# ErickRosete/tacorl

Hardware: AMD Instinct MI355X
Metric: offline grad-steps/sec (batch=256, 84x84 RGB) (higher is better)
Workload: dtype bf16; 1 GPU; tacorl actor-critic training_step, frozen LMP (BASELINE configs[1]); per_gpu_batch=256, global_batch=256, window=16, image=84x84x3, frames=fp32 CHW (reference batch schema), latent_plan=16, n_action_samples=4, phase=Q (epoch>=bc_epochs), action_decoder_loss=every step (reference behaviour), parallelism=dp1, hip_graph=True, losses_finite=True

## Files before the change

### include/tacorl_hip.h

```cpp
#ifndef TACORL_HIP_H
#define TACORL_HIP_H
#include <stddef.h>
#ifdef __cplusplus
extern "C" {
#endif

typedef void* tacorl_stream_t;

#define TACORL_MAXP 16
enum { TACORL_F32 = 0, TACORL_BF16 = 1 };
enum { TACORL_ACT_NONE = 0, TACORL_ACT_RELU = 1, TACORL_ACT_SILU = 2 };

int tacorl_hip_version(void);
int tacorl_hip_init(int device);
const char* tacorl_hip_last_error(void);
int tacorl_time_mark(unsigned long long* marks, int slot, tacorl_stream_t stream);
int tacorl_time_spin(unsigned long long* marks, int slot, long ticks, tacorl_stream_t stream);

int tacorl_linear_fwd(int nprob, const float* const* x, int ldx, const float* const* w,
                      const float* const* b, float* const* y, float* const* z, const int* M,
                      int K, int N, int act, int compute_dtype, tacorl_stream_t stream);
size_t tacorl_linear_add_fwd_ws_bytes(int nprob, const int* M, int K, int N);
int tacorl_linear_add_fwd(int nprob, const float* const* x, int ldx, const float* const* w,
                          const float* const* b, const float* const* addend, int ld_add, float* const* y,
                          int ldy, const int* M, int K, int N, int act, int compute_dtype, void* ws,
                          size_t ws_bytes, tacorl_stream_t stream);
int tacorl_rnn_linear_supported(int M, int K, int N);
int tacorl_rnn_linear_fwd(const void* x_bf16, const void* w_bf16, const float* bias, const float* addend,
                          int ld_add, float* y, void* y_bf16, int M, int K, int N, int act,
                          tacorl_stream_t stream);
int tacorl_rnn_linear_fwd_batch(int nprob, const void* const* x_bf16, const void* const* w_bf16,
                                const float* const* bias, const float* const* addend, int ld_add,
                                float* const* y, void* const* y_bf16, int M, int K, int N, const int* acts,
                                tacorl_stream_t stream);
int tacorl_rnn_linear_fwd_batch_twin(int nprob, const void* const* x_bf16, const void* const* x2_bf16,
                                     const void* const* w_bf16, const float* const* bias, const float* const* addend,
                                     const float* const* addend2, int ld_add, float* const* y, float* const* y2,
                                     void* const* y_bf16, void* const* y2_bf16, int M, int M2, int K, int N,
                                     const int* acts, tacorl_stream_t stream);
int tacorl_rnn_linear_fwd_batch_ext(int nprob, const void* const* x_bf16, const void* const* x2_bf16,
                                    const void* const* w_bf16, const float* const* bias, const float* const* addend,
                                    const float* const* addend2, int ld_add, float* const* y, float* const* y2,
                                    void* const* y_bf16, void* const* y2_bf16, int M, int M2, int K, int N,
                                    const int* acts, const void* const* x_ext, const void* const* x2_ext,
                                    const void* const* w_ext, const float* const* bias2, tacorl_stream_t stream);
int tacorl_build_ad_input_bf16(const float* plan, const float* emb, int ld_emb, void* out_bf16, int B, int T, int Tm,
                               int P, int E, tacorl_stream_t stream);
int tacorl_rnn_linear_bwd_step(const void* x_bf16, const void* wt_bf16, const float* addend, int ld_add,
                               const float* mask_src, float* y, void* y_bf16, int M, int K, int N,
                               tacorl_stream_t stream);
int tacorl_rnn_wgrad_supported(int R, int M, int N);
int tacorl_rnn_wgrad(const void* dz_bf16, int ld_dz, const void* x_bf16, int ld_x, int R, int M, int N, float* dw,
                     float* db, int accumulate, tacorl_stream_t stream);
int tacorl_rnn_wgrad_batch(int n, const void* const* dz_bf16, int ld_dz, const void* const* x_bf16, int ld_x, const int* R,
                           int M, int N, float* const* dw, float* const* db, int accumulate, tacorl_stream_t stream);
size_t tacorl_rnn_wgrad_slabs_ws_bytes(int slabs, int Mp, int N);
int tacorl_rnn_wgrad_slabs(const void* dz_bf16, int ld_dz, const void* x_bf16, int ld_x, int R, int Mp, int N, int rows,
                           int slabs, float* dw, float* db, int accumulate, void* ws, size_t ws_bytes, tacorl_stream_t stream);
int tacorl_rnn_linear_bwd_batch(int nprob, const void* const* x_bf16, const void* const* wt_bf16,
                                const float* const* addend, int ld_add, const float* const* mask_src,
                                float* const* y, void* const* y_bf16, int M, int K, int N, tacorl_stream_t stream);
int tacorl_transpose_to_bf16(const float* src, void* dst, int R, int C, tacorl_stream_t stream);
int tacorl_transpose_to_bf16_batch(int n, const float* const* src, void* const* dst, const int* R, const int* C,
                                   tacorl_stream_t stream);
int tacorl_transpose_pad_to_bf16(const float* src, void* dst, int R, int C, int ld_dst, tacorl_stream_t stream);
int tacorl_pad_to_bf16(const float* src, int ld_src, void* dst, int ld_dst, long rows, int cols, tacorl_stream_t stream);

int tacorl_linear_dgrad(int nprob, const float* const* dz, int ld_dz, const float* const* w,
                        float* const* out, int ld_out, const float* const* src, int ld_src, int act_src,
                        const float* const* addend, int ld_add, const int* M, int O, int I,
                        int compute_dtype, tacorl_stream_t stream);
size_t tacorl_linear_dgrad_ws_bytes(int nprob, const int* M, int O, int I);
int tacorl_linear_dgrad_splitk(int nprob, const float* const* dz, int ld_dz, const float* const* w,
                               float* const* out, int ld_out, const float* const* src, int ld_src, int act_src,
                               const float* const* addend, int ld_add, const int* M, int O, int I,
                               int compute_dtype, void* ws, size_t ws_bytes, tacorl_stream_t stream);
size_t tacorl_linear_wgrad_ws_bytes(int nprob, const int* M, int K, int O);
int tacorl_linear_wgrad(int nprob, const float* const* x, int ldx, const float* const* dz, int ld_dz,
                        const int* M, int K, int O, float* const* dw, float* const* db, int accumulate,
                        int compute_dtype, void* ws, size_t ws_bytes, tacorl_stream_t stream);
int tacorl_conv2d_relu_fwd(int nprob, const void* const* x, const float* const* w,
                           const float* const* b, float* const* y, const int* n_img, int H, int W,
                           int C, int KH, int KW, int S, int CO, int x_dtype, int compute_dtype,
                           tacorl_stream_t stream);

long tacorl_encoder_param_layout(long* offsets11);
long tacorl_encoder_act_layout(int n_img, int H, int W, long* offsets5);
int tacorl_encoder_fwd(int nprob, const void* const* img, const float* const* params,
                       float* const* out , float* const* act, const int* n_img, int H,
                       int W, int img_dtype, int compute_dtype, tacorl_stream_t stream);
size_t tacorl_encoder_bwd_ws_bytes(int nprob, const int* n_img, int H, int W);
int tacorl_encoder_bwd(int nprob, const void* const* img, const float* const* params,
                       const float* const* act, const float* const* d_out, float* const* grads,
                       const int* n_img, int H, int W, int img_dtype, int compute_dtype,
                       int accumulate, void* ws, size_t ws_bytes, tacorl_stream_t stream);

long tacorl_encoder_fused_wpk_bytes(void);
int tacorl_encoder_fused_supported(int H, int W);
int tacorl_encoder_fused_act_format(int H, int W);
int tacorl_encoder_pack_weights(int nprob, const float* const* params, void* const* packed,
                                tacorl_stream_t stream);
int tacorl_encoder_fwd_fused(int nprob, const void* const* img, const void* const* packed,
                             const float* const* params, float* const* out, float* const* act,
                             const int* n_img, int H, int W, tacorl_stream_t stream);
int tacorl_encoder_fwd_fused_wg(int nprob, const void* const* img, const void* const* packed,
                                const float* const* params, float* const* out, float* const* act,
                                const int* n_img, int H, int W, int max_workgroups, tacorl_stream_t stream);

size_t tacorl_encoder_bwd_fused_ws_bytes(int nprob, const int* n_img, int H, int W);
int tacorl_encoder_bwd_fused(int nprob, const void* const* img, const float* const* params,
                             const float* const* act, const float* const* d_out,
                             float* const* grads, const int* n_img, int H, int W, int accumulate,
                             void* ws, size_t ws_bytes, tacorl_stream_t stream);
int tacorl_encoder_bwd_fused_pack(int nprob, const float* const* params, const int* n_img, int H, int W,
                                  void* ws, size_t ws_bytes, tacorl_stream_t stream);
int tacorl_encoder_bwd_fused_head(int nprob, const float* const* params, const float* const* act,
                                  const float* const* d_out, const int* n_img, int H, int W,
                                  int prepacked, void* ws, size_t ws_bytes, tacorl_stream_t stream);
int tacorl_encoder_bwd_fused_fc_wgrad(int nprob, const float* const* act, const float* const* d_out,
                                      float* const* grads, const int* n_img, int H, int W,
                                      int accumulate, void* ws, size_t ws_bytes, tacorl_stream_t stream);
int tacorl_encoder_bwd_fused_conv(int nprob, const void* const* img, const float* const* params,
                                  const float* const* act, float* const* grads, const int* n_img, int H,
                                  int W, int accumulate, int prepacked, void* ws, size_t ws_bytes,
                                  tacorl_stream_t stream);
int tacorl_encoder_bwd_fused_conv_parts(int nprob, const void* const* img, const float* const* params,
                                        const float* const* act, float* const* grads, const int* n_img, int H,
                                        int W, int accumulate, int prepacked, int parts, void* ws,
                                        size_t ws_bytes, tacorl_stream_t stream);

long tacorl_mlp_param_layout(int n_layers, const int* dims, long* w_off, long* b_off);
long tacorl_mlp_act_layout(int M, int n_layers, const int* dims, const int* acts, long* z_off,
                           long* y_off);
int tacorl_mlp_fwd(int nprob, const float* const* x, int ldx, const float* const* params,
                   float* const* act, const int* M, int n_layers, const int* dims,
                   const int* acts, int compute_dtype, tacorl_stream_t stream);
int tacorl_mlp_fwd_fused_supported(int nprob, int n_layers, const int* dims, int ldx);
int tacorl_mlp_lean_supported(int nprob, int n_layers, const int* dims, int ldx, int ldo, int ldd);
int tacorl_mlp_fwd_fused(int nprob, const float* const* x, int ldx, const float* const* params,
                         const void* const* params_bf16, float* const* act, const int* M,
                         int n_layers, const int* dims, const int* acts, int lean, tacorl_stream_t stream);
int tacorl_mlp_fwd_fused_gather_supported(int nprob, const int* M, int n_layers, const int* dims, const int* acts,
                                          int ldx, int lean);
int tacorl_mlp_fwd_fused_gather(int nprob, const int* nseg, const float* const* seg_ptr, const int* seg_ld,
                                const int* seg_c0, const int* seg_mod, float* const* x_out, int ldx,
                                const float* const* params, const void* const* params_bf16, float* const* act,
                                const int* M, int n_layers, const int* dims, const int* acts, int lean,
                                tacorl_stream_t stream);
int tacorl_to_bf16_batch(int n, const float* const* src, void* const* dst, const long* count,
                         tacorl_stream_t stream);
size_t tacorl_mlp_bwd_ws_bytes(int nprob, const int* M, int n_layers, const int* dims);
int tacorl_mlp_bwd(int nprob, const float* const* x, int ldx, const float* const* params,
                   const float* const* act, const float* const* d_out, int ldo, float* const* grads,
                   float* const* d_x, int ldd, const int* M, int n_layers, const int* dims,
                   const int* acts, int compute_dtype, int accumulate, void* ws, size_t ws_bytes,
                   tacorl_stream_t stream);
int tacorl_mlp_bwd_fused_supported(int nprob, int n_layers, const int* dims, int ldo, int ldd);
size_t tacorl_mlp_bwd_fused_ws_bytes(int nprob, const int* M, int n_layers, const int* dims);
int tacorl_mlp_bwd_fused_dgrad(int nprob, const float* const* params, const float* const* act,
                               const float* const* d_out, int ldo, float* const* d_x, int ldd,
                               const int* M, int n_layers, const int* dims, const int* acts,
                               int prepacked, void* ws, size_t ws_bytes, tacorl_stream_t stream);
int tacorl_mlp_bwd_fused_pack(int nprob, const float* const* params, const int* M, int n_layers,
                              const int* dims, void* ws, size_t ws_bytes, tacorl_stream_t stream);
int tacorl_prep_batch_begin(void);
int tacorl_reduce_batch_begin(void);
int tacorl_reduce_batch_end(tacorl_stream_t stream);
int tacorl_prep_batch_end(tacorl_stream_t stream);
int tacorl_mlp_bwd_fused_wgrad(int nprob, const float* const* x, int ldx, const float* const* act,
                               const float* const* d_out, int ldo, float* const* grads, const int* M,
                               int n_layers, const int* dims, const int* acts, int accumulate, int lean,
                               void* ws, size_t ws_bytes, tacorl_stream_t stream);

int tacorl_pack_images(const float* src, long img_pitch, int src_nchw, void* dst, int dst_dtype,
                       int n, int C, int H, int W, tacorl_stream_t stream);
int tacorl_pack_images_batch(int njobs, const float* const* src, const long* img_pitch, void* const* dst,
                             const int* n_img, int dst_dtype, int H, int W, tacorl_stream_t stream);
int tacorl_pack_images_window_batch(int njobs, const float* const* src, const long* img_pitch, void* const* dst,
                                    const int* n_img, void* const* dst_first, void* const* dst_last,
                                    const int* window, int dst_dtype, int H, int W, tacorl_stream_t stream);
int tacorl_pack_images_u8_batch(int njobs, const void* const* src, const long* img_pitch_bytes, void* const* dst,
                                const int* n_img, int dst_dtype, int H, int W, tacorl_stream_t stream);
int tacorl_pack_images_u8_gather_batch(int njobs, const void* const* src, const long* img_pitch_bytes,
                                       const long* const* index, const int* index_stride, void* const* dst,
                                       const int* n_img, int dst_dtype, int H, int W, tacorl_stream_t stream);
int tacorl_gather_frames_u8(const void* frames, long frame_bytes, const long* index, void* dst, long n,
                            tacorl_stream_t stream);
int tacorl_pack_images_u8_aug_batch(int njobs, const void* const* src, const long* img_pitch_bytes,
                                    void* const* dst, const int* const* shift, const float* const* jitter,
                                    const int* n_img, int dst_dtype, int H, int W, int pad,
                                    tacorl_stream_t stream);
int tacorl_pack_images_u8_resize_aug_gather_batch(int njobs, const void* const* src, const long* img_pitch_bytes,
                                                  const long* const* index, const int* index_stride, void* const* dst,
                                                  const int* const* shift, const float* const* jitter, const int* n_img,
                                                  int dst_dtype, int src_H, int src_W, int H, int W, int pad,
                                                  tacorl_stream_t stream);
int tacorl_pack_images_u8_aug_gather_batch(int njobs, const void* const* src, const long* img_pitch_bytes,
                                           const long* const* index, const int* index_stride, void* const* dst,
                                           const int* const* shift, const float* const* jitter, const int* n_img,
                                           int dst_dtype, int H, int W, int pad, tacorl_stream_t stream);
int tacorl_stage_transition(const void* disp, int disp_dtype, float* reward, float* done, int B,
                            const float* acts_src, float* acts_dst, long n_acts, tacorl_stream_t stream);
int tacorl_copy_cols(const float* src, int ld_src, float* dst, int ld_dst, int rows, int cols,
                     int src_row_mod, int accumulate, tacorl_stream_t stream);
int tacorl_copy_cols_batch(int n, const float* const* src, const int* ld_src, float* const* dst,
                           const int* ld_dst, const int* rows, const int* cols,
                           const int* src_row_mod, const int* accumulate, tacorl_stream_t stream);
int tacorl_reduce_rows_mod(const float* in, int ld_in, float* out, int ld_out, int B, int cols,
                           int reps, tacorl_stream_t stream);
int tacorl_reduce_rows_mod_batch(int n, const float* const* in, int ld_in, float* const* out, int ld_out, int B,
                                 int cols, int reps, tacorl_stream_t stream);
int tacorl_uniform_actions(const float* u01, float* dst, int ld_dst, int rows, int A,
                           int discrete_gripper, tacorl_stream_t stream);

int tacorl_tanh_normal_sample(const float* head, int ld_head, const float* eps, const float* gumbel_u,
                              int hard_rsample, float* act_out, int ld_act, float* logp, int* grip_idx,
                              int n, int M, int Ac, tacorl_stream_t stream);
int tacorl_tanh_normal_sample_batch(int njobs, const float* const* head, int ld_head,
                                    const float* const* eps, const float* const* gumbel_u,
                                    const int* hard_rsample, float* const* act_out, int ld_act,
                                    float* const* logp, int* const* grip_idx, const int* n, int M, int Ac,
                                    const float* u01, float* u_dst, int u_rows, int A, int u_discrete,
                                    tacorl_stream_t stream);

int tacorl_add_rows_bcast(const float* x, int ldx, const float* add, float* out, int R, int T, int D,
                          int Dp, tacorl_stream_t stream);
int tacorl_attention_fwd(const float* qkv, float* out, int B, int T, int D, int H, tacorl_stream_t stream);
int tacorl_attention_dropout_fwd(const float* qkv, float* out, const unsigned char* keep, float keep_scale, int B,
                                 int T, int D, int H, tacorl_stream_t stream);
int tacorl_attention_dropout_bwd(const float* qkv, const float* d_out, float* d_qkv, const unsigned char* keep,
                                 float keep_scale, int B, int T, int D, int H, tacorl_stream_t stream);
int tacorl_dropout_mul(float* x, const unsigned char* keep, float keep_scale, long n, tacorl_stream_t stream);
int tacorl_add_layernorm_fwd(const float* x, const float* res, const float* w, const float* b, float* y,
                             float* stats, int R, int D, float eps, tacorl_stream_t stream);
int tacorl_pr_encoder_fused_supported(int D, int T, int H, int FF, int L);
int tacorl_pr_encoder_fused_train_supported(int D, int T, int H, int FF, int L);
int tacorl_pr_encoder_fused(const float* emb, int ld_emb, const float* params, const void* params_bf16,
                            const long* offsets, float* pooled, int B, int D, int T, int H, int FF, int L,
                            tacorl_stream_t stream);
int tacorl_pr_encoder_fused_sample(const float* emb, int ld_emb, const float* params, const void* params_bf16,
                                   const long* offsets, float* pooled, int B, int D, int T, int H, int FF, int L,
                                   const float* Wc, const float* bc, const float* eps, float* head, float* plan,
                                   int A, float min_std, tacorl_stream_t stream);
int tacorl_pr_encoder_fused_train(const float* emb, int ld_emb, const float* params, const void* params_bf16,
                                  const long* offsets, float* pooled, int B, int D, int T, int H, int FF, int L,
                                  float* const* save, tacorl_stream_t stream);
int tacorl_pr_encoder_bwd_fused(const float* params, const long* offsets, const float* d_pool, const float* d_head,
                                const float* Wc, int A2, float* dx, const float* const* saved, float* const* dz,
                                const void* const* wt, float* ln_part, float* const* ln_grads, int B, int D, int T, int H,
                                int FF, int L, tacorl_stream_t stream);
int tacorl_pr_encoder_fused_train_sample(const float* emb, int ld_emb, const float* params, const void* params_bf16,
                                         const long* offsets, float* pooled, int B, int D, int T, int H, int FF, int L,
                                         float* const* save, const float* Wc, const float* bc, const float* eps,
                                         float* head, float* plan, int A, float min_std, tacorl_stream_t stream);
int tacorl_pr_head_compose(const float* w_fc, const float* b_fc, const float* w_head, const float* b_head,
                           float* Wc, float* bc, int D, int FC, int A2, tacorl_stream_t stream);
int tacorl_mean_over_t(const float* x, float* out, int B, int T, int D, tacorl_stream_t stream);
int tacorl_pr_sample(const float* head, const float* eps, float* plan, float* mu_out, float* std_out,
                     int B, int A, float min_std, tacorl_stream_t stream);

int tacorl_build_ad_input(const float* plan, const float* emb, int ld_emb, float* out, int B, int T,
                          int Tm, int P, int E, tacorl_stream_t stream);
int tacorl_ad_input_proj(const float* plan, const float* emb, int ld_emb, const float* w_ih, const float* b_ih,
                         float* out, int B, int T, int Tm, int P, int E, int H, tacorl_stream_t stream);
size_t tacorl_logistic_mixture_ws_bytes(int B, int Tm, int Da);
int tacorl_logistic_mixture_loss(const float* heads, int ldh, const float* actions, float* d_heads,
                                 float* loss_out, int B, int T, int Tm, int Da, int K, int num_classes,
                                 float gripper_alpha, float grad_scale, void* ws, size_t ws_bytes,
                                 tacorl_stream_t stream);
int tacorl_logistic_mixture_finish(const void* ws, size_t ws_bytes, int B, int Tm, int Da, float* loss_out,
                                   tacorl_stream_t stream);
int tacorl_logistic_mixture_sample(const float* heads, int ldh, const float* rand_a, const float* rand_b,
                                   float* out, int R, int Da, int K, tacorl_stream_t stream);

int tacorl_relu_mask_mul(const float* dy, const float* add, const float* h, float* out, long n,
                         tacorl_stream_t stream);
int tacorl_ad_input_bwd(const float* dx, float* d_plan, float* d_emb, int ld_emb, int B, int T, int Tm,
                        int P, int E, int accumulate, tacorl_stream_t stream);
int tacorl_plmp_demb_finish(float* d_emb, const float* dx, int ld_dx, int D_in, const float* dS, int ld_ds,
                            const float* dgin, float* const* f_dout, int ncam, int B, int T, int Ec,
                            tacorl_stream_t stream);
int tacorl_bcast_over_t(const float* src, float* dst, int B, int T, int D, float scale, int accumulate,
                        tacorl_stream_t stream);
int tacorl_attention_bwd(const float* qkv, const float* d_out, float* d_qkv, int B, int T, int D, int H,
                         tacorl_stream_t stream);
size_t tacorl_add_layernorm_bwd_ws_bytes(int R, int D);
int tacorl_add_layernorm_bwd(const float* dy, const float* x, const float* res, const float* w,
                             const float* stats, float* dv, float* dw, float* db, int R, int D,
                             int accumulate, void* ws, size_t ws_bytes, tacorl_stream_t stream);
int tacorl_gauss_kl_balanced(const float* head_q, const float* head_p, float* d_head_q, float* d_head_p,
                             int B, int A, float kl_alpha, float kl_beta, float min_std, int balanced,
                             float grad_scale, float* out2, tacorl_stream_t stream);
int tacorl_pr_sample_bwd(const float* head, const float* eps, const float* d_plan, float* d_head, int B,
                         int A, float min_std, tacorl_stream_t stream);

enum {
  TACORL_LG_ALPHA_LOSS = 0, TACORL_LG_ALPHA, TACORL_LG_ACTOR_LOSS, TACORL_LG_BELL1, TACORL_LG_BELL2,
  TACORL_LG_CONS1, TACORL_LG_CONS2, TACORL_LG_Q1LOSS, TACORL_LG_Q2LOSS, TACORL_LG_ALPHA_P,
  TACORL_LG_ALPHA_P_LOSS, TACORL_LG_Q1_DATA, TACORL_LG_Q1_RAND, TACORL_LG_Q1_POL, TACORL_LG_Q2_DATA,
  TACORL_LG_Q2_RAND, TACORL_LG_Q2_POL, TACORL_LG_ACTION_LOSS, TACORL_LG_COUNT
};
int tacorl_alpha_loss(const float* logp, int B, const float* log_alpha, float target_entropy,
                      float grad_scale, float* g_log_alpha, float* logs, tacorl_stream_t stream);
int tacorl_alpha_loss_step(const float* logp, int B, float* log_alpha, float target_entropy, float* g_log_alpha,
                           float* logs, float* m, float* v, float lr, int* step_counter, tacorl_stream_t stream);
int tacorl_actor_qmin(const float* q1, const float* q2, const float* logp, int B, const float* log_alpha,
                      float* dq1, float* dq2, float grad_scale, float* logs, tacorl_stream_t stream);
int tacorl_actor_head_bwd(const float* head, int ld_head, const float* eps, const float* logp,
                          const float* g_act1, const float* g_act2, int ld_g, const float* value,
                          int ld_value, const int* grip_idx, const float* log_alpha, float grad_scale,
                          float* d_head, int B, int Ac, int has_grip, float* logs, tacorl_stream_t stream);

size_t tacorl_cql_ws_bytes(int B);
int tacorl_cql_loss(const float* q1, const float* q2, float* dq1, float* dq2, const float* tq1,
                    const float* tq2, const float* logp_cur, const float* logp_nxt, const float* next_logp,
                    const float* reward, const float* done, const float* log_alpha,
                    const float* log_alpha_prime, int B, int n, int A, float discount, float reward_scale,
                    float temp, float cons_w, float gap, int deterministic_backup, float grad_scale,
                    float* g_log_alpha_prime, float* logs, void* ws, size_t ws_bytes, tacorl_stream_t stream);

size_t tacorl_adam_ws_bytes(long n);
int tacorl_adam_step(float* param, const float* grad, float* m, float* v, long n, float lr,
                     float max_norm, int* step_counter, float* target, float tau, void* ws,
                     size_t ws_bytes, tacorl_stream_t stream);
size_t tacorl_adam_batch_ws_bytes(int nb);
int tacorl_adam_step_batch(int nb, float* const* param, const float* const* grad, float* const* m,
                           float* const* v, const long* n, const float* lr, const float* max_norm,
                           int* const* step_counter, float* const* target, const float* tau, void* ws,
                           size_t ws_bytes, tacorl_stream_t stream);
int tacorl_adam_step_batch_mirror(int nb, float* const* param, const float* const* grad, float* const* m,
// ... 10 lines not shown
```

### tacorl_amd/_lib.py

```python
import ctypes as C
import os

HERE = os.path.dirname(os.path.abspath(__file__))
LIB_PATH = os.environ.get("TACORL_HIP_LIB") or os.path.join(HERE, "lib", "libtacorl_hip.so")

F32, BF16 = 0, 1
ACT_NONE, ACT_RELU, ACT_SILU = 0, 1, 2
MAXP = 16

LOG_SLOTS = [
    "alpha_loss", "alpha", "actor_loss", "bellman_q1_loss", "bellman_q2_loss", "conservative_q1_loss",
    "conservative_q2_loss", "q1_loss", "q2_loss", "alpha_prime", "alpha_prime_loss", "q1_data", "q1_random",
    "q1_policy", "q2_data", "q2_random", "q2_policy", "action_loss",
]

_p, _i, _l, _f, _sz = C.c_void_p, C.c_int, C.c_long, C.c_float, C.c_size_t
_SIGS = {
    "tacorl_hip_version": (_i, []),
    "tacorl_hip_init": (_i, [_i]),
    "tacorl_hip_last_error": (C.c_char_p, []),
    "tacorl_time_mark": (_i, [_p, _i, _p]),
    "tacorl_time_spin": (_i, [_p, _i, _l, _p]),
    "tacorl_linear_fwd": (_i, [_i, _p, _i, _p, _p, _p, _p, _p, _i, _i, _i, _i, _p]),
    "tacorl_linear_add_fwd_ws_bytes": (_sz, [_i, _p, _i, _i]),
    "tacorl_linear_add_fwd": (_i, [_i, _p, _i, _p, _p, _p, _i, _p, _i, _p, _i, _i, _i, _i, _p, _sz, _p]),
    "tacorl_rnn_linear_supported": (_i, [_i, _i, _i]),
    "tacorl_rnn_linear_fwd": (_i, [_p, _p, _p, _p, _i, _p, _p, _i, _i, _i, _i, _p]),
    "tacorl_rnn_linear_fwd_batch": (_i, [_i, _p, _p, _p, _p, _i, _p, _p, _i, _i, _i, _p, _p]),
    "tacorl_rnn_linear_fwd_batch_twin": (_i, [_i, _p, _p, _p, _p, _p, _p, _i, _p, _p, _p, _p, _i, _i, _i, _i, _p, _p]),
    "tacorl_rnn_linear_fwd_batch_ext": (_i, [_i, _p, _p, _p, _p, _p, _p, _i, _p, _p, _p, _p, _i, _i, _i, _i, _p, _p, _p, _p, _p, _p]),
    "tacorl_rnn_linear_bwd_step": (_i, [_p, _p, _p, _i, _p, _p, _p, _i, _i, _i, _p]),
    "tacorl_rnn_linear_bwd_batch": (_i, [_i, _p, _p, _p, _i, _p, _p, _p, _i, _i, _i, _p]),
    "tacorl_rnn_wgrad_supported": (_i, [_i, _i, _i]),
    "tacorl_rnn_wgrad": (_i, [_p, _i, _p, _i, _i, _i, _i, _p, _p, _i, _p]),
    "tacorl_rnn_wgrad_batch": (_i, [_i, _p, _i, _p, _i, _p, _i, _i, _p, _p, _i, _p]),
    "tacorl_rnn_wgrad_slabs_ws_bytes": (_sz, [_i, _i, _i]),
    "tacorl_rnn_wgrad_slabs": (_i, [_p, _i, _p, _i, _i, _i, _i, _i, _i, _p, _p, _i, _p, _sz, _p]),
    "tacorl_transpose_to_bf16": (_i, [_p, _p, _i, _i, _p]),
    "tacorl_transpose_to_bf16_batch": (_i, [_i, _p, _p, _p, _p, _p]),
    "tacorl_transpose_pad_to_bf16": (_i, [_p, _p, _i, _i, _i, _p]),
    "tacorl_pad_to_bf16": (_i, [_p, _i, _p, _i, _l, _i, _p]),
    "tacorl_pr_encoder_fused_supported": (_i, [_i, _i, _i, _i, _i]),
    "tacorl_pr_encoder_fused_train_supported": (_i, [_i, _i, _i, _i, _i]),
    "tacorl_pr_encoder_fused": (_i, [_p, _i, _p, _p, _p, _p, _i, _i, _i, _i, _i, _i, _p]),
    "tacorl_pr_encoder_fused_train": (_i, [_p, _i, _p, _p, _p, _p, _i, _i, _i, _i, _i, _i, _p, _p]),
    "tacorl_pr_encoder_bwd_fused": (_i, [_p, _p, _p, _p, _p, _i, _p, _p, _p, _p, _p, _p, _i, _i, _i, _i, _i, _i, _p]),
    "tacorl_pr_encoder_fused_train_sample": (_i, [_p, _i, _p, _p, _p, _p, _i, _i, _i, _i, _i, _i, _p, _p, _p, _p, _p, _p, _i, _f, _p]),
    "tacorl_pr_encoder_fused_sample": (_i, [_p, _i, _p, _p, _p, _p, _i, _i, _i, _i, _i, _i, _p, _p, _p, _p, _p, _i, _f, _p]),
    "tacorl_pr_head_compose": (_i, [_p, _p, _p, _p, _p, _p, _i, _i, _i, _p]),
    "tacorl_to_bf16_batch": (_i, [_i, _p, _p, _p, _p]),
    "tacorl_mlp_bwd_fused_supported": (_i, [_i, _i, _p, _i, _i]),
    "tacorl_mlp_bwd_fused_ws_bytes": (_sz, [_i, _p, _i, _p]),
    "tacorl_mlp_bwd_fused_dgrad": (_i, [_i, _p, _p, _p, _i, _p, _i, _p, _i, _p, _p, _i, _p, _sz, _p]),
    "tacorl_mlp_bwd_fused_pack": (_i, [_i, _p, _p, _i, _p, _p, _sz, _p]),
    "tacorl_prep_batch_begin": (_i, []),
    "tacorl_reduce_batch_begin": (_i, []),
    "tacorl_reduce_batch_end": (_i, [_p]),
    "tacorl_prep_batch_end": (_i, [_p]),
    "tacorl_mlp_bwd_fused_wgrad": (_i, [_i, _p, _i, _p, _p, _i, _p, _p, _i, _p, _p, _i, _i, _p, _sz, _p]),
    "tacorl_mlp_fwd_fused_supported": (_i, [_i, _i, _p, _i]),
    "tacorl_mlp_lean_supported": (_i, [_i, _i, _p, _i, _i, _i]),
    "tacorl_mlp_fwd_fused": (_i, [_i, _p, _i, _p, _p, _p, _p, _i, _p, _p, _i, _p]),
    "tacorl_mlp_fwd_fused_gather_supported": (_i, [_i, _p, _i, _p, _p, _i, _i]),
    "tacorl_mlp_fwd_fused_gather": (_i, [_i, _p, _p, _p, _p, _p, _p, _i, _p, _p, _p, _p, _i, _p, _p, _i, _p]),
    "tacorl_add_rows_bcast": (_i, [_p, _i, _p, _p, _i, _i, _i, _i, _p]),
    "tacorl_attention_fwd": (_i, [_p, _p, _i, _i, _i, _i, _p]),
    "tacorl_attention_dropout_fwd": (_i, [_p, _p, _p, _f, _i, _i, _i, _i, _p]),
    "tacorl_attention_dropout_bwd": (_i, [_p, _p, _p, _p, _f, _i, _i, _i, _i, _p]),
    "tacorl_dropout_mul": (_i, [_p, _p, _f, _l, _p]),
    "tacorl_add_layernorm_fwd": (_i, [_p, _p, _p, _p, _p, _p, _i, _i, _f, _p]),
    "tacorl_mean_over_t": (_i, [_p, _p, _i, _i, _i, _p]),
    "tacorl_pr_sample": (_i, [_p, _p, _p, _p, _p, _i, _i, _f, _p]),
    "tacorl_build_ad_input": (_i, [_p, _p, _i, _p, _i, _i, _i, _i, _i, _p]),
    "tacorl_build_ad_input_bf16": (_i, [_p, _p, _i, _p, _i, _i, _i, _i, _i, _p]),
    "tacorl_ad_input_proj": (_i, [_p, _p, _i, _p, _p, _p, _i, _i, _i, _i, _i, _i, _p]),
    "tacorl_logistic_mixture_ws_bytes": (_sz, [_i, _i, _i]),
    "tacorl_logistic_mixture_loss": (_i, [_p, _i, _p, _p, _p, _i, _i, _i, _i, _i, _i, _f, _f, _p, _sz, _p]),
    "tacorl_logistic_mixture_finish": (_i, [_p, _sz, _i, _i, _i, _p, _p]),
    "tacorl_logistic_mixture_sample": (_i, [_p, _i, _p, _p, _p, _i, _i, _i, _p]),
    "tacorl_linear_dgrad": (_i, [_i, _p, _i, _p, _p, _i, _p, _i, _i, _p, _i, _p, _i, _i, _i, _p]),
    "tacorl_linear_dgrad_ws_bytes": (_sz, [_i, _p, _i, _i]),
    "tacorl_linear_dgrad_splitk": (_i, [_i, _p, _i, _p, _p, _i, _p, _i, _i, _p, _i, _p, _i, _i, _i, _p, _sz, _p]),
    "tacorl_linear_wgrad_ws_bytes": (_sz, [_i, _p, _i, _i]),
    "tacorl_linear_wgrad": (_i, [_i, _p, _i, _p, _i, _p, _i, _i, _p, _p, _i, _i, _p, _sz, _p]),
    "tacorl_relu_mask_mul": (_i, [_p, _p, _p, _p, _l, _p]),
    "tacorl_ad_input_bwd": (_i, [_p, _p, _p, _i, _i, _i, _i, _i, _i, _i, _p]),
    "tacorl_plmp_demb_finish": (_i, [_p, _p, _i, _i, _p, _i, _p, _p, _i, _i, _i, _i, _p]),
    "tacorl_bcast_over_t": (_i, [_p, _p, _i, _i, _i, _f, _i, _p]),
    "tacorl_attention_bwd": (_i, [_p, _p, _p, _i, _i, _i, _i, _p]),
    "tacorl_add_layernorm_bwd_ws_bytes": (_sz, [_i, _i]),
    "tacorl_add_layernorm_bwd": (_i, [_p, _p, _p, _p, _p, _p, _p, _p, _i, _i, _i, _p, _sz, _p]),
    "tacorl_gauss_kl_balanced": (_i, [_p, _p, _p, _p, _i, _i, _f, _f, _f, _i, _f, _p, _p]),
    "tacorl_pr_sample_bwd": (_i, [_p, _p, _p, _p, _i, _i, _f, _p]),
    "tacorl_conv2d_relu_fwd": (_i, [_i, _p, _p, _p, _p, _p, _i, _i, _i, _i, _i, _i, _i, _i, _i, _p]),
    "tacorl_encoder_param_layout": (_l, [_p]),
    "tacorl_encoder_act_layout": (_l, [_i, _i, _i, _p]),
    "tacorl_encoder_fwd": (_i, [_i, _p, _p, _p, _p, _p, _i, _i, _i, _i, _p]),
    "tacorl_encoder_bwd_ws_bytes": (_sz, [_i, _p, _i, _i]),
    "tacorl_encoder_bwd": (_i, [_i, _p, _p, _p, _p, _p, _p, _i, _i, _i, _i, _i, _p, _sz, _p]),
    "tacorl_encoder_fused_wpk_bytes": (_l, []),
    "tacorl_encoder_fused_supported": (_i, [_i, _i]),
    "tacorl_encoder_fused_act_format": (_i, [_i, _i]),
    "tacorl_encoder_pack_weights": (_i, [_i, _p, _p, _p]),
    "tacorl_encoder_fwd_fused": (_i, [_i, _p, _p, _p, _p, _p, _p, _i, _i, _p]),
    "tacorl_encoder_fwd_fused_wg": (_i, [_i, _p, _p, _p, _p, _p, _p, _i, _i, _i, _p]),
    "tacorl_encoder_bwd_fused_ws_bytes": (_sz, [_i, _p, _i, _i]),
    "tacorl_encoder_bwd_fused": (_i, [_i, _p, _p, _p, _p, _p, _p, _i, _i, _i, _p, _sz, _p]),
    "tacorl_encoder_bwd_fused_pack": (_i, [_i, _p, _p, _i, _i, _p, _sz, _p]),
    "tacorl_encoder_bwd_fused_head": (_i, [_i, _p, _p, _p, _p, _i, _i, _i, _p, _sz, _p]),
    "tacorl_encoder_bwd_fused_fc_wgrad": (_i, [_i, _p, _p, _p, _p, _i, _i, _i, _p, _sz, _p]),
    "tacorl_encoder_bwd_fused_conv": (_i, [_i, _p, _p, _p, _p, _p, _i, _i, _i, _i, _p, _sz, _p]),
    "tacorl_encoder_bwd_fused_conv_parts": (_i, [_i, _p, _p, _p, _p, _p, _i, _i, _i, _i, _i, _p, _sz, _p]),
    "tacorl_mlp_param_layout": (_l, [_i, _p, _p, _p]),
    "tacorl_mlp_act_layout": (_l, [_i, _i, _p, _p, _p, _p]),
    "tacorl_mlp_fwd": (_i, [_i, _p, _i, _p, _p, _p, _i, _p, _p, _i, _p]),
    "tacorl_mlp_bwd_ws_bytes": (_sz, [_i, _p, _i, _p]),
    "tacorl_mlp_bwd": (_i, [_i, _p, _i, _p, _p, _p, _i, _p, _p, _i, _p, _i, _p, _p, _i, _i, _p, _sz, _p]),
    "tacorl_pack_images": (_i, [_p, _l, _i, _p, _i, _i, _i, _i, _i, _p]),
    "tacorl_pack_images_batch": (_i, [_i, _p, _p, _p, _p, _i, _i, _i, _p]),
    "tacorl_pack_images_window_batch": (_i, [_i, _p, _p, _p, _p, _p, _p, _p, _i, _i, _i, _p]),
    "tacorl_pack_images_u8_batch": (_i, [_i, _p, _p, _p, _p, _i, _i, _i, _p]),
    "tacorl_pack_images_u8_gather_batch": (_i, [_i, _p, _p, _p, _p, _p, _p, _i, _i, _i, _p]),
    "tacorl_pack_images_u8_aug_gather_batch": (_i, [_i, _p, _p, _p, _p, _p, _p, _p, _p, _i, _i, _i, _i, _p]),
    "tacorl_pack_images_u8_resize_aug_gather_batch": (_i, [_i, _p, _p, _p, _p, _p, _p, _p, _p, _i, _i, _i, _i, _i, _i, _p]),
    "tacorl_gather_frames_u8": (_i, [_p, _l, _p, _p, _l, _p]),
    "tacorl_pack_images_u8_aug_batch": (_i, [_i, _p, _p, _p, _p, _p, _p, _i, _i, _i, _i, _p]),
    "tacorl_stage_transition": (_i, [_p, _i, _p, _p, _i, _p, _p, _l, _p]),
    "tacorl_copy_cols": (_i, [_p, _i, _p, _i, _i, _i, _i, _i, _p]),
    "tacorl_copy_cols_batch": (_i, [_i, _p, _p, _p, _p, _p, _p, _p, _p, _p]),
    "tacorl_reduce_rows_mod": (_i, [_p, _i, _p, _i, _i, _i, _i, _p]),
    "tacorl_reduce_rows_mod_batch": (_i, [_i, _p, _i, _p, _i, _i, _i, _i, _p]),
    "tacorl_uniform_actions": (_i, [_p, _p, _i, _i, _i, _i, _p]),
    "tacorl_tanh_normal_sample": (_i, [_p, _i, _p, _p, _i, _p, _i, _p, _p, _i, _i, _i, _p]),
    "tacorl_tanh_normal_sample_batch": (_i, [_i, _p, _i, _p, _p, _p, _p, _i, _p, _p, _p, _i, _i, _p, _p, _i, _i, _i, _p]),
    "tacorl_alpha_loss": (_i, [_p, _i, _p, _f, _f, _p, _p, _p]),
    "tacorl_alpha_loss_step": (_i, [_p, _i, _p, _f, _p, _p, _p, _p, _f, _p, _p]),
    "tacorl_actor_qmin": (_i, [_p, _p, _p, _i, _p, _p, _p, _f, _p, _p]),
    "tacorl_actor_head_bwd": (_i, [_p, _i, _p, _p, _p, _p, _i, _p, _i, _p, _p, _f, _p, _i, _i, _i, _p, _p]),
    "tacorl_cql_ws_bytes": (_sz, [_i]),
    "tacorl_cql_loss": (_i, [_p] * 13 + [_i, _i, _i, _f, _f, _f, _f, _f, _i, _f, _p, _p, _p, _sz, _p]),
    "tacorl_adam_ws_bytes": (_sz, [_l]),
    "tacorl_adam_step": (_i, [_p, _p, _p, _p, _l, _f, _f, _p, _p, _f, _p, _sz, _p]),
    "tacorl_adam_batch_ws_bytes": (_sz, [_i]),
    "tacorl_adam_step_batch": (_i, [_i, _p, _p, _p, _p, _p, _p, _p, _p, _p, _p, _p, _sz, _p]),
    "tacorl_adam_step_batch_mirror": (_i, [_i, _p, _p, _p, _p, _p, _p, _p, _p, _p, _p, _p, _p, _p, _sz, _p]),
}

_lib = None


class TacorlHipError(RuntimeError):
    pass


def lib():
    global _lib
    if _lib is None:
        import torch

        if not os.path.exists(LIB_PATH):
            raise TacorlHipError(
                f"{LIB_PATH} not found: the HIP extension is required (no CPU fallback). "
                "Build it with `python -m tacorl_amd.build`.")
        L = C.CDLL(LIB_PATH)
        override = bool(os.environ.get("TACORL_HIP_LIB"))
        missing = []
        for name, (res, args) in _SIGS.items():
            fn = getattr(L, name, None)
            if fn is None:
                missing.append(name)
                continue
            fn.restype, fn.argtypes = res, args
        if override:
            import sys

            if missing:
                raise TacorlHipError(f"TACORL_HIP_LIB={LIB_PATH} lacks {len(missing)} entry point(s) of this binding "
                                     f"({', '.join(missing[:5])}...): rebuild it from this tree")
            print(f"[tacorl_amd] TACORL_HIP_LIB override active: {LIB_PATH}", file=sys.stderr, flush=True)
        _lib = L
    return _lib


def declared_symbols():
    return list(_SIGS)


def call(name, *args):
    fn = getattr(lib(), name)
    rc = fn(*args)
    if fn.restype is _i and rc != 0:
        raise TacorlHipError(f"{name} failed ({rc}): {lib().tacorl_hip_last_error().decode()}")
    return rc


def ptr(t):
    return None if t is None else C.c_void_p(t.data_ptr())


def ptr_array(tensors):
    arr = (C.c_void_p * len(tensors))()
    for i, t in enumerate(tensors):
        if t is None:
            arr[i] = None
        elif isinstance(t, int):
            arr[i] = t
        elif isinstance(t, C.c_void_p):
            arr[i] = t.value
        else:
            arr[i] = t.data_ptr()
    return arr


def int_array(vals):
    return (C.c_int * len(vals))(*[int(v) for v in vals])


def stream():
    import torch

    return C.c_void_p(torch.cuda.current_stream().cuda_stream)
```

### tacorl_amd/csrc/encoder_fused.h

```cpp
#pragma once
#include "../../include/tacorl_hip.h"
#include "common.h"

#define EF_CHUNK 16
constexpr int cmaxi(int a, int b) { return a > b ? a : b; }
#define EF_MAXCH 12
#define EF_MAXP 16
#define ACT1_STRIDE 80
#define SA_STRIDE 272
#define H1_STRIDE 528

typedef unsigned int u32x4 __attribute__((ext_vector_type(4)));
typedef unsigned int u32x2 __attribute__((ext_vector_type(2)));

struct EFProblem {
  const __bf16* img;
  const u32x4* wpk;
  const float* params;
  float* out;
  float* act;
  long a_y2, a_y3, a_sa, a_h1;
  int n_img;
  int cost;
  long ustart;
};
struct EFArgs {
  EFProblem p[EF_MAXP];
  long utotal;
  int nprob;
  int H, W, OH1, OW1, OH2, OW2, OH3, OW3;
  int img_bytes;
  int lds_img;
  int act_bf16;
};

#define WP_C1 0
#define WP_C2 (WP_C1 + 2 * 6 * 64)
#define WP_C3 (WP_C2 + 4 * 16 * 64)
#define WP_F1 (WP_C3 + 4 * 18 * 64)
#define WP_F2 (WP_F1 + 16 * 4 * 64)
#define WP_TOTAL (WP_F2 + 2 * 8 * 64)

__device__ __forceinline__ bf16x8 as_bf16x8(u32x4 v) { return __builtin_bit_cast(bf16x8, v); }
__device__ __forceinline__ float relu1(float x) {
  float r;
  asm("v_max_f32_e32 %0, 0, %1" : "=v"(r) : "v"(x));
  return r;
}
#define EF_DPP4(OP, CTRL, x)                                                                  \
  asm volatile(OP " %0, %0, %0 " CTRL " row_mask:0xf bank_mask:0xf\n\t"                        \
               OP " %1, %1, %1 " CTRL " row_mask:0xf bank_mask:0xf\n\t"                        \
               OP " %2, %2, %2 " CTRL " row_mask:0xf bank_mask:0xf\n\t"                        \
               OP " %3, %3, %3 " CTRL " row_mask:0xf bank_mask:0xf"                             \
               : "+v"((x)[0]), "+v"((x)[1]), "+v"((x)[2]), "+v"((x)[3]))
#define EF_DPP4_FIRST(OP, CTRL, x)                                                            \
  asm volatile("s_nop 1\n\t"                                                                   \
               OP " %0, %0, %0 " CTRL " row_mask:0xf bank_mask:0xf\n\t"                        \
               OP " %1, %1, %1 " CTRL " row_mask:0xf bank_mask:0xf\n\t"                        \
               OP " %2, %2, %2 " CTRL " row_mask:0xf bank_mask:0xf\n\t"                        \
               OP " %3, %3, %3 " CTRL " row_mask:0xf bank_mask:0xf"                             \
               : "+v"((x)[0]), "+v"((x)[1]), "+v"((x)[2]), "+v"((x)[3]))
#define EF_ROW16_4(OP, x)                          \
  do {                                             \
    EF_DPP4_FIRST(OP, "quad_perm:[1,0,3,2]", x);   \
    EF_DPP4(OP, "quad_perm:[2,3,0,1]", x);         \
    EF_DPP4(OP, "row_half_mirror", x);             \
    EF_DPP4(OP, "row_mirror", x);                  \
  } while (0)
__device__ __forceinline__ u32x2 pack4_bf16(float a, float b, float c, float d) {
  bf16x4 t = {(__bf16)a, (__bf16)b, (__bf16)c, (__bf16)d};
  return __builtin_bit_cast(u32x2, t);
}

#ifndef EF_VAR
#define EF_VAR 0
#endif
#if EF_VAR & 2
#define MFMA_AW(acc, wfrag, bfrag) asm volatile("" : "+v"(acc) : "a"(wfrag), "v"(bfrag))
#else
#define MFMA_AW(acc, wfrag, bfrag) \
  asm volatile("v_mfma_f32_16x16x32_bf16 %0, %1, %2, %0" : "+v"(acc) : "a"(wfrag), "v"(bfrag))
#endif
#define MFMA_CHAIN_BEGIN(acc) asm volatile("s_nop 1" : "+v"(acc))
#if EF_VAR & 2
#define MFMA_FIRST_AW(acc, wfrag, bfrag, bias) asm volatile("" : "=v"(acc) : "a"(wfrag), "v"(bfrag), "v"(bias))
#else
#define MFMA_FIRST_AW(acc, wfrag, bfrag, bias) \
  asm volatile("v_mfma_f32_16x16x32_bf16 %0, %1, %2, %3" : "=v"(acc) : "a"(wfrag), "v"(bfrag), "v"(bias))
#endif
#define MFMA_CHAIN_END(acc) asm volatile("s_nop 11" : "+v"(acc))
#if EF_VAR & 2
#define EF_MFMA_TXT(...) ""
#else
#define EF_MFMA_TXT(...) __VA_ARGS__
#endif

int ef_ring_supported(int H, int W);
int ef_ring_launch(EFArgs& a, int nb, int H, int W, hipStream_t st);
```

### tacorl_amd/csrc/encoder_fused.hip

```cpp
#include <stdio.h>
#include <stdlib.h>

#include "encoder_fused.h"
#include "enc_bwd_fused.h"

#ifndef EF_DEFER
#define EF_DEFER 1
#endif
#define EF_DCHUNK 8
#ifndef EF_SETUP_COST
#define EF_SETUP_COST 128
#endif
#ifndef EF_ACT_COST
#define EF_ACT_COST 72
#endif


struct EFPackArgs {
  const float* params[16];
  u32x4* out[16];
};
__global__ void ef_pack_kernel(EFPackArgs a, long o_w1, long o_w2, long o_w3, long o_f1, long o_f2) {
  const float* __restrict__ params = a.params[blockIdx.y];
  u32x4* __restrict__ out = a.out[blockIdx.y];
  const int f = blockIdx.x * 4 + (threadIdx.x >> 6), l = threadIdx.x & 63;
  if (f >= WP_TOTAL / 64) return;
  const float* W; int K, j, s;
  if (f < WP_C2 / 64) { W = params + o_w1; K = 192; j = f / 6; s = f % 6; }
  else if (f < WP_C3 / 64) { int r = f - WP_C2 / 64; W = params + o_w2; K = 512; j = r / 16; s = r % 16; }
  else if (f < WP_F1 / 64) { int r = f - WP_C3 / 64; W = params + o_w3; K = 576; j = r / 18; s = r % 18; }
  else if (f < WP_F2 / 64) { int r = f - WP_F1 / 64; W = params + o_f1; K = 128; j = r / 4; s = r % 4; }
  else { int r = f - WP_F2 / 64; W = params + o_f2; K = 256; j = r / 8; s = r % 8; }
  const float* src = W + (long)(16 * j + (l & 15)) * K + 32 * s + 8 * (l >> 4);
  if (f < WP_C2 / 64)
    src = W + (long)(8 * ((l & 15) >> 2) + 4 * j + (l & 3)) * K + (4 * (s / 3) + (l >> 4)) * 24 + 8 * (s % 3);
  else if (f < WP_C3 / 64)
    src = W + (long)(32 * (j >> 1) + 8 * ((l & 15) >> 2) + 4 * (j & 1) + (l & 3)) * K + 32 * s + 8 * (l >> 4);
  bf16x8 v;
#pragma unroll
  for (int e = 0; e < 8; e++) v[e] = (__bf16)src[e];
  out[(long)f * 64 + l] = __builtin_bit_cast(u32x4, v);
}

extern "C" long tacorl_encoder_fused_wpk_bytes(void) { return (long)WP_TOTAL * 16; }
extern "C" int tacorl_encoder_pack_weights(int nprob, const float* const* params, void* const* packed,
                                           tacorl_stream_t stream) {
  long po[11];
  tacorl_encoder_param_layout(po);
  if (nprob < 1 || nprob > 16) return TACORL_EINVAL;
  EFPackArgs a{};
  for (int p = 0; p < nprob; p++) { a.params[p] = params[p]; a.out[p] = (u32x4*)packed[p]; }
  hipLaunchKernelGGL(ef_pack_kernel, dim3((WP_TOTAL / 64 + 3) / 4, nprob), dim3(256), 0, (hipStream_t)stream, a, po[0],
                     po[2], po[4], po[7], po[9]);
  return hipGetLastError() == hipSuccess ? TACORL_OK : TACORL_ELAUNCH;
}

#define MFMA6_FIRST(acc, bias, w, o, f) \
  asm volatile(EF_MFMA_TXT("v_mfma_f32_16x16x32_bf16 %0, %1, %7, %13\n\t" \
      "v_mfma_f32_16x16x32_bf16 %0, %2, %8, %0\n\t" \
      "v_mfma_f32_16x16x32_bf16 %0, %3, %9, %0\n\t" \
      "v_mfma_f32_16x16x32_bf16 %0, %4, %10, %0\n\t" \
      "v_mfma_f32_16x16x32_bf16 %0, %5, %11, %0\n\t" \
      "v_mfma_f32_16x16x32_bf16 %0, %6, %12, %0\n\t") \
      : "=&v"(acc) : "a"((w)[(o) + 0]), "a"((w)[(o) + 1]), "a"((w)[(o) + 2]), "a"((w)[(o) + 3]), "a"((w)[(o) + 4]), "a"((w)[(o) + 5]), "v"((f)[0]), "v"((f)[1]), "v"((f)[2]), "v"((f)[3]), "v"((f)[4]), "v"((f)[5]), "v"(bias))
#define MFMA6_MORE(acc, w, o, f) \
  asm volatile(EF_MFMA_TXT("v_mfma_f32_16x16x32_bf16 %0, %1, %7, %0\n\t" \
      "v_mfma_f32_16x16x32_bf16 %0, %2, %8, %0\n\t" \
      "v_mfma_f32_16x16x32_bf16 %0, %3, %9, %0\n\t" \
      "v_mfma_f32_16x16x32_bf16 %0, %4, %10, %0\n\t" \
      "v_mfma_f32_16x16x32_bf16 %0, %5, %11, %0\n\t" \
      "v_mfma_f32_16x16x32_bf16 %0, %6, %12, %0\n\t") \
      : "+v"(acc) : "a"((w)[(o) + 0]), "a"((w)[(o) + 1]), "a"((w)[(o) + 2]), "a"((w)[(o) + 3]), "a"((w)[(o) + 4]), "a"((w)[(o) + 5]), "v"((f)[0]), "v"((f)[1]), "v"((f)[2]), "v"((f)[3]), "v"((f)[4]), "v"((f)[5]))
#define MFMA8_FIRST(acc, bias, w, o, f) \
  asm volatile(EF_MFMA_TXT("v_mfma_f32_16x16x32_bf16 %0, %1, %9, %17\n\t" \
      "v_mfma_f32_16x16x32_bf16 %0, %2, %10, %0\n\t" \
      "v_mfma_f32_16x16x32_bf16 %0, %3, %11, %0\n\t" \
      "v_mfma_f32_16x16x32_bf16 %0, %4, %12, %0\n\t" \
      "v_mfma_f32_16x16x32_bf16 %0, %5, %13, %0\n\t" \
      "v_mfma_f32_16x16x32_bf16 %0, %6, %14, %0\n\t" \
      "v_mfma_f32_16x16x32_bf16 %0, %7, %15, %0\n\t" \
      "v_mfma_f32_16x16x32_bf16 %0, %8, %16, %0\n\t") \
      : "=&v"(acc) : "a"((w)[(o) + 0]), "a"((w)[(o) + 1]), "a"((w)[(o) + 2]), "a"((w)[(o) + 3]), "a"((w)[(o) + 4]), "a"((w)[(o) + 5]), "a"((w)[(o) + 6]), "a"((w)[(o) + 7]), "v"((f)[0]), "v"((f)[1]), "v"((f)[2]), "v"((f)[3]), "v"((f)[4]), "v"((f)[5]), "v"((f)[6]), "v"((f)[7]), "v"(bias))
#define MFMA8_MORE(acc, w, o, f) \
  asm volatile(EF_MFMA_TXT("v_mfma_f32_16x16x32_bf16 %0, %1, %9, %0\n\t" \
      "v_mfma_f32_16x16x32_bf16 %0, %2, %10, %0\n\t" \
      "v_mfma_f32_16x16x32_bf16 %0, %3, %11, %0\n\t" \
      "v_mfma_f32_16x16x32_bf16 %0, %4, %12, %0\n\t" \
      "v_mfma_f32_16x16x32_bf16 %0, %5, %13, %0\n\t" \
      "v_mfma_f32_16x16x32_bf16 %0, %6, %14, %0\n\t" \
      "v_mfma_f32_16x16x32_bf16 %0, %7, %15, %0\n\t" \
      "v_mfma_f32_16x16x32_bf16 %0, %8, %16, %0\n\t") \
      : "+v"(acc) : "a"((w)[(o) + 0]), "a"((w)[(o) + 1]), "a"((w)[(o) + 2]), "a"((w)[(o) + 3]), "a"((w)[(o) + 4]), "a"((w)[(o) + 5]), "a"((w)[(o) + 6]), "a"((w)[(o) + 7]), "v"((f)[0]), "v"((f)[1]), "v"((f)[2]), "v"((f)[3]), "v"((f)[4]), "v"((f)[5]), "v"((f)[6]), "v"((f)[7]))
#define MFMA9_FIRST(acc, bias, w, o, f) \
  asm volatile(EF_MFMA_TXT("v_mfma_f32_16x16x32_bf16 %0, %1, %10, %19\n\t" \
      "v_mfma_f32_16x16x32_bf16 %0, %2, %11, %0\n\t" \
      "v_mfma_f32_16x16x32_bf16 %0, %3, %12, %0\n\t" \
      "v_mfma_f32_16x16x32_bf16 %0, %4, %13, %0\n\t" \
      "v_mfma_f32_16x16x32_bf16 %0, %5, %14, %0\n\t" \
      "v_mfma_f32_16x16x32_bf16 %0, %6, %15, %0\n\t" \
      "v_mfma_f32_16x16x32_bf16 %0, %7, %16, %0\n\t" \
      "v_mfma_f32_16x16x32_bf16 %0, %8, %17, %0\n\t" \
      "v_mfma_f32_16x16x32_bf16 %0, %9, %18, %0\n\t") \
      : "=&v"(acc) : "a"((w)[(o) + 0]), "a"((w)[(o) + 1]), "a"((w)[(o) + 2]), "a"((w)[(o) + 3]), "a"((w)[(o) + 4]), "a"((w)[(o) + 5]), "a"((w)[(o) + 6]), "a"((w)[(o) + 7]), "a"((w)[(o) + 8]), "v"((f)[0]), "v"((f)[1]), "v"((f)[2]), "v"((f)[3]), "v"((f)[4]), "v"((f)[5]), "v"((f)[6]), "v"((f)[7]), "v"((f)[8]), "v"(bias))
#define MFMA9_MORE(acc, w, o, f) \
  asm volatile(EF_MFMA_TXT("v_mfma_f32_16x16x32_bf16 %0, %1, %10, %0\n\t" \
      "v_mfma_f32_16x16x32_bf16 %0, %2, %11, %0\n\t" \
      "v_mfma_f32_16x16x32_bf16 %0, %3, %12, %0\n\t" \
      "v_mfma_f32_16x16x32_bf16 %0, %4, %13, %0\n\t" \
      "v_mfma_f32_16x16x32_bf16 %0, %5, %14, %0\n\t" \
      "v_mfma_f32_16x16x32_bf16 %0, %6, %15, %0\n\t" \
      "v_mfma_f32_16x16x32_bf16 %0, %7, %16, %0\n\t" \
      "v_mfma_f32_16x16x32_bf16 %0, %8, %17, %0\n\t" \
      "v_mfma_f32_16x16x32_bf16 %0, %9, %18, %0\n\t") \
      : "+v"(acc) : "a"((w)[(o) + 0]), "a"((w)[(o) + 1]), "a"((w)[(o) + 2]), "a"((w)[(o) + 3]), "a"((w)[(o) + 4]), "a"((w)[(o) + 5]), "a"((w)[(o) + 6]), "a"((w)[(o) + 7]), "a"((w)[(o) + 8]), "v"((f)[0]), "v"((f)[1]), "v"((f)[2]), "v"((f)[3]), "v"((f)[4]), "v"((f)[5]), "v"((f)[6]), "v"((f)[7]), "v"((f)[8]))


template <int H_, int W_>
struct EFGeom {
  static constexpr int H = H_, W = W_;
  static constexpr int OH1 = (H - 8) / 4 + 1, OW1 = (W - 8) / 4 + 1;
  static constexpr int OH2 = (OH1 - 4) / 2 + 1, OW2 = (OW1 - 4) / 2 + 1;
  static constexpr int OH3 = OH2 - 2, OW3 = OW2 - 2;
  static constexpr int IMG_BYTES = H * W * 6;
  static constexpr int NPX1 = OH1 * OW1, NPX2 = OH2 * OW2, NPX3 = OH3 * OW3;
  static constexpr int PAD1 = (H == 84 && W == 84) ? 16 : (H == 44 && W == 60) ? 0 : 48;
  static constexpr int PX2 = 160;
  static constexpr int PAD2 = (H == 44 && W == 60) ? 32 : 192;
  static constexpr int PITCH1 = OW1 * 80 + PAD1, PITCH2 = OW2 * PX2 + PAD2;
  static constexpr int ACT1_BYTES = OH1 * PITCH1, ACT2_BYTES = OH2 * PITCH2;
  static constexpr bool S2 = (H == 84 && W == 84);
  static constexpr int D1S = 16 * 64 + 16, D2S = 9 * 128 + 16;
  static constexpr bool DEFER = EF_DEFER != 0 && NPX2 % 16 == 1 && NPX3 % 16 == 1 && NPX2 > 16 && NPX3 > 16 &&
                                2 * ((IMG_BYTES + 15) & ~15) + ACT1_BYTES + ACT2_BYTES + EF_CHUNK * (272 + 528) +
                                        EF_DCHUNK * (D1S + D2S) <= 160 * 1024;
  static constexpr int DEFER_BYTES = DEFER ? EF_DCHUNK * (D1S + D2S) : 0;
  static constexpr int NPX2M = DEFER ? NPX2 - 1 : NPX2, NPX3M = DEFER ? NPX3 - 1 : NPX3;
  static constexpr int FIXED_BYTES = ACT1_BYTES + ACT2_BYTES + EF_CHUNK * (272 + 528) + DEFER_BYTES;
  static constexpr bool WHOLE = 2 * ((IMG_BYTES + 15) & ~15) + FIXED_BYTES <= 160 * 1024;
  static constexpr int BR = WHOLE ? OH1 : 4, NB = (OH1 + BR - 1) / BR;
  static constexpr int BAND_ROWS = WHOLE ? H : 4 * BR + 4;
  static constexpr int BAND_BYTES = BAND_ROWS * W * 6, LDS_IMG = (BAND_BYTES + 15) & ~15;
  static constexpr int NPXB = BR * OW1;
  static constexpr int LDS_BYTES = 2 * LDS_IMG + FIXED_BYTES;
  static constexpr bool OK = (WHOLE ? IMG_BYTES % 16 == 0 : (W * 6) % 16 == 0) && BAND_BYTES <= EF_MAXCH * 256 * 16 &&
                             LDS_BYTES <= 160 * 1024 && OH3 >= 1 && OW3 >= 1;
};

#ifndef EF_VAR
#define EF_VAR 0
#endif
#ifndef EF_X
#define EF_X 0
#endif
#if EF_X & 8
#define EF_IMG_BARRIER() do { } while (0)
#else
#define EF_IMG_BARRIER() __builtin_amdgcn_s_barrier()
#endif
#if defined(EF_STAMPS) || defined(EF_BLKCLK)
__device__ unsigned long long ef_blk[512];
extern "C" int tacorl_ef_blk_read(unsigned long long* out) {
  return hipMemcpyFromSymbol(out, HIP_SYMBOL(ef_blk), sizeof(ef_blk)) == hipSuccess ? TACORL_OK : TACORL_ELAUNCH;
}
#endif
// ... 44 lines not shown
  if ((long)u_hi <= seg_s || (long)u_lo >= seg_e) continue;
  const int pcost = a_.p[pi].cost;
  const long f0 = (long)u_lo > seg_s ? ((long)u_lo - seg_s + pcost - 1) / pcost : 0;
  const long f1 = (long)u_hi < seg_e ? ((long)u_hi - seg_s + pcost - 1) / pcost : a_.p[pi].n_img;
  if (f1 <= f0) continue;
  const EFProblem P = a_.p[pi];
  int tid;
  asm volatile("v_mov_b32 %0, 0" : "=v"(tid));
  tid += threadIdx.x;
  const int w = tid >> 6, l = tid & 63, r16 = l & 15, g = l >> 4;
  const int nworkers = 1;
  const long worker = f0, seg_end = f1;

  unsigned char* act1 = lds + 2 * a.lds_img;
  const int npx1 = a.OH1 * a.OW1, npx2 = a.OH2 * a.OW2, npx3 = a.OH3 * a.OW3;
  unsigned char* act2 = act1 + G::ACT1_BYTES;
  unsigned char* sa = act2 + G::ACT2_BYTES;
  unsigned char* h1 = sa + EF_CHUNK * SA_STRIDE;
  unsigned char* const d1 = h1 + EF_CHUNK * H1_STRIDE;
  unsigned char* const d2 = d1 + EF_DCHUNK * G::D1S;
  unsigned char* const ps = h1;
  static_assert(!G::DEFER || EF_DCHUNK * 1024 <= EF_CHUNK * H1_STRIDE, "the soft-argmax state fits the FC tail's h1 buffer");
  static_assert(EF_CHUNK % EF_DCHUNK == 0, "a leftover-pixel group never straddles an FC chunk");

  long po[11];
  {
    const long sz[11] = {32 * 8 * 8 * 3, 32, 64 * 4 * 4 * 32, 64, 64 * 3 * 3 * 64, 64, 1, 256 * 128, 256, 32 * 256, 32};
    long off = 0;
    for (int i = 0; i < 11; i++) { po[i] = off; off = (off + sz[i] + 3) & ~3L; }
  }
  const int cg = w & 1, ph = w >> 1;
  u32x4 wc1a[6], wc1b[6], wc2a[16], wc2b[16], wc3[18];
#pragma unroll
  for (int s = 0; s < 6; s++) { wc1a[s] = P.wpk[WP_C1 + s * 64 + l]; wc1b[s] = P.wpk[WP_C1 + (6 + s) * 64 + l]; }
#pragma unroll
  for (int s = 0; s < 16; s++) {
    wc2a[s] = P.wpk[WP_C2 + ((2 * cg) * 16 + s) * 64 + l];
    wc2b[s] = P.wpk[WP_C2 + ((2 * cg + 1) * 16 + s) * 64 + l];
  }
#pragma unroll
  for (int s = 0; s < 18; s++) wc3[s] = P.wpk[WP_C3 + (w * 18 + s) * 64 + l];
  float b1[2][4], b2[2][4], b3[4];
#pragma unroll
  for (int q = 0; q < 4; q++) {
    b1[0][q] = P.params[po[1] + 8 * g + q];
    b1[1][q] = P.params[po[1] + 8 * g + 4 + q];
    b2[0][q] = P.params[po[3] + 32 * cg + 8 * g + q];
    b2[1][q] = P.params[po[3] + 32 * cg + 8 * g + 4 + q];
    b3[q] = P.params[po[5] + 16 * w + 4 * g + q];
  }
  const f32x4 bias1a = {b1[0][0], b1[0][1], b1[0][2], b1[0][3]}, bias1b = {b1[1][0], b1[1][1], b1[1][2], b1[1][3]},
              bias2a = {b2[0][0], b2[0][1], b2[0][2], b2[0][3]}, bias2b = {b2[1][0], b2[1][1], b2[1][2], b2[1][3]},
              bias3 = {b3[0], b3[1], b3[2], b3[3]};
  const float temp = P.params[po[6]];
  asm volatile("" ::"v"(bias1a), "v"(bias1b), "v"(bias2a), "v"(bias2b), "v"(bias3), "v"(temp));

#if EF_VAR & 1
  u32x4 kconst;
  asm volatile("v_mov_b32 %0, 0x3c003c00" : "=v"(kconst[0]));
  kconst[1] = kconst[2] = kconst[3] = kconst[0];
#endif
  const int k1g = g * a.W * 6;

  const unsigned dma_voff = G::WHOLE ? (unsigned)l * 16u : (unsigned)tid * 16u;
  const unsigned dma_voff_l = (unsigned)l * 16u;
  const unsigned lds_base = (unsigned)(unsigned long)(__attribute__((address_space(3))) unsigned char*)lds;
  constexpr int NPC = (G::IMG_BYTES + 1023) / 1024;
  constexpr int NT1W = (G::NPXB + 15) >> 4, PER1W = (NT1W + 3) >> 2, NFULL = NT1W - 4 * (PER1W - 1);
  constexpr int DQ_BAL = NFULL == 4 ? (NPC + 3) / 4 : (NPC + 4 * NFULL + 3) / 4;
  constexpr int DQ_HI = PER1W > 1 && DQ_BAL > 2 * (PER1W - 1) ? 2 * (PER1W - 1) : DQ_BAL;
  constexpr int DQ_LO = NFULL == 4 ? DQ_HI : cmaxi((NPC - (4 - NFULL) * DQ_HI + NFULL - 1) / NFULL, 0);
  static_assert(!G::WHOLE || NFULL * DQ_LO + (4 - NFULL) * DQ_HI >= NPC, "every KiB of the image has an issuer");
  const int wu = __builtin_amdgcn_readfirstlane(w);
  const int dqn = wu < NFULL ? DQ_LO : DQ_HI, dq0 = wu < NFULL ? wu * DQ_LO : NFULL * DQ_LO + (wu - NFULL) * DQ_HI;
  auto dma_pieces = [&](long img_idx, int band, int buf, int i0, int i1) {
    const int row0 = G::WHOLE ? 0 : 4 * G::BR * band;
    const int rows = G::WHOLE ? G::H : min(G::BAND_ROWS, G::H - row0);
    const int n16 = G::WHOLE ? (G::IMG_BYTES >> 4) : (rows * G::W * 6) >> 4;
    const unsigned char* src = reinterpret_cast<const unsigned char*>(P.img) + img_idx * G::IMG_BYTES + row0 * (G::W * 6);
    if constexpr (!G::WHOLE) {
      static_assert(G::WHOLE || G::BAND_BYTES <= 4 * 4096, "a band is at most four KiB pieces per wave");
      const int p0 = 4 * wu, left = n16 - p0 * 64, nfull = left <= 0 ? 0 : (left >= 256 ? 4 : left >> 6);
      const unsigned dstw = lds_base + buf * a.lds_img + p0 * 1024;
      const unsigned char* srcw = src + p0 * 1024;
      const unsigned m0v = __builtin_amdgcn_readfirstlane(dstw);
      unsigned keep_m0;
#define EF_BAND_ASM(LOADS)                                                                                              \
  asm volatile("s_mov_b32 %0, m0\n\ts_mov_b32 m0, %2\n\ts_nop 0\n\t" LOADS "s_mov_b32 m0, %0"                         \
               : "=&s"(keep_m0) : "v"(dma_voff_l), "s"(m0v), "s"(srcw) : "memory")
#define EF_LD(OFF) "global_load_lds_dwordx4 %1, %3 offset:" #OFF "\n\t"
      if (nfull == 4) EF_BAND_ASM(EF_LD(0) EF_LD(1024) EF_LD(2048) EF_LD(3072));
      else if (nfull == 3) EF_BAND_ASM(EF_LD(0) EF_LD(1024) EF_LD(2048));
      else if (nfull == 2) EF_BAND_ASM(EF_LD(0) EF_LD(1024));
      else if (nfull == 1) EF_BAND_ASM(EF_LD(0));
      const int part = left - 64 * nfull;
      if (nfull < 4 && part > 0 && l < part) {
        asm volatile("s_mov_b32 %0, m0\n\ts_mov_b32 m0, %2\n\ts_nop 0\n\tglobal_load_lds_dwordx4 %1, %3\n\ts_mov_b32 m0, %0"
                     : "=&s"(keep_m0)
                     : "v"(dma_voff_l), "s"(__builtin_amdgcn_readfirstlane(dstw + nfull * 1024)), "s"(srcw + nfull * 1024)
                     : "memory");
      }
#undef EF_LD
#undef EF_BAND_ASM
      return;
    }
    const unsigned dst0 = lds_base + buf * a.lds_img + (G::WHOLE ? dq0 : w) * 1024;
    if constexpr (G::WHOLE) src += dq0 * 1024;
#pragma unroll
    for (int i = i0; i < i1; i++) {
      if (i >= (G::WHOLE ? DQ_HI : EF_MAXCH)) break;
      constexpr int STEP = G::WHOLE ? 1024 : 4096;
      const int c0 = G::WHOLE ? (dq0 + i) * 64 : i * 256 + w * 64;
      constexpr int LASTN = (G::IMG_BYTES >> 4) - (NPC - 1) * 64;
      const bool wave_on = G::WHOLE ? (i < dqn && dq0 + i < NPC) : c0 < n16;
      if (wave_on) {
        if (G::WHOLE ? (dq0 + i < NPC - 1 || l < LASTN) : (c0 + l < n16)) {
          unsigned keep_m0;
          asm volatile("s_mov_b32 %0, m0\n\ts_mov_b32 m0, %2\n\ts_nop 0\n\tglobal_load_lds_dwordx4 %1, %3\n\ts_mov_b32 m0, %0"
                       : "=&s"(keep_m0)
                       : "v"(dma_voff), "s"(__builtin_amdgcn_readfirstlane(dst0 + i * STEP)), "s"(src + i * STEP)
                       : "memory");
        }
      }
    }
  };
  auto dma_load = [&](long img_idx, int band, int buf) { dma_pieces(img_idx, band, buf, 0, G::WHOLE ? DQ_HI : EF_MAXCH); };
  constexpr int DQ0_LAST = NFULL == 4 ? 3 * DQ_HI : NFULL * DQ_LO + (3 - NFULL) * DQ_HI;
  constexpr int ILAST = NPC - 1 - DQ0_LAST;
  const unsigned char* lean_src = nullptr;
  unsigned lean_dst = 0;
  auto lean_begin = [&](long img_idx, int buf) {
    lean_src = reinterpret_cast<const unsigned char*>(P.img) + img_idx * G::IMG_BYTES + dq0 * 1024;
    lean_dst = lds_base + buf * a.lds_img + dq0 * 1024;
  };
#define EF_LEAN_LD(OFF) asm volatile("global_load_lds_dwordx4 %0, %1 offset:" #OFF :: "v"(dma_voff), "s"(gsrc) : "memory")
  auto lean_piece = [&](int i) {
    if (!G::WHOLE || i >= DQ_HI) return;
    const bool on = i < DQ_LO || wu >= NFULL;
    if (!on) return;
    if (i > ILAST && wu == 3) return;
    const unsigned char* gsrc = lean_src + (i & ~3) * 1024;
    if ((i & 3) == 0) asm volatile("s_mov_b32 m0, %0\n\ts_nop 0" :: "s"(__builtin_amdgcn_readfirstlane(lean_dst + i * 1024)) : "memory");
    constexpr int LASTN = (G::IMG_BYTES >> 4) - (NPC - 1) * 64;
    if (i == ILAST && wu == 3 && l >= LASTN) return;
    switch (i & 3) {
      case 0: EF_LEAN_LD(0); break;
      case 1: EF_LEAN_LD(1024); break;
      case 2: EF_LEAN_LD(2048); break;
      default: EF_LEAN_LD(3072); break;
    }
  };
#undef EF_LEAN_LD

  long cur = worker;
  int it = 0, buf = 0;
  dma_load(cur, 0, 0);
  __builtin_amdgcn_s_waitcnt(0x0F70);
  __syncthreads();
  STAMP(0);

  while (true) {
    const int slot = it & (EF_CHUNK - 1);
    const int dslot = it & (EF_DCHUNK - 1);
    const long nxt = cur + nworkers;
    const bool has_next = nxt < seg_end;
#pragma unroll 1
    for (int band = 0; band < G::NB; band++) {
#if !(EF_X & 1)
      if (band + 1 < G::NB) dma_load(cur, band + 1, buf ^ 1);
      else if (has_next && !G::WHOLE) dma_load(nxt, 0, buf ^ 1);
#endif
#if EF_X & 4
      if (G::WHOLE) lean_begin(worker, buf ^ 1);
#else
      if (G::WHOLE) lean_begin(has_next ? nxt : cur, buf ^ 1);
#endif
      STAMP(1);
      const unsigned char* ib = lds + buf * a.lds_img;
      constexpr int NT1 = (G::NPXB + 15) >> 4, PER1 = (NT1 + 3) >> 2;
      const int npxb = G::WHOLE ? npx1 : min(G::BR, a.OH1 - band * G::BR) * a.OW1;
      const int nt1 = G::WHOLE ? NT1 : (npxb + 15) >> 4, px0 = band * G::NPXB;
      auto px1 = [&](int mt, int& oy, int& ox) -> bool {
        if (G::S2) {
          constexpr int half = G::OW1 / 2, NE = G::OH1 * half, TE = NE / 16, REM = NE % 16;
          static_assert(!G::S2 || (G::OW1 % 2 == 0 && REM <= 8 && G::WHOLE), "stride-2 conv1 tiles");
          int par, n; bool ok = true;
          if (mt < 2 * TE) { par = mt >= TE ? 1 : 0; n = 16 * (mt - par * TE) + r16; }
          else { par = r16 >> 3; n = 16 * TE + (r16 & 7); ok = (r16 & 7) < REM; n = min(n, NE - 1); }
          oy = n / half; ox = 2 * (n - oy * half) + par;
          return ok;
        } else {
          const int pb = mt * 16 + r16, pc = min(pb, npxb - 1);
          oy = pc / a.OW1; ox = pc - oy * a.OW1;
          return pb < npxb;
        }
      };
      auto base1 = [&](int oy, int ox) { return ib + ((4 * oy * a.W + 4 * ox) * 3) * 2 + k1g; };
      auto ld1 = [&](const unsigned char* base, u32x4 (&bf)[6]) {
#pragma unroll
        for (int s = 0; s < 6; s++) {
          const int off = (s / 3) * 4 * G::W * 6 + (s % 3) * 16;
#if EF_VAR & 1
          bf[s] = kconst; (void)base;
#else
          const u32x2 lo = *reinterpret_cast<const u32x2*>(base + off);
          const u32x2 hi = *reinterpret_cast<const u32x2*>(base + off + 8);
          bf[s] = u32x4{lo[0], lo[1], hi[0], hi[1]};
#endif
        }
      };
      auto ld1one = [&](const unsigned char* base, int s) -> u32x4 {
        const int off = (s / 3) * 4 * G::W * 6 + (s % 3) * 16;
#if EF_VAR & 1
        (void)base; return kconst;
#else
        const u32x2 lo = *reinterpret_cast<const u32x2*>(base + off);
        const u32x2 hi = *reinterpret_cast<const u32x2*>(base + off + 8);
        return u32x4{lo[0], lo[1], hi[0], hi[1]};
#endif
      };
      constexpr int DPT = !G::WHOLE ? 0 : PER1 > 1 ? cmaxi((DQ_HI + PER1 - 2) / (PER1 - 1), (DQ_LO + PER1 - 1) / PER1) : DQ_HI;
      static_assert(DPT <= 2, "a tile's first chain places at most two DMA pieces");
      constexpr bool OV = G::WHOLE;
      f32x4 A0[PER1], A1[PER1];
      int OY[PER1], OX[PER1];
      bool OK[PER1];
#pragma unroll
      for (int i = 0; i < PER1; i++) OK[i] = px1(min(w + 4 * i, nt1 - 1), OY[i], OX[i]);
      auto epi1 = [&](int i) {
        if (OK[i]) {
          const f32x4 acc0 = A0[i], acc1 = A1[i];
          const int oyi = band * G::BR + OY[i], ox = OX[i];
          const f32x4 r0 = {relu1(acc0[0]), relu1(acc0[1]), relu1(acc0[2]), relu1(acc0[3])};
          const f32x4 r1 = {relu1(acc1[0]), relu1(acc1[1]), relu1(acc1[2]), relu1(acc1[3])};
          const u32x2 lo = pack4_bf16(r0[0], r0[1], r0[2], r0[3]), hi = pack4_bf16(r1[0], r1[1], r1[2], r1[3]);
          const u32x4 pk = {lo[0], lo[1], hi[0], hi[1]};
#if !(EF_X & 2)
          *reinterpret_cast<u32x4*>(act1 + oyi * G::PITCH1 + ox * ACT1_STRIDE + (8 * g) * 2) = pk;
#else
          asm volatile("" :: "v"(pk));
#endif
          if (P.act)
            *reinterpret_cast<u32x4*>(reinterpret_cast<__bf16*>(P.act) + (long)cur * npx1 * 32 + (unsigned)((oyi * a.OW1 + ox) * 32 + 8 * g)) = pk;
        }
      };
      u32x4 fa[6], fb[6];
      auto dma_of_tile = [&](int i) {
#if !(EF_X & 1)
        if (G::WHOLE) {
#pragma unroll
          for (int q = 0; q < DPT; q++) lean_piece(i * DPT + q);
        }
#endif
      };
      auto chains1 = [&](int i, u32x4 (&bf)[6], int prev) {
        const bool do_refill = i + 2 < PER1;
        const unsigned char* refill = base1(OY[do_refill ? i + 2 : i], OX[do_refill ? i + 2 : i]);
        __builtin_amdgcn_sched_barrier(0);
        MFMA_FIRST_AW(A0[i], wc1a[0], bf[0], bias1a);
#pragma unroll
        for (int s = 1; s < 6; s++) {
          MFMA_AW(A0[i], wc1a[s], bf[s]);
#if !(EF_X & 1)
          if (G::WHOLE && (s == 1 || s == 3) && (s >> 1) < DPT) lean_piece(i * DPT + (s >> 1));
#endif
          if (s == 4 && prev >= 0) {
            asm volatile("" : "+v"(A0[prev]), "+v"(A1[prev]));
            epi1(prev);
          }
          if (i == 0 && PER1 > 1) {
            const unsigned char* b1 = base1(OY[1], OX[1]);
            if (s == 1) fb[0] = ld1one(b1, 0);
            if (s == 2) { fb[1] = ld1one(b1, 1); fb[2] = ld1one(b1, 2); }
            if (s == 3) fb[3] = ld1one(b1, 3);
            if (s == 4) { fb[4] = ld1one(b1, 4); fb[5] = ld1one(b1, 5); }
          }
          __builtin_amdgcn_sched_barrier(0);
        }
        MFMA_FIRST_AW(A1[i], wc1b[0], bf[0], bias1b);
#pragma unroll
        for (int s = 1; s < 6; s++) {
          MFMA_AW(A1[i], wc1b[s], bf[s]);
          if (do_refill) bf[s - 1] = ld1one(refill, s - 1);
          __builtin_amdgcn_sched_barrier(0);
        }
        if (do_refill) bf[5] = ld1one(refill, 5);
        __builtin_amdgcn_sched_barrier(0);
      };
      auto finish1 = [&](int i) {
        MFMA_CHAIN_END(A1[i]);
        asm volatile("" : "+v"(A0[i]));
        epi1(i);
      };
      ld1(base1(OY[0], OX[0]), fa);
#pragma unroll
      for (int i = 0; i < PER1; i++) {
        const bool exists = (OV && i + 1 < PER1) || w + 4 * i < nt1;
        if (exists) {
          if (i & 1) chains1(i, fb, OV && i > 0 ? i - 1 : -1); else chains1(i, fa, OV && i > 0 ? i - 1 : -1);
          if (!OV || i + 1 == PER1) finish1(i);
        } else {
          dma_of_tile(i);
          if (OV && i > 0) finish1(i - 1);
        }
      }
      static_assert(!G::WHOLE || ((PER1 - (NFULL < 4 ? 1 : 0)) * DPT >= DQ_HI && PER1 * DPT >= DQ_LO), "every piece of the next image is issued");
      if (band + 1 < G::NB) {
        asm volatile("s_waitcnt vmcnt(0)" ::: "memory");
        __syncthreads();
        buf ^= 1;
      }
    }
    STAMP(2);
    asm volatile("s_waitcnt lgkmcnt(0)" ::: "memory");
    EF_IMG_BARRIER();
    STAMP(3);

    {
      constexpr int NT2 = (G::NPX2M + 15) >> 4;
      auto base2 = [&](int mt) {
        const int pc = min(mt * 16 + r16, npx2 - 1);
        const int oy = pc / a.OW2, ox = pc - oy * a.OW2;
        return act1 + (2 * oy) * G::PITCH1 + 2 * ox * ACT1_STRIDE + 16 * g;
      };
      auto ld2 = [&](const unsigned char* base, int h, u32x4 (&bf)[8]) {
#pragma unroll
        for (int i = 0; i < 8; i++) {
          const int s = 8 * h + i, ky = s >> 2, kx = s & 3;
#if EF_VAR & 1
          bf[i] = kconst; (void)base;
#else
          bf[i] = *reinterpret_cast<const u32x4*>(base + ky * G::PITCH1 + kx * ACT1_STRIDE);
#endif
        }
      };
      u32x4 fa[8], fb[8];
      auto ld2one = [&](const unsigned char* base, int s) -> u32x4 {
#if EF_VAR & 1
        (void)base; return kconst;
#else
        return *reinterpret_cast<const u32x4*>(base + (s >> 2) * G::PITCH1 + (s & 3) * ACT1_STRIDE);
#endif
      };
      constexpr int PER2 = (NT2 + 1) / 2;
      f32x4 C0[PER2], C1[PER2];
      auto epi2 = [&](int t2) {
        const f32x4 acc0 = C0[t2], acc1 = C1[t2];
        int oz;
        asm volatile("s_mov_b32 %0, 0" : "=s"(oz));
        const int pm = (ph + 2 * t2) * 16 + r16 + oz;
        if (pm < npx2) {
          const f32x4 r0 = {relu1(acc0[0]), relu1(acc0[1]), relu1(acc0[2]), relu1(acc0[3])};
          const f32x4 r1 = {relu1(acc1[0]), relu1(acc1[1]), relu1(acc1[2]), relu1(acc1[3])};
          const u32x2 lo = pack4_bf16(r0[0], r0[1], r0[2], r0[3]), hi = pack4_bf16(r1[0], r1[1], r1[2], r1[3]);
          const u32x4 pk = {lo[0], lo[1], hi[0], hi[1]};
          const int oy2 = pm / a.OW2, ox2 = pm - oy2 * a.OW2;
          *reinterpret_cast<u32x4*>(act2 + oy2 * G::PITCH2 + ox2 * G::PX2 + (32 * cg + 8 * g) * 2) = pk;
          if (P.act) {
            __bf16* y = reinterpret_cast<__bf16*>(P.act + P.a_y2) + (long)cur * (npx2 * 64) + (unsigned)(pm * 64 + 32 * cg + 8 * g);
            *reinterpret_cast<u32x4*>(y) = pk;
          }
        }
      };
      auto finish2 = [&](int t2) {
        MFMA_CHAIN_END(C1[t2]);
        asm volatile("" : "+v"(C0[t2]));
        epi2(t2);
      };
      if constexpr (G::DEFER) {
        static_assert(!G::DEFER || (NT2 == 5 && PER2 == 3 && G::NPX2M == 80), "leftover-pixel deferral: five full conv2 tiles");
        u32x4 d1v;
        const bool d1w = wu == 3;
        int lz;
        asm volatile("v_mov_b32 %0, 0" : "=v"(lz));
        lz += l;
        if (d1w) d1v = *reinterpret_cast<const u32x4*>(act1 + (2 * (G::OH2 - 1) + (lz >> 4)) * G::PITCH1 +
                                                        (2 * (G::OW2 - 1) + ((lz >> 2) & 3)) * ACT1_STRIDE + (lz & 3) * 16);
        const unsigned char* bcur = base2(ph);
        const unsigned char* const bfirst = bcur;
        ld2(bcur, 0, fa);
        if (d1w) *reinterpret_cast<u32x4*>(d1 + dslot * G::D1S + (lz >> 2) * 64 + (lz & 3) * 16) = d1v;
        auto epi2h = [&]() {
          const f32x4 acc = C0[2];
          int oz;
          asm volatile("s_mov_b32 %0, 0" : "=s"(oz));
          const int pm = (NT2 - 1) * 16 + r16 + oz;
          const int gq = (l + oz) >> 4;
          const u32x2 pk = pack4_bf16(relu1(acc[0]), relu1(acc[1]), relu1(acc[2]), relu1(acc[3]));
          const int oy2 = pm / a.OW2, ox2 = pm - oy2 * a.OW2;
          *reinterpret_cast<u32x2*>(act2 + oy2 * G::PITCH2 + ox2 * G::PX2 + (32 * cg + 8 * gq + 4 * ph) * 2) = pk;
          if (P.act) {
            __bf16* y = reinterpret_cast<__bf16*>(P.act + P.a_y2) + (long)cur * (npx2 * 64) + (unsigned)(pm * 64 + 32 * cg + 8 * gq + 4 * ph);
            *reinterpret_cast<u32x2*>(y) = pk;
          }
        };
#pragma unroll
        for (int t2 = 0; t2 < 2; t2++) {
          const int mt = ph + 2 * t2;
          bcur = base2(t2 == 0 ? mt + 2 : NT2 - 1);
          __builtin_amdgcn_sched_barrier(0);
          MFMA_FIRST_AW(C0[t2], wc2a[0], fa[0], bias2a);
#pragma unroll
          for (int i = 1; i < 8; i++) {
            MFMA_AW(C0[t2], wc2a[i], fa[i]);
            if (i == 4 && t2 > 0) {
              asm volatile("" : "+v"(C0[t2 - 1]), "+v"(C1[t2 - 1]));
              epi2(t2 - 1);
            }
            if (t2 == 0) fb[i - 1] = ld2one(bfirst, 8 + i - 1);
            __builtin_amdgcn_sched_barrier(0);
          }
          if (t2 == 0) fb[7] = ld2one(bfirst, 15);
          MFMA_FIRST_AW(C1[t2], wc2b[0], fa[0], bias2b);
#pragma unroll
          for (int i = 1; i < 8; i++) {
            MFMA_AW(C1[t2], wc2b[i], fa[i]);
            fa[i - 1] = ld2one(bcur, i - 1);
            __builtin_amdgcn_sched_barrier(0);
          }
          MFMA_AW(C0[t2], wc2a[8], fb[0]);
          fa[7] = ld2one(bcur, 7);
          __builtin_amdgcn_sched_barrier(0);
#pragma unroll
          for (int i = 1; i < 8; i++) MFMA_AW(C0[t2], wc2a[8 + i], fb[i]);
          MFMA_AW(C1[t2], wc2b[8], fb[0]);
#pragma unroll
          for (int i = 1; i < 8; i++) {
            MFMA_AW(C1[t2], wc2b[8 + i], fb[i]);
            fb[i - 1] = ld2one(bcur, 8 + i - 1);
            __builtin_amdgcn_sched_barrier(0);
          }
          fb[7] = ld2one(bcur, 15);
          __builtin_amdgcn_sched_barrier(0);
        }
        if (ph == 0) {
          MFMA_FIRST_AW(C0[2], wc2a[0], fa[0], bias2a);
#pragma unroll
          for (int i = 1; i < 5; i++) MFMA_AW(C0[2], wc2a[i], fa[i]);
        } else {
          MFMA_FIRST_AW(C0[2], wc2b[0], fa[0], bias2b);
#pragma unroll
          for (int i = 1; i < 5; i++) MFMA_AW(C0[2], wc2b[i], fa[i]);
        }
        __builtin_amdgcn_sched_barrier(0);
        asm volatile("" : "+v"(C0[1]), "+v"(C1[1]));
        epi2(1);
        __builtin_amdgcn_sched_barrier(0);
        if (ph == 0) {
#pragma unroll
          for (int i = 5; i < 16; i++) { if (i < 8) MFMA_AW(C0[2], wc2a[i], fa[i]); else MFMA_AW(C0[2], wc2a[i], fb[i - 8]); }
        } else {
#pragma unroll
          for (int i = 5; i < 16; i++) { if (i < 8) MFMA_AW(C0[2], wc2b[i], fa[i]); else MFMA_AW(C0[2], wc2b[i], fb[i - 8]); }
        }
        MFMA_CHAIN_END(C0[2]);
        epi2h();
      } else if (ph < NT2) {
        const unsigned char* bcur = base2(ph);
        const unsigned char* const bfirst = bcur;
        ld2(bcur, 0, fa);
#pragma unroll
        for (int t2 = 0; t2 < PER2; t2++) {
          const int mt = ph + 2 * t2;
          const bool exists = t2 + 1 < PER2 || NT2 % 2 == 0 || mt < NT2;
          if (exists) {
            bcur = base2(mt + 2 < NT2 ? mt + 2 : mt);
            const bool refill = NT2 % 2 != 0 || t2 + 1 < NT2 / 2;
            __builtin_amdgcn_sched_barrier(0);
            MFMA_FIRST_AW(C0[t2], wc2a[0], fa[0], bias2a);
#pragma unroll
            for (int i = 1; i < 8; i++) {
              MFMA_AW(C0[t2], wc2a[i], fa[i]);
              if (i == 4 && t2 > 0) {
                asm volatile("" : "+v"(C0[t2 - 1]), "+v"(C1[t2 - 1]));
                epi2(t2 - 1);
              }
              if (t2 == 0) fb[i - 1] = ld2one(bfirst, 8 + i - 1);
              __builtin_amdgcn_sched_barrier(0);
            }
            if (t2 == 0) fb[7] = ld2one(bfirst, 15);
            MFMA_FIRST_AW(C1[t2], wc2b[0], fa[0], bias2b);
#pragma unroll
            for (int i = 1; i < 8; i++) {
              MFMA_AW(C1[t2], wc2b[i], fa[i]);
              if (refill) fa[i - 1] = ld2one(bcur, i - 1);
              __builtin_amdgcn_sched_barrier(0);
            }
            MFMA_AW(C0[t2], wc2a[8], fb[0]);
            if (refill) fa[7] = ld2one(bcur, 7);
            __builtin_amdgcn_sched_barrier(0);
#pragma unroll
            for (int i = 1; i < 8; i++) MFMA_AW(C0[t2], wc2a[8 + i], fb[i]);
            MFMA_AW(C1[t2], wc2b[8], fb[0]);
#pragma unroll
            for (int i = 1; i < 8; i++) {
              MFMA_AW(C1[t2], wc2b[8 + i], fb[i]);
              if (refill) fb[i - 1] = ld2one(bcur, 8 + i - 1);
              __builtin_amdgcn_sched_barrier(0);
            }
            if (refill) fb[7] = ld2one(bcur, 15);
            __builtin_amdgcn_sched_barrier(0);
            if (t2 + 1 == PER2) finish2(t2);
          } else if (t2 > 0) {
            finish2(t2 - 1);
          }
        }
      }
    }
    STAMP(4);
    const bool early_land = G::WHOLE && P.act == nullptr;
#if EF_X & 32
    if (early_land) asm volatile("s_waitcnt lgkmcnt(0)" ::: "memory");
#else
    if (early_land) asm volatile("s_waitcnt vmcnt(0) lgkmcnt(0)" ::: "memory");
#endif
    else asm volatile("s_waitcnt lgkmcnt(0)" ::: "memory");
    EF_IMG_BARRIER();
    STAMP(5);

    {
      constexpr int NT3 = (G::NPX3M + 15) >> 4;
      const float inv_t = (1.0f / temp) * 1.44269504088896f;
      u32x4 d2v;
      const bool d2w = G::DEFER && wu == 2;
      int lz3 = 0;
      if (G::DEFER) { asm volatile("v_mov_b32 %0, 0" : "=v"(lz3)); lz3 += l; }
      if (d2w) {
        const int j = lz3 >> 3, ky = (j * 11) >> 5, kx = j - 3 * ky;
        d2v = *reinterpret_cast<const u32x4*>(act2 + (G::OH3 - 1 + ky) * G::PITCH2 + (G::OW3 - 1 + kx) * G::PX2 + (lz3 & 7) * 16);
      }
      f32x4 v3[NT3];
      float fx[NT3], fy[NT3];
      auto base3 = [&](int mt, int& ox, int& oy) {
        const int pc = min(mt * 16 + r16, npx3 - 1);
        oy = pc / a.OW3; ox = pc - oy * a.OW3;
        return act2 + oy * G::PITCH2 + ox * G::PX2 + 16 * g;
      };
      auto ld3 = [&](const unsigned char* base, int h, u32x4 (&bf)[9]) {
#pragma unroll
        for (int i = 0; i < 9; i++) {
          const int s = 9 * h + i, tap = s >> 1, ky = tap / 3, kx = tap - 3 * ky;
#if EF_VAR & 1
          bf[i] = kconst; (void)base;
#else
          bf[i] = *reinterpret_cast<const u32x4*>(base + ky * G::PITCH2 + kx * G::PX2 + 64 * (s & 1));
#endif
        }
      };
      u32x4 fa[9], fb[9];
      int ox, oy;
      const unsigned char* bcur = base3(0, ox, oy);
      const unsigned char* const bfirst = bcur;
      ld3(bcur, 0, fa);
      if (d2w) *reinterpret_cast<u32x4*>(d2 + dslot * G::D2S + (lz3 >> 3) * 128 + (lz3 & 7) * 16) = d2v;
      auto ld3one = [&](const unsigned char* base, int s) -> u32x4 {
        const int tap = s >> 1, ky = tap / 3, kx = tap - 3 * ky;
#if EF_VAR & 1
        (void)base; return kconst;
#else
        return *reinterpret_cast<const u32x4*>(base + ky * G::PITCH2 + kx * G::PX2 + 64 * (s & 1));
#endif
      };
      f32x4 accs[NT3];
      auto epi3 = [&](int mt) {
        const f32x4 acc = accs[mt];
        const bool ok = mt * 16 + r16 < G::NPX3M;
        int oz3;
        asm volatile("s_mov_b32 %0, 0" : "=s"(oz3));
        if (P.act && ok)
          *reinterpret_cast<f32x4*>(P.act + P.a_y3 + (long)cur * npx3 * 64 + (unsigned)((mt * 16 + r16 + oz3) * 64 + 16 * w + 4 * g)) =
              f32x4{relu1(acc[0]), relu1(acc[1]), relu1(acc[2]), relu1(acc[3])};
#pragma unroll
        for (int q = 0; q < 4; q++)
          v3[mt][q] = (mt * 16 + 15 < G::NPX3M || ok) ? relu1(acc[q]) * inv_t : -INFINITY;
      };
#pragma unroll
      for (int mt = 0; mt < NT3; mt++) {
        fx[mt] = (float)ox; fy[mt] = (float)oy;
        const bool more = mt + 1 < NT3;
        if (more) bcur = base3(mt + 1, ox, oy);
        __builtin_amdgcn_sched_barrier(0);
        MFMA_FIRST_AW(accs[mt], wc3[0], fa[0], bias3);
#pragma unroll
        for (int i = 1; i < 18; i++) {
          if (i < 9) MFMA_AW(accs[mt], wc3[i], fa[i]); else MFMA_AW(accs[mt], wc3[i], fb[i - 9]);
          if (mt == 0 && i <= 9) fb[i - 1] = ld3one(bfirst, 9 + i - 1);
          if (more) { if (i - 1 < 9) fa[i - 1] = ld3one(bcur, i - 1); else fb[i - 10] = ld3one(bcur, i - 1); }
          if (i == 4 && mt > 0) { asm volatile("" : "+v"(accs[mt - 1])); epi3(mt - 1); }
          __builtin_amdgcn_sched_barrier(0);
        }
        if (more) fb[8] = ld3one(bcur, 17);
        __builtin_amdgcn_sched_barrier(0);
      }
      MFMA_CHAIN_END(accs[NT3 - 1]);
      epi3(NT3 - 1);
      STAMP(6);
      float mx[4], se[4], sx[4], sy[4];
#if EF_X & 16
#pragma unroll
      for (int q = 0; q < 4; q++) { mx[q] = v3[0][q]; se[q] = v3[1][q]; sx[q] = v3[2][q]; sy[q] = v3[NT3 - 1][q]; }
#else
#pragma unroll
      for (int q = 0; q < 4; q++) {
        float m = v3[0][q];
#pragma unroll
        for (int mt = 1; mt < NT3; mt++) m = fmaxf(m, v3[mt][q]);
        mx[q] = m; se[q] = 0.f; sx[q] = 0.f; sy[q] = 0.f;
      }
      EF_ROW16_4("v_max_f32_dpp", mx);
      {
        const f32x2 m01 = {mx[0], mx[1]}, m23 = {mx[2], mx[3]};
        f32x2 se01 = {0.f, 0.f}, se23 = {0.f, 0.f}, sxy[4] = {{0.f, 0.f}, {0.f, 0.f}, {0.f, 0.f}, {0.f, 0.f}};
#pragma unroll
        for (int mt = 0; mt < NT3; mt++) {
          const f32x2 d01 = f32x2{v3[mt][0], v3[mt][1]} - m01, d23 = f32x2{v3[mt][2], v3[mt][3]} - m23;
          const f32x2 e01 = {__builtin_amdgcn_exp2f(d01[0]), __builtin_amdgcn_exp2f(d01[1])};
          const f32x2 e23 = {__builtin_amdgcn_exp2f(d23[0]), __builtin_amdgcn_exp2f(d23[1])};
          se01 += e01; se23 += e23;
          const f32x2 fxy = {fx[mt], fy[mt]};
          sxy[0] = __builtin_elementwise_fma(f32x2{e01[0], e01[0]}, fxy, sxy[0]);
          sxy[1] = __builtin_elementwise_fma(f32x2{e01[1], e01[1]}, fxy, sxy[1]);
          sxy[2] = __builtin_elementwise_fma(f32x2{e23[0], e23[0]}, fxy, sxy[2]);
          sxy[3] = __builtin_elementwise_fma(f32x2{e23[1], e23[1]}, fxy, sxy[3]);
        }
        se[0] = se01[0]; se[1] = se01[1]; se[2] = se23[0]; se[3] = se23[1];
#pragma unroll
        for (int q = 0; q < 4; q++) { sx[q] = sxy[q][0]; sy[q] = sxy[q][1]; }
      }
      EF_ROW16_4("v_add_f32_dpp", se);
      EF_ROW16_4("v_add_f32_dpp", sx);
      EF_ROW16_4("v_add_f32_dpp", sy);
#endif
      if constexpr (G::DEFER) {
        if (r16 == 0) {
#pragma unroll
          for (int q = 0; q < 4; q++)
            *reinterpret_cast<f32x4*>(ps + dslot * 1024 + (16 * w + 4 * g + q) * 16) = f32x4{mx[q], se[q], sx[q], sy[q]};
        }
      } else
      if (r16 == 0) {
        float fx_[4], fy_[4];
#pragma unroll
        for (int q = 0; q < 4; q++) {
          const float r = __builtin_amdgcn_rcpf(se[q]);
          fx_[q] = sx[q] * r; fy_[q] = sy[q] * r;
        }
        const u32x2 lo = pack4_bf16(fx_[0], fy_[0], fx_[1], fy_[1]), hi = pack4_bf16(fx_[2], fy_[2], fx_[3], fy_[3]);
        *reinterpret_cast<u32x4*>(sa + slot * SA_STRIDE + 4 * (16 * w + 4 * g)) = u32x4{lo[0], lo[1], hi[0], hi[1]};
        if (P.act) {
          float* f = P.act + P.a_sa + (long)cur * 128 + (unsigned)(2 * (16 * w + 4 * g));
          *reinterpret_cast<f32x4*>(f) = f32x4{fx_[0], fy_[0], fx_[1], fy_[1]};
          *reinterpret_cast<f32x4*>(f + 4) = f32x4{fx_[2], fy_[2], fx_[3], fy_[3]};
        }
      }
    }

    STAMP(7);
    if constexpr (G::DEFER) {
      if (dslot == EF_DCHUNK - 1 || !has_next) {
        int ld_;
        asm volatile("v_mov_b32 %0, 0" : "=v"(ld_));
        ld_ += l;
        const int r16 = ld_ & 15, g = ld_ >> 4;
        const int nd = dslot + 1, jimg = min(r16, nd - 1);
        const long img0 = cur - (long)dslot * nworkers;
        {
          const unsigned char* bA = d1 + jimg * G::D1S + 16 * g;
          u32x4 f[16];
#pragma unroll
          for (int s2 = 0; s2 < 16; s2++) f[s2] = *reinterpret_cast<const u32x4*>(bA + s2 * 64);
          f32x4 acc;
          __builtin_amdgcn_sched_barrier(0);
          if (ph == 0) {
            MFMA_FIRST_AW(acc, wc2a[0], f[0], bias2a);
#pragma unroll
            for (int s2 = 1; s2 < 16; s2++) MFMA_AW(acc, wc2a[s2], f[s2]);
          } else {
            MFMA_FIRST_AW(acc, wc2b[0], f[0], bias2b);
#pragma unroll
            for (int s2 = 1; s2 < 16; s2++) MFMA_AW(acc, wc2b[s2], f[s2]);
          }
          MFMA_CHAIN_END(acc);
          const u32x2 pk = pack4_bf16(relu1(acc[0]), relu1(acc[1]), relu1(acc[2]), relu1(acc[3]));
          if (r16 < nd) {
            *reinterpret_cast<u32x2*>(d2 + r16 * G::D2S + 8 * 128 + (32 * cg + 8 * g + 4 * ph) * 2) = pk;
            if (P.act) {
              __bf16* y = reinterpret_cast<__bf16*>(P.act + P.a_y2) + img0 * (npx2 * 64) +
                          (unsigned)(r16 * (unsigned)nworkers * (unsigned)(npx2 * 64) + (npx2 - 1) * 64 + 32 * cg + 8 * g + 4 * ph);
              *reinterpret_cast<u32x2*>(y) = pk;
            }
          }
        }
        asm volatile("s_waitcnt lgkmcnt(0)" ::: "memory");
        __builtin_amdgcn_s_barrier();
        {
          const unsigned char* bB = d2 + jimg * G::D2S + 16 * g;
          u32x4 f[18];
#pragma unroll
          for (int s3 = 0; s3 < 18; s3++) f[s3] = *reinterpret_cast<const u32x4*>(bB + (s3 >> 1) * 128 + 64 * (s3 & 1));
          f32x4 st[4];
#pragma unroll
          for (int q = 0; q < 4; q++) st[q] = *reinterpret_cast<const f32x4*>(ps + jimg * 1024 + (16 * w + 4 * g + q) * 16);
          f32x4 acc;
          __builtin_amdgcn_sched_barrier(0);
          MFMA_FIRST_AW(acc, wc3[0], f[0], bias3);
#pragma unroll
          for (int s3 = 1; s3 < 18; s3++) MFMA_AW(acc, wc3[s3], f[s3]);
          MFMA_CHAIN_END(acc);
          const float inv_t = (1.0f / temp) * 1.44269504088896f;
          const f32x4 y3 = {relu1(acc[0]), relu1(acc[1]), relu1(acc[2]), relu1(acc[3])};
          float fx_[4], fy_[4];
#pragma unroll
          for (int q = 0; q < 4; q++) {
            const float v = y3[q] * inv_t, m = st[q][0];
            const float M = fmaxf(m, v);
            const float ea = __builtin_amdgcn_exp2f(m - M), eb = __builtin_amdgcn_exp2f(v - M);
            const float se = st[q][1] * ea + eb;
            const float sx = st[q][2] * ea + eb * (float)(G::OW3 - 1), sy = st[q][3] * ea + eb * (float)(G::OH3 - 1);
            const float r = __builtin_amdgcn_rcpf(se);
            fx_[q] = sx * r; fy_[q] = sy * r;
          }
          if (r16 < nd) {
            const u32x2 lo = pack4_bf16(fx_[0], fy_[0], fx_[1], fy_[1]), hi = pack4_bf16(fx_[2], fy_[2], fx_[3], fy_[3]);
            *reinterpret_cast<u32x4*>(sa + (slot - dslot + r16) * SA_STRIDE + 4 * (16 * w + 4 * g)) = u32x4{lo[0], lo[1], hi[0], hi[1]};
            if (P.act) {
              const unsigned jo = (unsigned)r16 * (unsigned)nworkers;
              *reinterpret_cast<f32x4*>(P.act + P.a_y3 + img0 * (npx3 * 64) + (unsigned)(jo * (unsigned)(npx3 * 64) + (npx3 - 1) * 64 + 16 * w + 4 * g)) = y3;
              float* fo = P.act + P.a_sa + img0 * 128 + (unsigned)(jo * 128u + 2 * (16 * w + 4 * g));
              *reinterpret_cast<f32x4*>(fo) = f32x4{fx_[0], fy_[0], fx_[1], fy_[1]};
              *reinterpret_cast<f32x4*>(fo + 4) = f32x4{fx_[2], fy_[2], fx_[3], fy_[3]};
            }
          }
        }
      }
    }
    const bool chunk_done = (slot == EF_CHUNK - 1) || !has_next;
    if (chunk_done) {
      u32x4 wf1[4][4];
      int lf;
      asm volatile("v_mov_b32 %0, 0" : "=v"(lf));
      lf += tid;
      const int w = lf >> 6, l = lf & 63, g = l >> 4;
#pragma unroll
      for (int j = 0; j < 4; j++)
#pragma unroll
        for (int s = 0; s < 4; s++) wf1[j][s] = P.wpk[WP_F1 + ((4 * w + j) * 4 + s) * 64 + l];
      f32x4 bf1[4];
#pragma unroll
      for (int j = 0; j < 4; j++) bf1[j] = *reinterpret_cast<const f32x4*>(P.params + po[8] + 16 * (4 * w + j) + 4 * g);
      u32x4 wf2[8];
#pragma unroll
      for (int s = 0; s < 8; s++) wf2[s] = P.wpk[WP_F2 + ((w & 1) * 8 + s) * 64 + l];
      const f32x4 bf2 = *reinterpret_cast<const f32x4*>(P.params + po[10] + 16 * (w & 1) + 4 * g);
      asm volatile("s_waitcnt lgkmcnt(0)" ::: "memory");
      __builtin_amdgcn_s_barrier();
      const int n_in_chunk = slot + 1;
      {
        const unsigned char* base = sa + min(r16, EF_CHUNK - 1) * SA_STRIDE + 16 * g;
#pragma unroll
        for (int j = 0; j < 4; j++) {
          f32x4 acc = {0.f, 0.f, 0.f, 0.f};
          const u32x4 (&wf)[4] = wf1[j];
          const float c0 = bf1[j][0], c1 = bf1[j][1], c2 = bf1[j][2], c3 = bf1[j][3];
#pragma unroll
          for (int s = 0; s < 4; s++)
            acc = __builtin_amdgcn_mfma_f32_16x16x32_bf16(as_bf16x8(wf[s]), as_bf16x8(*reinterpret_cast<const u32x4*>(base + 64 * s)), acc, 0, 0, 0);
          const f32x4 r = {fmaxf(acc[0] + c0, 0.f), fmaxf(acc[1] + c1, 0.f), fmaxf(acc[2] + c2, 0.f), fmaxf(acc[3] + c3, 0.f)};
          if (r16 < EF_CHUNK)
            *reinterpret_cast<u32x2*>(h1 + r16 * H1_STRIDE + (16 * (4 * w + j) + 4 * g) * 2) = pack4_bf16(r[0], r[1], r[2], r[3]);
          if (P.act && r16 < n_in_chunk)
            *reinterpret_cast<f32x4*>(P.act + P.a_h1 + (worker + (long)(it - slot) * nworkers) * 256 +
                                      (unsigned)(r16 * (unsigned)nworkers * 256u + 16 * (4 * w + j) + 4 * g)) = r;
        }
      }
      asm volatile("s_waitcnt lgkmcnt(0)" ::: "memory");
      __builtin_amdgcn_s_barrier();
      if (w < 2) {
        const unsigned char* base = h1 + min(r16, EF_CHUNK - 1) * H1_STRIDE + 16 * g;
        f32x4 acc = {0.f, 0.f, 0.f, 0.f};
        const float c0 = bf2[0], c1 = bf2[1], c2 = bf2[2], c3 = bf2[3];
#pragma unroll
        for (int s = 0; s < 8; s++)
          acc = __builtin_amdgcn_mfma_f32_16x16x32_bf16(as_bf16x8(wf2[s]), as_bf16x8(*reinterpret_cast<const u32x4*>(base + 64 * s)), acc, 0, 0, 0);
        int lq;
        asm volatile("v_mov_b32 %0, 0" : "=v"(lq));
        lq += l;
        const int r16 = lq & 15, g = lq >> 4;
        if (r16 < n_in_chunk) {
          float* o = P.out + (worker + (long)(it - slot) * nworkers) * 32 + (unsigned)(r16 * (unsigned)nworkers * 32u + 16 * w + 4 * g);
          f32x4 r = {acc[0] + c0, acc[1] + c1, acc[2] + c2, acc[3] + c3};
          *reinterpret_cast<f32x4*>(o) = r;
        }
      }
    }
    STAMP(8);
    if (!has_next) {
      asm volatile("s_waitcnt vmcnt(0)" ::: "memory");
      break;
    }
    if (!early_land) {
      asm volatile("s_waitcnt vmcnt(0)" ::: "memory");
      __syncthreads();
    }
    STAMP(9);
    cur = nxt; it++; buf ^= 1;
  }
#if defined(EF_STAMPS) || defined(EF_BLKCLK)
  n_served += it + 1;
#endif
  __syncthreads();
  }
#if defined(EF_STAMPS) || defined(EF_BLKCLK)
  if (threadIdx.x == 0 && blockIdx.x < 256) { ef_blk[blockIdx.x] = clock64() - t_entry; ef_blk[256 + blockIdx.x] = n_served; }
#endif
}


#define EF_GEOMS(X) X(84, 84) X(64, 64) X(44, 60) X(128, 128)

extern "C" int tacorl_encoder_fused_supported(int H, int W) {
#define X(h, w) if (H == h && W == w) return EFGeom<h, w>::OK ? 1 : 0;
  EF_GEOMS(X)
#undef X
  return ef_ring_supported(H, W);
}

template <int H, int W>
static int ef_launch(EFArgs& a, int nb, hipStream_t st) {
  static bool attr_set = false;
  auto kfn = encoder_fused_kernel<H, W>;
  if (!attr_set) {
    (void)hipFuncSetAttribute(reinterpret_cast<const void*>(kfn), hipFuncAttributeMaxDynamicSharedMemorySize, 160 * 1024);
    attr_set = true;
  }
  constexpr size_t lds_bytes = EFGeom<H, W>::LDS_BYTES;
  hipLaunchKernelGGL(kfn, dim3(nb), dim3(256), lds_bytes, st, a);
  return hipGetLastError() == hipSuccess ? TACORL_OK : TACORL_ELAUNCH;
}

extern "C" int tacorl_encoder_fused_act_format(int H, int W) {
  if (ef_ring_supported(H, W)) return ebw_supported(H, W) ? 1 : 2;
  return tacorl_encoder_fused_supported(H, W) ? 1 : 0;
}

extern "C" int tacorl_encoder_fwd_fused(int nprob, const void* const* img, const void* const* packed,
                                        const float* const* params, float* const* out, float* const* act,
                                        const int* n_img, int H, int W, tacorl_stream_t stream) {
  return tacorl_encoder_fwd_fused_wg(nprob, img, packed, params, out, act, n_img, H, W, 0, stream);
}
extern "C" int tacorl_encoder_fwd_fused_wg(int nprob, const void* const* img, const void* const* packed,
                                           const float* const* params, float* const* out, float* const* act,
                                           const int* n_img, int H, int W, int max_workgroups, tacorl_stream_t stream) {
  if (nprob < 1 || nprob > EF_MAXP || !tacorl_encoder_fused_supported(H, W)) return TACORL_EINVAL;
  if (max_workgroups < 0 || (max_workgroups > 0 && max_workgroups < nprob)) return TACORL_EINVAL;
  EFArgs a{};
  a.nprob = nprob; a.H = H; a.W = W;
  long total = 0;
  for (int p = 0; p < nprob; p++) total += n_img[p];
  if (total == 0) return TACORL_OK;
  const int budget = max_workgroups > 0 && max_workgroups < 256 ? max_workgroups : 256;
  const bool ring = ef_ring_supported(H, W) != 0;
  a.act_bf16 = tacorl_encoder_fused_act_format(H, W) == 1;
  const int setup_cost = ring ? EF_SETUP_COST / 4 : EF_SETUP_COST;
  long units = 0;
  int first = 1;
  for (int p = 0; p < nprob; p++) {
    a.p[p].img = (const __bf16*)img[p]; a.p[p].wpk = (const u32x4*)packed[p]; a.p[p].params = params[p];
    a.p[p].out = out[p]; a.p[p].n_img = n_img[p];
    a.p[p].act = act ? act[p] : nullptr;
    a.p[p].cost = a.p[p].act ? (ring ? (a.act_bf16 ? 84 : 96) : EF_ACT_COST) : 64;
    if (n_img[p] > 0 && !first) units += setup_cost;
    a.p[p].ustart = units;
    units += (long)a.p[p].cost * n_img[p];
    if (n_img[p] > 0) first = 0;
    if (a.p[p].act) {
      long ao[5];
      tacorl_encoder_act_layout(n_img[p], H, W, ao);
      a.p[p].a_y2 = ao[1]; a.p[p].a_y3 = ao[2]; a.p[p].a_sa = ao[3]; a.p[p].a_h1 = ao[4];
    }
  }
  a.utotal = units;
  const int nb = (int)(total < budget ? total : budget);
  if (ring) return ef_ring_launch(a, nb, H, W, (hipStream_t)stream);
#define X(h, w) if (H == h && W == w) return ef_launch<h, w>(a, nb, (hipStream_t)stream);
  EF_GEOMS(X)
#undef X
  return TACORL_EINVAL;
}
```

### tacorl_amd/csrc/rl_ops.hip

```cpp
#include <stdio.h>

#include "../../include/tacorl_hip.h"
#include "common.h"

#define LAUNCH_OK() (hipGetLastError() == hipSuccess ? TACORL_OK : TACORL_ELAUNCH)

__device__ __forceinline__ float softplusf(float x) {
  return x > 20.f ? x : log1pf(expf(x));
}
__device__ __forceinline__ float block_sum_256(float v, float* sh) {
  v = wave_sum(v);
  __syncthreads();
  if ((threadIdx.x & 63) == 0) sh[threadIdx.x >> 6] = v;
  __syncthreads();
  return sh[0] + sh[1] + sh[2] + sh[3];
}

template <typename OutT>
__global__ void pack_images_kernel(const float* __restrict__ src, long img_pitch, int src_nchw,
                                   OutT* __restrict__ dst, int n, int C, int HW) {
  const long total = (long)n * HW;
  for (long i = (long)blockIdx.x * blockDim.x + threadIdx.x; i < total; i += (long)gridDim.x * blockDim.x) {
    const long img = i / HW;
    const int px = (int)(i - img * HW);
    const float* s = src + img * img_pitch;
    OutT* d = dst + i * C;
    for (int c = 0; c < C; c++) d[c] = (OutT)(src_nchw ? s[(long)c * HW + px] : s[(long)px * C + c]);
  }
}
extern "C" int tacorl_pack_images(const float* src, long img_pitch, int src_nchw, void* dst, int dst_dtype,
                                  int n, int C, int H, int W, tacorl_stream_t stream) {
  if (n <= 0) return TACORL_OK;
  const long total = (long)n * H * W;
  const int blocks = (int)((total + 255) / 256 > 4096 ? 4096 : (total + 255) / 256);
  if (dst_dtype == TACORL_BF16)
    hipLaunchKernelGGL(pack_images_kernel<__bf16>, dim3(blocks), dim3(256), 0, (hipStream_t)stream, src, img_pitch,
                       src_nchw, (__bf16*)dst, n, C, H * W);
  else
    hipLaunchKernelGGL(pack_images_kernel<float>, dim3(blocks), dim3(256), 0, (hipStream_t)stream, src, img_pitch,
                       src_nchw, (float*)dst, n, C, H * W);
  return LAUNCH_OK();
}

#define PACK_MAXJ 8
struct PackTbl {
  const float* src[PACK_MAXJ];
  void* dst[PACK_MAXJ];
  long pitch[PACK_MAXJ];
  int n[PACK_MAXJ];
  void* dupA[PACK_MAXJ];
  void* dupB[PACK_MAXJ];
  int dupT[PACK_MAXJ];
};
template <typename OutT>
__global__ void pack_nchw3_batch_kernel(PackTbl t, int HW) {
  const int j = blockIdx.y, q4 = HW / 4;
  const long total = (long)t.n[j] * q4;
  const float* __restrict__ src = t.src[j];
  OutT* __restrict__ dst = reinterpret_cast<OutT*>(t.dst[j]);
  for (long q = (long)blockIdx.x * blockDim.x + threadIdx.x; q < total; q += (long)gridDim.x * blockDim.x) {
    const long img = q / q4;
    const int p = (int)(q - img * q4) * 4;
    const float* s = src + img * t.pitch[j] + p;
    const f32x4 r = *reinterpret_cast<const f32x4*>(s), g = *reinterpret_cast<const f32x4*>(s + HW),
                b = *reinterpret_cast<const f32x4*>(s + 2 * HW);
    const float v[12] = {r[0], g[0], b[0], r[1], g[1], b[1], r[2], g[2], b[2], r[3], g[3], b[3]};
    OutT* d = dst + (img * HW + p) * 3;
    OutT* d2 = nullptr;
    if (t.dupT[j] > 0) {
      const long b = img / t.dupT[j];
      const int tt = (int)(img - b * t.dupT[j]);
      OutT* base = tt == 0 ? reinterpret_cast<OutT*>(t.dupA[j]) : (tt == t.dupT[j] - 1 ? reinterpret_cast<OutT*>(t.dupB[j]) : nullptr);
      if (base) d2 = base + (b * HW + p) * 3;
    }
    if constexpr (sizeof(OutT) == 2) {
#pragma unroll
      for (int k = 0; k < 3; k++) {
        const bf16x4 o = bf16x4{(__bf16)v[4 * k], (__bf16)v[4 * k + 1], (__bf16)v[4 * k + 2], (__bf16)v[4 * k + 3]};
        *reinterpret_cast<bf16x4*>(d + 4 * k) = o;
        if (d2) *reinterpret_cast<bf16x4*>(d2 + 4 * k) = o;
      }
    } else {
#pragma unroll
      for (int k = 0; k < 3; k++) {
        const f32x4 o = f32x4{v[4 * k], v[4 * k + 1], v[4 * k + 2], v[4 * k + 3]};
        *reinterpret_cast<f32x4*>(d + 4 * k) = o;
        if (d2) *reinterpret_cast<f32x4*>(d2 + 4 * k) = o;
      }
    }
  }
}
extern "C" int tacorl_pack_images_batch(int njobs, const float* const* src, const long* img_pitch, void* const* dst,
                                        const int* n_img, int dst_dtype, int H, int W, tacorl_stream_t stream) {
  return tacorl_pack_images_window_batch(njobs, src, img_pitch, dst, n_img, nullptr, nullptr, nullptr, dst_dtype, H, W, stream);
}
extern "C" int tacorl_pack_images_window_batch(int njobs, const float* const* src, const long* img_pitch, void* const* dst,
                                               const int* n_img, void* const* dst_first, void* const* dst_last,
                                               const int* window, int dst_dtype, int H, int W, tacorl_stream_t stream) {
  if (njobs < 1 || njobs > PACK_MAXJ || (H * W) % 4) return TACORL_EINVAL;
  PackTbl t{};
  long mx = 0;
  int m = 0;
  for (int j = 0; j < njobs; j++) {
    if (n_img[j] <= 0) continue;
    if (((uintptr_t)src[j] & 15) || ((uintptr_t)dst[j] & 15) || img_pitch[j] % 4) return TACORL_EINVAL;
    const int T = window ? window[j] : 0;
    if (T < 0 || (T > 0 && (T < 2 || n_img[j] % T || !dst_first || !dst_last || !dst_first[j] || !dst_last[j] ||
                            (((uintptr_t)dst_first[j] | (uintptr_t)dst_last[j]) & 15))))
      return TACORL_EINVAL;
    t.dupT[m] = T; t.dupA[m] = T ? dst_first[j] : nullptr; t.dupB[m] = T ? dst_last[j] : nullptr;
    t.src[m] = src[j]; t.dst[m] = dst[j]; t.pitch[m] = img_pitch[j]; t.n[m] = n_img[j];
    const long tot = (long)n_img[j] * (H * W / 4);
    mx = tot > mx ? tot : mx;
    m++;
  }
  if (m == 0) return TACORL_OK;
  const int blocks = (int)((mx + 255) / 256 > 8192 ? 8192 : (mx + 255) / 256);
  if (dst_dtype == TACORL_BF16)
    hipLaunchKernelGGL(pack_nchw3_batch_kernel<__bf16>, dim3(blocks, m), dim3(256), 0, (hipStream_t)stream, t, H * W);
  else
    hipLaunchKernelGGL(pack_nchw3_batch_kernel<float>, dim3(blocks, m), dim3(256), 0, (hipStream_t)stream, t, H * W);
  return LAUNCH_OK();
}

struct PackU8Tbl {
  const unsigned char* src[PACK_MAXJ];
  void* dst[PACK_MAXJ];
  long pitch[PACK_MAXJ];
  const long* idx[PACK_MAXJ];
  int istride[PACK_MAXJ];
  int n[PACK_MAXJ];
};
typedef unsigned int pk_u32x4 __attribute__((ext_vector_type(4)));
template <typename OutT>
__global__ void pack_u8_batch_kernel(PackU8Tbl t, int chunks) {
  const int j = blockIdx.y;
  const long total = (long)t.n[j] * chunks;
  const unsigned char* __restrict__ src = t.src[j];
  OutT* __restrict__ dst = reinterpret_cast<OutT*>(t.dst[j]);
  const long* __restrict__ idx = t.idx[j];
  const int istride = t.istride[j];
  for (long q = (long)blockIdx.x * blockDim.x + threadIdx.x; q < total; q += (long)gridDim.x * blockDim.x) {
    const long img = q / chunks;
    const int c = (int)(q - img * chunks);
    const long frame = idx ? idx[img * istride] : img;
    const pk_u32x4 v = *reinterpret_cast<const pk_u32x4*>(src + frame * t.pitch[j] + (long)c * 16);
    float f[16];
#pragma unroll
    for (int e = 0; e < 16; e++) {
      const float x = (float)((v[e >> 2] >> (8 * (e & 3))) & 0xffu);
      f[e] = (x / 255.0f - 0.5f) / 0.5f;
    }
    OutT* d = dst + (img * chunks + c) * 16;
    if constexpr (sizeof(OutT) == 2) {
#pragma unroll
      for (int k = 0; k < 4; k++)
        *reinterpret_cast<bf16x4*>(d + 4 * k) = bf16x4{(__bf16)f[4 * k], (__bf16)f[4 * k + 1], (__bf16)f[4 * k + 2], (__bf16)f[4 * k + 3]};
    } else {
#pragma unroll
      for (int k = 0; k < 4; k++) *reinterpret_cast<f32x4*>(d + 4 * k) = f32x4{f[4 * k], f[4 * k + 1], f[4 * k + 2], f[4 * k + 3]};
    }
  }
}
extern "C" int tacorl_pack_images_u8_batch(int njobs, const void* const* src, const long* img_pitch_bytes, void* const* dst,
                                           const int* n_img, int dst_dtype, int H, int W, tacorl_stream_t stream) {
  return tacorl_pack_images_u8_gather_batch(njobs, src, img_pitch_bytes, nullptr, nullptr, dst, n_img, dst_dtype, H, W, stream);
}
extern "C" int tacorl_pack_images_u8_gather_batch(int njobs, const void* const* src, const long* img_pitch_bytes,
                                                  const long* const* index, const int* index_stride, void* const* dst,
                                                  const int* n_img, int dst_dtype, int H, int W, tacorl_stream_t stream) {
  const long bytes = (long)H * W * 3;
  if (njobs < 1 || njobs > PACK_MAXJ || bytes % 16) return TACORL_EINVAL;
  PackU8Tbl t{};
  long mx = 0;
  int m = 0;
  for (int j = 0; j < njobs; j++) {
    if (n_img[j] <= 0) continue;
    if (((uintptr_t)src[j] & 15) || ((uintptr_t)dst[j] & 15) || img_pitch_bytes[j] % 16) return TACORL_EINVAL;
    t.src[m] = (const unsigned char*)src[j]; t.dst[m] = dst[j]; t.pitch[m] = img_pitch_bytes[j]; t.n[m] = n_img[j];
    t.idx[m] = index ? index[j] : nullptr;
    t.istride[m] = (index && index[j] && index_stride) ? index_stride[j] : 1;
    if (t.idx[m] && t.istride[m] < 1) return TACORL_EINVAL;
    const long tot = (long)n_img[j] * (bytes / 16);
    mx = tot > mx ? tot : mx;
    m++;
  }
  if (m == 0) return TACORL_OK;
  const int blocks = (int)((mx + 255) / 256 > 8192 ? 8192 : (mx + 255) / 256);
  if (dst_dtype == TACORL_BF16)
    hipLaunchKernelGGL(pack_u8_batch_kernel<__bf16>, dim3(blocks, m), dim3(256), 0, (hipStream_t)stream, t, (int)(bytes / 16));
  else
    hipLaunchKernelGGL(pack_u8_batch_kernel<float>, dim3(blocks, m), dim3(256), 0, (hipStream_t)stream, t, (int)(bytes / 16));
  return LAUNCH_OK();
}

__global__ void stage_transition_kernel(const void* __restrict__ disp, int disp_dtype, float* __restrict__ reward,
                                        float* __restrict__ done, int B, const float* __restrict__ acts_src,
                                        float* __restrict__ acts_dst, long n_acts) {
  const long i = (long)blockIdx.x * blockDim.x + threadIdx.x;
  if (i < B) {
    bool one;
    if (disp_dtype == 0) one = static_cast<const float*>(disp)[i] == 1.0f;
    else if (disp_dtype == 1) one = static_cast<const long long*>(disp)[i] == 1;
    else if (disp_dtype == 2) one = static_cast<const int*>(disp)[i] == 1;
    else one = static_cast<const unsigned char*>(disp)[i] == 1;
    const float r = one ? 1.0f : 0.0f;
    reward[i] = r;
    if (done) done[i] = r;
  }
  for (long k = i; k < n_acts; k += (long)gridDim.x * blockDim.x) acts_dst[k] = acts_src[k];
}
extern "C" int tacorl_stage_transition(const void* disp, int disp_dtype, float* reward, float* done, int B,
                                       const float* acts_src, float* acts_dst, long n_acts, tacorl_stream_t stream) {
  if (!disp || !reward || B < 1 || disp_dtype < 0 || disp_dtype > 3 || (n_acts > 0 && (!acts_src || !acts_dst))) return TACORL_EINVAL;
  const long work = n_acts > B ? n_acts : B;
  const int blocks = (int)((work + 255) / 256 > 1024 ? 1024 : (work + 255) / 256);
  hipLaunchKernelGGL(stage_transition_kernel, dim3(blocks < (B + 255) / 256 ? (B + 255) / 256 : blocks), dim3(256), 0,
                     (hipStream_t)stream, disp, disp_dtype, reward, done, B, acts_src, acts_dst, n_acts);
  return LAUNCH_OK();
}

__global__ void copy_cols_kernel(const float* __restrict__ src, int ld_src, float* __restrict__ dst, int ld_dst,
                                 int rows, int cols, int src_row_mod, int accumulate) {
  const long total = (long)rows * cols;
  for (long i = (long)blockIdx.x * blockDim.x + threadIdx.x; i < total; i += (long)gridDim.x * blockDim.x) {
    const int r = (int)(i / cols), c = (int)(i - (long)r * cols);
    const int rs = src_row_mod > 0 ? r % src_row_mod : r;
    const float v = src[(long)rs * ld_src + c];
    float* d = dst + (long)r * ld_dst + c;
    *d = accumulate ? *d + v : v;
  }
}
extern "C" int tacorl_copy_cols(const float* src, int ld_src, float* dst, int ld_dst, int rows, int cols,
                                int src_row_mod, int accumulate, tacorl_stream_t stream) {
  if (rows <= 0 || cols <= 0) return TACORL_OK;
  const long total = (long)rows * cols;
  const int blocks = (int)((total + 255) / 256 > 2048 ? 2048 : (total + 255) / 256);
  hipLaunchKernelGGL(copy_cols_kernel, dim3(blocks), dim3(256), 0, (hipStream_t)stream, src, ld_src, dst, ld_dst, rows,
                     cols, src_row_mod, accumulate);
  return LAUNCH_OK();
}

#define COPY_MAXB 32
struct CopyTbl {
  const float* src[COPY_MAXB];
  float* dst[COPY_MAXB];
  int ld_src[COPY_MAXB], ld_dst[COPY_MAXB], rows[COPY_MAXB], cols[COPY_MAXB], mod[COPY_MAXB], acc[COPY_MAXB];
};
__global__ void copy_cols_batch_kernel(CopyTbl t) {
  const int d = blockIdx.y, cols = t.cols[d], mod = t.mod[d], acc = t.acc[d];
  const long total = (long)t.rows[d] * cols;
  const float* __restrict__ src = t.src[d];
  float* __restrict__ dst = t.dst[d];
  for (long i = (long)blockIdx.x * blockDim.x + threadIdx.x; i < total; i += (long)gridDim.x * blockDim.x) {
    const int r = (int)(i / cols), c = (int)(i - (long)r * cols);
    const int rs = mod > 0 ? r % mod : r;
    const float v = src[(long)rs * t.ld_src[d] + c];
    float* o = dst + (long)r * t.ld_dst[d] + c;
    *o = acc ? *o + v : v;
  }
}
extern "C" int tacorl_copy_cols_batch(int n, const float* const* src, const int* ld_src, float* const* dst,
                                      const int* ld_dst, const int* rows, const int* cols, const int* src_row_mod,
                                      const int* accumulate, tacorl_stream_t stream) {
  if (n < 0 || n > COPY_MAXB) return TACORL_EINVAL;
  CopyTbl t{};
  long maxt = 0;
  int m = 0;
  for (int i = 0; i < n; i++) {
    if (rows[i] <= 0 || cols[i] <= 0) continue;
    t.src[m] = src[i]; t.dst[m] = dst[i]; t.ld_src[m] = ld_src[i]; t.ld_dst[m] = ld_dst[i]; t.rows[m] = rows[i];
    t.cols[m] = cols[i]; t.mod[m] = src_row_mod ? src_row_mod[i] : 0; t.acc[m] = accumulate ? accumulate[i] : 0;
    const long tot = (long)rows[i] * cols[i];
    maxt = tot > maxt ? tot : maxt;
// ... 710 lines not shown
```

### tacorl_amd/engine.py

```python
import contextlib
import os

import torch

from . import blocks, ops
from . import dist as D
from ._lib import ACT_NONE, ACT_RELU, ACT_SILU, BF16, F32, LOG_SLOTS, call, ptr


def _al4(x):
    return (x + 3) // 4 * 4


class NetBlock:

    def __init__(self, cams, goal_cams, head_dims, head_acts, head_names, device, head_parts=None, hidden=256):
        self.cams, self.goal_cams = list(cams), list(goal_cams)
        self.all_cams = sorted(set(self.cams) | set(self.goal_cams))
        self.E_obs, self.G = 32 * len(self.cams), 32 * len(self.goal_cams)
        self.genc_dims, self.genc_acts = [self.G, hidden, hidden, self.G], [ACT_RELU, ACT_RELU, ACT_NONE]
        self.head_dims, self.head_acts = list(head_dims), list(head_acts)
        off = 0
        self.enc_off = {}
        for c in self.all_cams:
            self.enc_off[c] = off
            off += blocks.encoder_size()
        self.genc_off = off
        off += blocks.mlp_size(self.genc_dims)
        self.head_off = off
        off += blocks.mlp_size(self.head_dims)
        self.size = off
        z = lambda: torch.zeros(self.size, device=device)
        self.param, self.grad, self.m, self.v = z(), z(), z(), z()
        self.param_bf16 = torch.zeros(self.size, device=device, dtype=torch.bfloat16)
        self.step = torch.zeros(1, dtype=torch.int32, device=device)
        self._head_names, self._head_parts = head_names, head_parts
        self.views, self.grad_views = self._views_of(self.param), self._views_of(self.grad)

    def _views_of(self, flat):
        dst = {}
        for c in self.all_cams:
            for k, v in blocks.encoder_views(flat, self.enc_off[c]).items():
                dst[f"encoder.networks.{c}.{k}"] = v
        gn = [(f"goal_encoder.mlp.{i}.weight", f"goal_encoder.mlp.{i}.bias") for i in (0, 2, 4)]
        dst.update(blocks.mlp_views(flat, self.genc_off, self.genc_dims, gn))
        if self._head_parts is None:
            dst.update(blocks.mlp_views(flat, self.head_off, self.head_dims, self._head_names))
        else:
            dst.update(blocks.mlp_views(flat, self.head_off, self.head_dims[:-1], self._head_names))
            dst.update(blocks.head_views(flat, self.head_off, self.head_dims, self.head_dims[-2], self._head_parts))
        return dst

    def views_of(self, flat):
        return self._views_of(flat)

    def rebind_grad(self, flat):
        assert flat.numel() == self.size and flat.is_contiguous()
        flat.copy_(self.grad)
        self.grad = flat
        self.grad_views = self._views_of(flat)

    def enc(self, cam, flat=None):
        flat = self.param if flat is None else flat
        return flat.data_ptr() + 4 * self.enc_off[cam]

    def genc(self, flat=None):
        return (self.param if flat is None else flat).data_ptr() + 4 * self.genc_off

    def head(self, flat=None):
        return (self.param if flat is None else flat).data_ptr() + 4 * self.head_off

    def genc_bf16(self):
        return self.param_bf16.data_ptr() + 2 * self.genc_off

    def head_bf16(self):
        return self.param_bf16.data_ptr() + 2 * self.head_off


class Scalar:
    def __init__(self, device, value=0.0):
        self.param = torch.full((1,), float(value), device=device)
        self.grad, self.m, self.v = (torch.zeros(1, device=device) for _ in range(3))
        self.step = torch.zeros(1, dtype=torch.int32, device=device)


class ACEngine:
    def __init__(self, cams, goal_cams, hw, action_dim, B, device, *, n=4, discount=0.99, tau=0.005, actor_lr=3e-4,
                 critic_lr=3e-4, deterministic_backup=False, reward_scale=1.0, clip_grad_val=1.0,
                 conservative_weight=1.0, lagrange_thresh=5.0, temp=1.0, with_lagrange=False,
                 discrete_gripper=False, target_entropy=-7.0, policy_layers=3, q_layers=3, hidden=256,
                 compute=F32, img_dtype=torch.float32, world_size=1):
        if sorted(cams) != sorted(goal_cams):
            raise NotImplementedError("observation and goal modalities must coincide (all in-scope configs)")
        self.cams, self.hw, self.B, self.n, self.A = list(cams), dict(hw or {}), B, n, action_dim
        self.dev, self.compute, self.img_dtype = device, compute, img_dtype
        self.dg = bool(discrete_gripper)
        self.Ac = action_dim - 1 if self.dg else action_dim
        self.HD = 2 * self.Ac + (2 if self.dg else 0)
        self.hp = dict(discount=discount, tau=tau, actor_lr=actor_lr, critic_lr=critic_lr,
                       deterministic_backup=deterministic_backup, reward_scale=reward_scale,
                       clip=clip_grad_val, cons_w=conservative_weight, gap=lagrange_thresh, temp=temp,
                       target_entropy=target_entropy)
        self.with_lagrange = with_lagrange
        self.world = world_size
        self.hidden = hidden
        nc = len(self.cams)
        self.Eo = self.G = 32 * nc
        self.E = self.Eo + self.G
        self.ldq = _al4(self.E + action_dim)
        self.lds = self.E
        pol_dims = [self.E] + [hidden] * policy_layers + [self.HD]
        q_dims = [self.E + action_dim] + [hidden] * q_layers + [1]
        silu_p, silu_q = [ACT_SILU] * policy_layers + [ACT_NONE], [ACT_SILU] * q_layers + [ACT_NONE]
        pn = [(f"actor.policy.fc_layers.{i}.weight", f"actor.policy.fc_layers.{i}.bias") for i in range(policy_layers)]
        parts = [("actor.policy.fc_mean", self.Ac), ("actor.policy.fc_log_std", self.Ac)]
        if self.dg:
            parts.append(("actor.policy.gripper_action", 2))
        qn = [(f"critic.Q.fc_layers.{i}.weight", f"critic.Q.fc_layers.{i}.bias") for i in range(q_layers)]
        qn.append(("critic.Q.out.weight", "critic.Q.out.bias"))
        self.actor = NetBlock(cams, goal_cams, pol_dims, silu_p, pn, device, head_parts=parts, hidden=hidden)
        mk = lambda: NetBlock(cams, goal_cams, q_dims, silu_q, qn, device, hidden=hidden)
        self.q1, self.q2, self.tq1, self.tq2 = mk(), mk(), mk(), mk()
        self.log_alpha, self.log_alpha_prime = Scalar(device), Scalar(device)
        self.arena_extra = []
        self._bind_arena()
        self.extra_enc, self._wpk = [], {}
        self.B = None
        if B:
            self.ensure_batch(B)

    def _bind_arena(self):
        blks = [self.actor, self.q1, self.q2]
        sizes = [b.size for b in blks] + [4] + [b.size for b in self.arena_extra]
        arena = torch.zeros(sum(sizes), device=self.dev)
        o = 0
        for blk in blks:
            blk.rebind_grad(arena[o: o + blk.size])
            o += blk.size
        old = self.log_alpha_prime.grad
        arena[o: o + 1].copy_(old.reshape(-1)[:1])
        self.log_alpha_prime.grad = arena[o: o + 1]
        o += 4
        for blk in self.arena_extra:
            blk.rebind_grad(arena[o: o + blk.size])
            o += blk.size
        self.grad_arena = arena

    def extend_arena(self, blk):
        if not any(b is blk for b in self.arena_extra):
            ops.note_alloc()
            self.arena_extra.append(blk)
            self._bind_arena()

    def ensure_batch(self, B, hw=None):
        hw = dict(hw) if hw is not None else self.hw
        if self.B != B or hw != self.hw:
            self.B, self.hw = B, hw
            self._alloc()

    def _alloc(self):
        B, n, dev = self.B, self.n, self.dev
        ops.note_alloc()
        f = lambda *s: torch.zeros(*s, device=dev)
        self.X3 = {c: torch.zeros(3 * B, *self.hw[c], 3, device=dev, dtype=self.img_dtype) for c in self.cams}
        self.enc_probs = [("a_og", self.actor, 0, 2 * B), ("a_nx", self.actor, 2 * B, B), ("q1", self.q1, 0, 2 * B),
                          ("q2", self.q2, 0, 2 * B), ("tq1", self.tq1, B, 2 * B), ("tq2", self.tq2, B, 2 * B)]
        self.enc_out = {(k, c): f(nimg, 32) for k, _, _, nimg in self.enc_probs for c in self.cams}
        self.enc_act = {(k, c): f(ops.encoder_act_layout(nimg, *self.hw[c])[1])
                        for k, _, _, nimg in self.enc_probs for c in self.cams}
        self.enc_dout = {(k, c): f(2 * B, 32) for k in ("a_og", "q1", "q2") for c in self.cams}
        nets = [("a", self.actor), ("q1", self.q1), ("q2", self.q2), ("tq1", self.tq1), ("tq2", self.tq2)]
        self.nets = nets
        self.gin = {k: f(B, self.G) for k, _ in nets}
        self.gact = {k: f(ops.mlp_act_layout(B, net.genc_dims, net.genc_acts)[2]) for k, net in nets}
        self.g_yoff = ops.mlp_act_layout(B, self.actor.genc_dims, self.actor.genc_acts)[1][-1]
        self.S = {k: f(B, self.lds) for k in ("a", "a_nx", "q1", "q2", "tq1", "tq2")}
        pd, pa = self.actor.head_dims, self.actor.head_acts
        self.pact = {k: f(ops.mlp_act_layout(B, pd, pa)[2]) for k in ("a", "a_nx")}
        self.p_yoff = ops.mlp_act_layout(B, pd, pa)[1][-1]
        R = (3 * n + 1) * B
        self.R = R
        self.acts_main, self.act_pi, self.act_next = f(R, self.A), f(B, self.A), f(B, self.A)
        self.logp_pi, self.logp_next = f(B), f(B)
        self.logp_cur, self.logp_nxt = f(n * B), f(n * B)
        self.grip_pi = torch.zeros(B, dtype=torch.int32, device=dev)
        qd, qa = self.q1.head_dims, self.q1.head_acts
        self.XQ = {k: f(R, self.ldq) for k in ("q1", "q2")}
        self.XQpi = {k: f(B, self.ldq) for k in ("q1", "q2")}
        self.XT = {k: f(B, self.ldq) for k in ("tq1", "tq2")}
        self.qact = {k: f(ops.mlp_act_layout(R, qd, qa)[2]) for k in ("q1", "q2")}
        self.qact_pi = {k: f(ops.mlp_act_layout(B, qd, qa)[2]) for k in ("q1", "q2")}
        self.qact_t = {k: f(ops.mlp_act_layout(B, qd, qa)[2]) for k in ("tq1", "tq2")}
        self.q_yoff_R = ops.mlp_act_layout(R, qd, qa)[1][-1]
        self.q_yoff_B = ops.mlp_act_layout(B, qd, qa)[1][-1]
        self.dq = {k: f(R) for k in ("q1", "q2")}
        self.dq_pi = {k: f(B) for k in ("q1", "q2")}
        self.dXQ = {k: f(R, self.ldq) for k in ("q1", "q2")}
        self.dXQpi = {k: f(B, self.ldq) for k in ("q1", "q2")}
        self.d_head = f(B, self.HD)
        self.dS = {k: f(B, self.lds) for k in ("a", "q1", "q2")}
        self.dgin = {k: f(B, self.G) for k in ("a", "q1", "q2")}
        self.reward, self.done = f(B), f(B)
        self.action = self.acts_main[:B]
        shapes = dict(eps_pi=(B, self.Ac), eps_next=(B, self.Ac), eps_cur=(n, B, self.Ac), eps_nxt=(n, B, self.Ac))
        shapes.update(getattr(self, "extra_normal", {}))
        ushapes = dict(u_rand=(n * B, self.A))
        if self.dg:
            ushapes.update(g_pi=(B, 2), g_next=(B, 2), g_cur=(n, B, 2), g_nxt=(n, B, 2))

        def carve(sh):
            import math
            sizes = {k: _al4(math.prod(v)) for k, v in sh.items()}
            flat = f(sum(sizes.values()))
            out, off = {}, 0
            for k, v in sh.items():
                out[k] = flat[off: off + math.prod(v)].view(*v)
                off += sizes[k]
            return flat, out

        self._noise_normal, nn_ = carve(shapes)
        self._noise_uniform, nu_ = carve(ushapes)
        self.extra_noise = {k: nn_.pop(k) for k in getattr(self, "extra_normal", {})}
        self.noise = dict(eps_pi=nn_["eps_pi"], eps_next=nn_["eps_next"], u_rand=nu_["u_rand"], eps_cur=nn_["eps_cur"],
                          eps_nxt=nn_["eps_nxt"])
        if self.dg:
            self.noise.update({k: nu_[k] for k in ("g_pi", "g_next", "g_cur", "g_nxt")})
        self.logs = f(32)
        self.cql_ws = torch.empty(max(256, ops.L.lib().tacorl_cql_ws_bytes(B)), dtype=torch.uint8, device=dev)

    def set_noise(self, noise=None):
        if noise is None:
            self._noise_normal.normal_()
            self._noise_uniform.uniform_()
            return
        for k, buf in self.noise.items():
            buf.copy_(noise[k].reshape(buf.shape))
        for k, buf in self.extra_noise.items():
            if k in noise:
                buf.copy_(noise[k].reshape(buf.shape))

    def load_images(self, cam, obs, goal, nxt, nchw=True):
        H, W = self.hw[cam]
        xd = BF16 if self.img_dtype == torch.bfloat16 else F32
        esz, img = self.X3[cam].element_size(), H * W * 3
        jobs = []
        if obs.dtype == torch.uint8:
            for i, t in enumerate((obs, goal, nxt)):
                assert t.is_cuda and t.dtype == torch.uint8 and t[0].is_contiguous() and tuple(t.shape[-3:]) == (H, W, 3)
                pitch = t.stride(0) if t.shape[0] > 1 else img
                jobs.append((t.data_ptr(), pitch, self.X3[cam].data_ptr() + i * self.B * img * esz, self.B))
            if img % 16 or any(j[0] % 16 or j[1] % 16 for j in jobs):
                raise ValueError("uint8 frames: H*W*3 and the image pitch must be multiples of 16, tensors 16-byte aligned")
            ops.pack_images_u8_batch(jobs, xd, H, W)
            return
        for i, t in enumerate((obs, goal, nxt)):
            assert t.is_cuda and t.dtype == torch.float32 and t[0].is_contiguous()
            pitch = t.stride(0) if t.shape[0] > 1 else 3 * H * W
            jobs.append((t.data_ptr(), pitch, self.X3[cam].data_ptr() + i * self.B * img * esz, self.B))
        if nchw and (H * W) % 4 == 0 and all(j[0] % 16 == 0 and j[1] % 4 == 0 for j in jobs):
            ops.pack_images_batch(jobs, xd, H, W)
        else:
            for src, pitch, dst, n_ in jobs:
                call("tacorl_pack_images", src, pitch, int(nchw), dst, xd, n_, 3, H, W, ops.stream())

    def load_transition(self, action, reward, done):
        self.action.copy_(action.reshape(self.B, self.A).float())
        self.reward.copy_(reward.reshape(self.B).float())
        self.done.copy_(done.reshape(self.B).float())

    def _img_ptr(self, cam, first_row):
        H, W = self.hw[cam]
        return self.X3[cam].data_ptr() + first_row * H * W * 3 * self.X3[cam].element_size()

    GRAD_PROBS = ("a_og", "q1", "q2")
    use_fused = True
    wgrad_side_streams = os.environ.get("TACORL_WGRAD_SIDE", "0") == "1"
    conv_wgrad_side_stream = False

    def _fused_ok(self, c):
        if not self.use_fused or self.compute != BF16 or self.img_dtype != torch.bfloat16:
            return False
        return bool(ops.L.lib().tacorl_encoder_fused_supported(*self.hw[c]))

    def _fused_bwd_ok(self, c):
        return self._fused_ok(c) and ops.L.lib().tacorl_encoder_bwd_fused_ws_bytes(
            3, ops.int_array([2 * self.B] * 3), *self.hw[c]) > 0

    def _packed(self, net, c):
        key = (id(net), c)
        if key not in self._wpk:
            ops.note_alloc()
            self._wpk[key] = torch.empty(ops.L.lib().tacorl_encoder_fused_wpk_bytes(), dtype=torch.uint8, device=self.dev)
        return self._wpk[key]

    def _all_problems(self, c, which="all"):
        pr = [] if which == "extra" else [
            (self._img_ptr(c, r0), net, self.enc_out[(k, c)], self.enc_act[(k, c)], n, k in self.GRAD_PROBS, c)
            for k, net, r0, n in self.enc_probs]
        if which != "own":
            pr += [(x["img"], x["net"], x["out"], x["act"], x["n"], False, c) for x in self.extra_enc if x["cam"] == c]
        return pr

    def encode_split(self, between):
        groups = self._fused_groups()
        if not self.extra_enc or len(groups) != 1 or sorted(groups[0]) != sorted(self.cams) or not all(self._fused_bwd_ok(c) for c in self.cams):
            return False
        cs = groups[0]
        for which in ("extra", "own"):
            pr = [x for c in cs for x in self._all_problems(c, which)]
            for c in cs:
                self._pack_encoders(c, list({id(x[1]): x[1] for x in pr if x[6] == c}.values()), only_stale=self.ef_pack_late)
            if which == "own":
                self._launch_fused(cs[0], pr, max_wg=int(os.environ.get("TACORL_EF_SPLIT_BUDGET", "160")))
            else:
                self._launch_fused(cs[0], pr)
                between()
        return True

    ef_pack_late = os.environ.get("TACORL_EF_PACK_LATE", "1") == "1"

    def _pack_encoders(self, c, nets, only_stale=False):
        vers = self.__dict__.setdefault("_wpk_ver", {})
        if only_stale:
            nets = [n_ for n_ in nets if vers.get((id(n_), c)) != n_.param._version]
        if not nets:
            return
        call("tacorl_encoder_pack_weights", len(nets), ops.ptr_array([n_.enc(c) for n_ in nets]),
             ops.ptr_array([self._packed(n_, c) for n_ in nets]), ops.stream())
        for n_ in nets:
            vers[(id(n_), c)] = n_.param._version

    def _late_pack_nets(self):
        return [self.actor, self.q1, self.q2, self.tq1, self.tq2]

    def packs_stale(self):
        if not self.ef_pack_late or not getattr(self, "_wpk_ver", None):
            return False
        nets = {id(n_): n_ for n_ in self._late_pack_nets()}
        nets.update({id(x["net"]): x["net"] for x in self.extra_enc})
        return any(self._wpk_ver.get((i, c), n_.param._version) != n_.param._version
                   for i, n_ in nets.items() for c in self.cams if (i, c) in self._wpk_ver)

    def packs_written(self):
        vers = getattr(self, "_wpk_ver", None)
        if self.ef_pack_late and vers:
            for n_ in self._late_pack_nets():
                for c in self.cams:
                    if (id(n_), c) in vers:
                        vers[(id(n_), c)] = n_.param._version

    def _launch_fused(self, c, pr, max_wg=0):
        H, W = self.hw[c]
        call("tacorl_encoder_fwd_fused_wg", len(pr), ops.ptr_array([x[0] for x in pr]),
             ops.ptr_array([self._packed(x[1], x[6]) for x in pr]), ops.ptr_array([x[1].enc(x[6]) for x in pr]),
             ops.ptr_array([x[2] for x in pr]), ops.ptr_array([x[3] if x[5] else None for x in pr]),
             ops.int_array([x[4] for x in pr]), H, W, int(max_wg), ops.stream())

    def _fused_groups(self):
        groups, out = {}, []
        for c in self.cams:
            if self._fused_ok(c):
                groups.setdefault((tuple(self.hw[c]), bool(self._fused_bwd_ok(c))), []).append(c)
        for (_, bwd_ok), cs in groups.items():
            if (bwd_ok and len(cs) > 1 and os.environ.get("TACORL_EF_MERGE_CAMS", "1") == "1"
                    and sum(len(self._all_problems(c)) for c in cs) <= 16):
                out.append(cs)
            else:
                out += [[c] for c in cs]
        return out

    def encode_fused_only(self):
        n_total = 0
        for cs in self._fused_groups():
            pr = [x for c in cs for x in self._all_problems(c)]
            self._launch_fused(cs[0], pr)
            n_total += sum(x[4] for x in pr)
        return n_total

    def _encode_all(self):
        xd = BF16 if self.img_dtype == torch.bfloat16 else F32
        merged = {c: cs for cs in self._fused_groups() if len(cs) > 1 for c in cs}
        for c in self.cams:
            H, W = self.hw[c]
            pr = self._all_problems(c)
            if c in merged:
                if merged[c][0] != c:
                    continue
                allp = []
                for cc in merged[c]:
                    prc = self._all_problems(cc)
                    self._pack_encoders(cc, list({id(x[1]): x[1] for x in prc}.values()), only_stale=self.ef_pack_late)
                    allp += prc
                self._launch_fused(c, allp)
                continue
            if self._fused_ok(c):
                saves = self._fused_bwd_ok(c) or ops.L.lib().tacorl_encoder_fused_act_format(H, W) == 2
                slow = [] if saves else [x for x in pr if x[5]]
                pr = [x for x in pr if not (slow and x[5])]
                nets = {id(x[1]): x[1] for x in pr}
                self._pack_encoders(c, list(nets.values()), only_stale=self.ef_pack_late)
                self._launch_fused(c, pr)
                pr = slow
            if pr:
                call("tacorl_encoder_fwd", len(pr), ops.ptr_array([x[0] for x in pr]),
                     ops.ptr_array([x[1].enc(c) for x in pr]), ops.ptr_array([x[2] for x in pr]),
                     ops.ptr_array([x[3] for x in pr]), ops.int_array([x[4] for x in pr]), H, W, xd, self.compute,
                     ops.stream())

    adam_writes_mirrors = os.environ.get("TACORL_ADAM_MIRRORS", "0") == "1"

    def _mirror_nets(self):
        return [self.actor, self.q1, self.q2, self.tq1, self.tq2]

    def mirrors_stale(self):
        return self.compute == BF16 and any(getattr(n_, "_mirror_ver", None) != n_.param._version for n_ in self._mirror_nets())

    def mirrors_written(self):
        if self.compute == BF16 and self.adam_writes_mirrors:
            for n_ in self._mirror_nets():
                n_._mirror_ver = n_.param._version

    def _refresh_bf16(self):
        if self.compute != BF16:
            return
        nets = [n_ for n_ in self._mirror_nets()
                if not self.adam_writes_mirrors or getattr(n_, "_mirror_ver", None) != n_.param._version
                or os.environ.get("TACORL_ALWAYS_REFRESH") == "1"]
        if not nets:
            return
        call("tacorl_to_bf16_batch", len(nets), ops.ptr_array([n_.genc() for n_ in nets]),
             ops.ptr_array([n_.genc_bf16() for n_ in nets]), (ops.C.c_long * len(nets))(*[n_.size - n_.genc_off for n_ in nets]),
             ops.stream())
        for n_ in nets:
            n_._mirror_ver = n_.param._version

    def _mlp_bwd_sites(self):
        B = self.B
        qd, pd, gd = self.q1.head_dims, self.actor.head_dims, self.actor.genc_dims
        return [("q", [self.q1.head(), self.q2.head()], [self.R, self.R], qd),
                ("qpi", [self.q1.head(), self.q2.head()], [B, B], qd),
                ("pi", [self.actor.head()], [B], pd),
                ("genc", [self.actor.genc(), self.q1.genc(), self.q2.genc()], [B] * 3, gd)]

    def _prepack_backward(self):
        self._prepacked = False
        if self.compute != BF16:
            return
        inline = os.environ.get("TACORL_PACK_INLINE", "1") == "1"
        if getattr(self, "_pack_stream", None) is None:
            self._pack_stream = torch.cuda.Stream(device=self.dev)
        ps = torch.cuda.current_stream() if inline else self._pack_stream
        if not inline:
            ps.wait_stream(torch.cuda.current_stream())
        with torch.cuda.stream(ps):
            for tag, params, M, dims in self._mlp_bwd_sites():
                ops.mlp_bwd_fused_pack(params, M, dims, "mlp_bwdf_" + tag, self.dev)
            nets = [self.actor, self.q1, self.q2]
            for cs in self._ebw_sequences():
                c = cs[0]
                if self._fused_bwd_ok(c):
                    H, W = self.hw[c]
                    np_ = 3 * len(cs)
                    n3 = ops.int_array([2 * self.B] * np_)
                    nb = ops.L.lib().tacorl_encoder_bwd_fused_ws_bytes(np_, n3, H, W)
                    ws = ops.workspace(nb, self.dev, "enc_bwd_fused_" + "+".join(cs))
                    call("tacorl_encoder_bwd_fused_pack", np_, ops.ptr_array([x.enc(cc) for cc in cs for x in nets]), n3, H, W, ptr(ws),
                         ws.numel(), ops.stream())
        self._prepacked = True

    gather_inputs = os.environ.get("TACORL_MLP_GATHER", "1") == "1"

    def _gather_ok(self, tag):
        if not (self.gather_inputs if self.gather_inputs is not None else os.environ.get("TACORL_MLP_GATHER", "1") == "1") \
                or self.compute != BF16:
            return False
        cache = self.__dict__.setdefault("_gather_cache", {})
        key = (tag, self.B)
        if key not in cache:
            B = self.B
            M, net, ldx = {"genc": ([B] * 5, (self.actor.genc_dims, self.actor.genc_acts), self.G),
                           "pi": ([B] * 2, (self.actor.head_dims, self.actor.head_acts), self.lds),
                           "q": ([self.R, self.R, B, B, B, B], (self.q1.head_dims, self.q1.head_acts), self.ldq)}[tag]
            geom_ok = self.G % 4 == 0 and self.Eo % 8 == 0 and self.E % 8 == 0 and self.g_yoff % 4 == 0
            cache[key] = geom_ok and (tag != "q" or self.A % 4 == 0) and ops.mlp_fwd_gather_ok(
                M, net[0], net[1], ldx, self.compute, self._lean(tag))
        return cache[key]

    def _emb_segs(self, ek, row0, gk, mod=0):
        segs = [(self.enc_out[(ek, c)], row0 * 32, 32, 32 * j, mod) for j, c in enumerate(self.cams)]
        segs.append((self.gact[gk], self.g_yoff, self.G, self.Eo, mod))
        return segs

    _OBS_SRC = {"a": ("a_og", 0, "a"), "a_nx": ("a_nx", 0, "a"), "q1": ("q1", 0, "q1"), "q2": ("q2", 0, "q2"),
                "tq1": ("tq1", 1, "tq1"), "tq2": ("tq2", 1, "tq2")}

    def _assemble_states(self):
        B = self.B
        src = {"a": ("a_og", B), "q1": ("q1", B), "q2": ("q2", B), "tq1": ("tq1", 0), "tq2": ("tq2", 0)}
        nets = dict(self.nets)
        ks = ["a", "q1", "q2", "tq1", "tq2"]
        if self._gather_ok("genc"):
            segs = [[(self.enc_out[(src[k][0], c)], src[k][1] * 32, 32, 32 * j, 0) for j, c in enumerate(self.cams)] for k in ks]
            ops.mlp_fwd_gather(segs, [self.gin[k] for k in ks], self.G, [nets[k].genc() for k in ks],
                               [nets[k].genc_bf16() for k in ks], [self.gact[k] for k in ks], [B] * 5, self.actor.genc_dims,
                               self.actor.genc_acts, lean=self._lean("genc"))
# ... 305 lines not shown
```

### tacorl_amd/modules/tacorl/tacorl.py

```python
from pathlib import Path

import os

import torch
import torch.nn as nn

from ... import dist as D
from ... import ops
from ..._lib import BF16, F32, call, ptr
from ..common import register_views
from ..cql.cql_offline_lightning import CQL_Offline


class TACORL(CQL_Offline):
    def __init__(self, play_lmp_dir: str = "~/tacorl/models/play_lmp", lmp_epoch_to_load: int = -1,
                 overwrite_lmp_cfg: dict = {}, finetune_action_decoder: bool = False,
                 action_decoder_lr: float = 1e-4, *args, play_lmp=None, **kwargs):
        self.play_lmp_dir = Path(play_lmp_dir).expanduser()
        self.lmp_epoch_to_load = lmp_epoch_to_load
        self.overwrite_lmp_cfg = overwrite_lmp_cfg
        self.finetune_action_decoder = finetune_action_decoder
        self.action_decoder_lr = action_decoder_lr
        self.action_loss_every_n_steps = kwargs.pop("action_loss_every_n_steps", 1)
        self.lmp_unsafe_pickle = bool(kwargs.pop("lmp_unsafe_pickle", False))
        self.__dict__["_play_lmp"] = play_lmp
        super().__init__(*args, **kwargs)

    def build_networks(self):
        from ..play_lmp.play_lmp_for_rl import PlayLMP, load_play_lmp

        lmp = self.__dict__.pop("_play_lmp", None)
        if lmp is None:
            lmp = load_play_lmp(self.play_lmp_dir, self.lmp_epoch_to_load, self.overwrite_lmp_cfg, device=self.dev,
                                compute_dtype=self.compute, image_dtype=self.img_dtype, unsafe_pickle=self.lmp_unsafe_pickle)
        assert isinstance(lmp, PlayLMP)
        from .. import cfgcheck

        cfgcheck.check_critic(self.critic_cfg, "critic")
        cfgcheck.check_representation(self.critic_encoder_cfg, "critic_encoder", lmp.plan_proposal_obs_modalities)
        self.action_decoder_modalities = list(lmp.action_decoder_modalities)
        self.plan_recognition_modalities = list(lmp.plan_recognition_modalities)
        self.all_modalities = sorted(set(self.action_decoder_modalities + self.plan_recognition_modalities))
        cams, goal_cams = list(lmp.plan_proposal_obs_modalities), list(lmp.plan_proposal_goal_modalities)
        self.obs_modalities, self.goal_modalities = cams, goal_cams
        self.action_dim = lmp.pr.latent_plan_dim
        a = dict(policy_layers=lmp.policy_layers, q_layers=lmp.policy_layers, hidden=lmp.hidden,
                 discrete_gripper=False)
        self._make_engine(cams, goal_cams, self.action_dim, a)
        e = self.engine
        e.actor.param.copy_(lmp.net.param)
        from ...init import init_views_

        for q in (e.q1, e.q2):
            init_views_(q.views)
            n = q.head_off - q.genc_off
            q.param[q.genc_off: q.genc_off + n].copy_(lmp.net.param[lmp.net.genc_off: lmp.net.genc_off + n])
        self.sync_targets()
        self._register()
        self.lmp_net, self.pr, self.ad = lmp.net, lmp.pr, lmp.ad
        enc_views = {k[len("encoder."):]: v for k, v in lmp.net.views.items() if k.startswith("encoder.")}
        register_views(self, "perceptual_encoder.", enc_views, requires_grad=False)
        register_views(self, "plan_recognition.", lmp.pr.blk.views, requires_grad=False)
        if self.ad is not None:
            e.pre_metrics = [self.ad.finish_loss]
            self._pv["action_decoder"] = register_views(self, "action_decoder.", self.ad.blk.views)
            for k, v in self.ad.buffers.items():
                self.action_decoder.register_buffer(k, v)
            if self.finetune_action_decoder:
                e.extend_arena(self.ad.blk)
        self._T = None
        from ..inference import attach_rollout_surface

        attach_rollout_surface(self, e.actor, cams, goal_cams, self.action_dim, False, lmp_net=self.lmp_net,
                               lmp_cams=self.action_decoder_modalities, ad=self.ad)

    def named_gradients(self):
        out = super().named_gradients()
        if self.ad is not None and self.finetune_action_decoder:
            out.update({f"action_decoder.{k}": v for k, v in self.ad.blk.grad_views.items()})
        return out

    def _ensure_seq(self, B, T, hw):
        if self._T == (B, T, tuple(sorted(hw.items()))):
            return
        ops.note_alloc()
        dev = self.dev
        self.frames = {c: torch.zeros(B * T, *hw[c], 3, device=dev, dtype=self.img_dtype) for c in self.all_modalities}
        self.f_out = {c: torch.zeros(B * T, 32, device=dev) for c in self.all_modalities}
        self.f_act = {c: torch.zeros(ops.encoder_act_layout(B * T, *hw[c])[1], device=dev) for c in self.all_modalities}
        npr = len(self.plan_recognition_modalities)
        self.pr_in = torch.zeros(B * T, 32 * npr, device=dev)
        e = self.engine
        assert e.action.shape == (B, self.action_dim) and e.action.dtype == torch.float32
        self.plan, self.reward = e.action, e.reward
        self.engine.extra_enc = [dict(cam=c, img=self.frames[c], net=self.lmp_net, out=self.f_out[c],
                                      act=self.f_act[c], n=B * T) for c in self.all_modalities]
        self._T = (B, T, tuple(sorted(hw.items())))

    def _stage_small(self, batch, noise, B, T):
        e = self.engine
        disp, acts = batch["disp"], batch["actions"] if self.ad is not None else None
        dd = {torch.float32: 0, torch.int64: 1, torch.int32: 2, torch.uint8: 3, torch.bool: 3}.get(disp.dtype)
        if (dd is not None and disp.is_cuda and disp.is_contiguous() and disp.numel() == B
                and (acts is None or (acts.is_cuda and acts.is_contiguous() and acts.dtype == torch.float32
                                      and acts.shape == self.acts.shape))):
            call("tacorl_stage_transition", ptr(disp), dd, ptr(self.reward), ptr(e.done), B,
                 ptr(acts) if acts is not None else None, ptr(self.acts) if acts is not None else None,
                 acts.numel() if acts is not None else 0, ops.stream())
        else:
            if acts is not None:
                self.acts.copy_(acts)
            self.reward.copy_(disp == 1)
            e.done.copy_(self.reward)
        e.set_noise(noise)

    def _stage_frames(self, batch, noise, nchw=True):
        from ...data.replay import wait_ready

        wait_ready(batch)
        rp = batch.get("replay")
        if rp is not None:
            u8, nchw, B, T = True, False, rp["B"], rp["T"]
            states = rp["frames"]
            hw = {c: tuple(v.shape[1:3]) for c, v in states.items()}
        else:
            states = batch["states"]
            u8 = next(iter(states.values())).dtype == torch.uint8
            if u8:
                nchw = False
            B, T = next(iter(states.values())).shape[:2]
            hw = {c: (tuple(v.shape[-2:]) if nchw else tuple(v.shape[-3:-1])) for c, v in states.items()}
        src_hw = dict(hw)
        rs = (batch.get("aug") or {}).get("resize") or {}
        if rs:
            if not u8:
                raise ValueError("aug['resize'] needs the dataset's uint8 frames (the resize is part of the uint8 pack)")
            hw = {c: tuple(rs.get(c, hw[c])) for c in hw}
        self.engine.extra_normal = {"eps_pr": (B, self.action_dim)}
        self.engine.ensure_batch(B, {c: hw[c] for c in self.engine.cams})
        self.eps_pr = self.engine.extra_noise["eps_pr"]
        self._ensure_seq(B, T, hw)
        xd = BF16 if self.img_dtype == torch.bfloat16 else F32
        e = self.engine
        if self.ad is not None and (getattr(self, "acts", None) is None or self.acts.shape[:2] != (B, T)):
            ops.note_alloc()
            self.acts = torch.zeros(B, T, 7, device=self.dev)
        if getattr(self, "_stage_stream", None) is None:
            self._stage_stream = torch.cuda.Stream(device=self.dev)
        main = torch.cuda.current_stream()
        side = self._stage_stream if getattr(self, "stage_side", True) else main
        side.wait_stream(main)
        with torch.cuda.stream(side):
            self._stage_small(batch, noise, B, T)
        for c in sorted(set(self.all_modalities) | set(e.cams)):
            H, W = hw[c]
            v = states[c]
            sz = 1 if u8 else 4
            assert v.is_cuda and v.is_contiguous() and v.dtype == (torch.uint8 if u8 else torch.float32)
            if rp is not None:
                Hs, Ws = src_hw[c]
                ids, fb = rp["ids"], 3 * Hs * Ws
                assert ids.is_cuda and ids.dtype == torch.int64 and ids.is_contiguous() and ids.numel() == B * T + B
                ip = ids.data_ptr()
                jobs = [(v.data_ptr(), fb, self.frames[c].data_ptr(), B * T, ip, 1)] if c in self.all_modalities else []
                if c in e.cams:
                    esz, x3, ob = e.X3[c].element_size(), e.X3[c].data_ptr(), 3 * H * W
                    jobs += [(v.data_ptr(), fb, x3, B, ip, T), (v.data_ptr(), fb, x3 + B * ob * esz, B, ip + 8 * B * T, 1),
                             (v.data_ptr(), fb, x3 + 2 * B * ob * esz, B, ip + 8 * (T - 1), T)]
                if fb % 16 or v.data_ptr() % 16:
                    raise ValueError("uint8 dataset: H*W*3 must be a multiple of 16 and the tensor 16-byte aligned")
                aug = batch.get("aug")
                if aug is None:
                    ops.pack_images_u8_gather_batch(jobs, xd, H, W)
                else:
                    st, gl = aug["states"][c], aug["goal"][c]
                    sh, ji = st.get("shift"), st.get("jitter")
                    row = lambda t, k: None if t is None else t[:, k].contiguous()
                    flat = lambda t: None if t is None else t.reshape(B * T, t.shape[-1]).contiguous()
                    tabs = [(flat(sh), flat(ji))] if c in self.all_modalities else []
                    if c in e.cams:
                        tabs += [(row(sh, 0), row(ji, 0)), (gl.get("shift"), gl.get("jitter")), (row(sh, T - 1), row(ji, T - 1))]
                    ops.pack_images_u8_resize_aug_batch([j + t for j, t in zip(jobs, tabs)], xd, (Hs, Ws), H, W, aug["pad"][c])
                continue
            Hs, Ws = src_hw[c]
            simg = 3 * Hs * Ws
            jobs = [(v.data_ptr(), simg, self.frames[c].data_ptr(), B * T)] if c in self.all_modalities else []
            if c in e.cams:
                g = batch["goal"][c]
                assert g.is_cuda and g.is_contiguous() and g.dtype == v.dtype
                esz, img = e.X3[c].element_size(), H * W * 3
                x3 = e.X3[c].data_ptr()
                jobs += [(v.data_ptr(), T * simg, x3, B), (g.data_ptr(), simg, x3 + B * img * esz, B),
                         (v.data_ptr() + sz * (T - 1) * simg, T * simg, x3 + 2 * B * img * esz, B)]
            aug = batch.get("aug") if u8 else None
            if aug is not None:
                st, gl = aug["states"][c], aug["goal"][c]
                sh, ji = st.get("shift"), st.get("jitter")
                row = lambda t, k: None if t is None else t[:, k].contiguous()
                flat = lambda t: None if t is None else t.reshape(B * T, t.shape[-1]).contiguous()
                tabs = [(flat(sh), flat(ji))] if c in self.all_modalities else []
                if c in e.cams:
                    tabs += [(row(sh, 0), row(ji, 0)), (gl.get("shift"), gl.get("jitter")), (row(sh, T - 1), row(ji, T - 1))]
                ops.pack_images_u8_resize_aug_batch([j + (None, 1) + t for j, t in zip(jobs, tabs)], xd, (Hs, Ws), H, W,
                                                    aug["pad"][c])
            elif u8:
                if (H * W * 3) % 16 or any(j[0] % 16 for j in jobs):
                    raise ValueError("uint8 frames: H*W*3 must be a multiple of 16 and the tensors 16-byte aligned")
                ops.pack_images_u8_batch(jobs, xd, H, W)
            elif nchw and (H * W) % 4 == 0:
                import ctypes as C
                if (c in self.all_modalities and c in e.cams and len(jobs) == 4 and T >= 2
                        and os.environ.get("TACORL_PACK_DEDUP", "1") == "1"):
                    win, _, goal, _ = jobs
                    x3, img_b = e.X3[c].data_ptr(), H * W * 3 * e.X3[c].element_size()
                    js = [win, goal]
                    call("tacorl_pack_images_window_batch", 2, (C.c_void_p * 2)(*[j[0] for j in js]),
                         (C.c_long * 2)(*[j[1] for j in js]), (C.c_void_p * 2)(*[j[2] for j in js]),
                         ops.int_array([j[3] for j in js]), (C.c_void_p * 2)(x3, None), (C.c_void_p * 2)(x3 + 2 * B * img_b, None),
                         ops.int_array([T, 0]), xd, H, W, ops.stream())
                    continue
                call("tacorl_pack_images_batch", len(jobs), (C.c_void_p * len(jobs))(*[j[0] for j in jobs]),
                     (C.c_long * len(jobs))(*[j[1] for j in jobs]), (C.c_void_p * len(jobs))(*[j[2] for j in jobs]),
                     ops.int_array([j[3] for j in jobs]), xd, H, W, ops.stream())
            else:
                for src, pitch, dst, n in jobs:
                    call("tacorl_pack_images", src, pitch, int(nchw), dst, xd, n, 3, H, W, ops.stream())
        main.wait_stream(side)
        return B, T, hw

    def _ad_due(self):
        k = self.action_loss_every_n_steps
        return self.ad is not None and (self.finetune_action_decoder or k <= 1 or (self._step_count + 1) % k == 0)

    def _device_front(self, B, T, hw, optimize, with_ad=True):
        e = self.engine
        ops.mark("front:start")
        if getattr(self, "_pr_stream", None) is None:
            prio = -1 if os.environ.get("TACORL_PR_PRIO", "0") == "1" else 0
            self._pr_stream, self._side_stream = torch.cuda.Stream(device=self.dev, priority=prio), torch.cuda.Stream(device=self.dev)
        main = torch.cuda.current_stream()
        mods = self.plan_recognition_modalities
        emb, ld = (self.f_out[mods[0]], 32) if len(mods) == 1 else (self.pr_in, self.pr_in.shape[1])
        ad_prep, ad_prepared = None, False
        if (with_ad and optimize and self.finetune_action_decoder and getattr(self, "ad_early_prepare", True)
                and self.ad._bwd_fast(B, self.compute)):
            self._side_stream.wait_stream(main)
            with torch.cuda.stream(self._side_stream):
                self.ad.refresh_mirrors(B, T - 1)
                ad_prepared = self.ad.prepare_backward(B, T - 1, self.compute)
                ad_prep = torch.cuda.Event()
                ad_prep.record(self._side_stream)
        sp = os.environ.get("TACORL_EF_SPLIT_LMP", "auto")
        split = with_ad and (sp == "1" or (sp == "auto" and (T >= 24 or (optimize and self.finetune_action_decoder))))
        forked = []

        def fork_branches():
            forked.append(self._fork_pr_ad(B, T, main, mods, emb, ld, with_ad, optimize, ad_prep, ad_prepared))

        if not (split and e.encode_split(fork_branches)):
            e._encode_all()
        ops.mark("front:encoded")
        if not forked:
            fork_branches()
        ready, ad_on_side = forked[0]
        e.action_ready = ready
        e.phase_a(encoded=True, optimize=optimize)
        if ad_prep is not None:
            main.wait_stream(self._side_stream)
        segmented = self._segmented() or not self._use_graph
        if with_ad and not ad_on_side:
            if segmented:
                main.wait_stream(self._pr_stream)
            else:
                self._ad_join = self._pr_stream
        if segmented:
            main.wait_stream(self._pr_stream)
            e.action_ready = None
            self._join_ad()

    def _fork_pr_ad(self, B, T, main, mods, emb, ld, with_ad, optimize, ad_prep, ad_prepared):
        e = self.engine
        self._ad_join = None
        ad_on_side = with_ad and not (optimize and self.finetune_action_decoder)
        self._pr_stream.wait_stream(main)
        with torch.cuda.stream(self._pr_stream):
            ops.mark("pr:start")
            if len(mods) > 1:
                for j, c in enumerate(mods):
                    ops.copy_cols(self.f_out[c], 0, 32, self.pr_in, 32 * j, self.pr_in.shape[1], B * T, 32)
            self.pr.forward(emb, ld, B, T, self.compute, inference=True, sample=(self.eps_pr, self.plan), frozen=True)
            ops.mark("pr:plan")
            ready = torch.cuda.Event()
            ready.record(self._pr_stream)
            if with_ad and not ad_on_side:
                if ad_prep is not None:
                    self._pr_stream.wait_event(ad_prep)
                self.ad.loss_step(self, self.acts, self.plan, B, T, True, defer_update=self._defer_ad_update(),
                                  mirrors_current=ad_prep is not None, prepared=ad_prepared)
        if ad_on_side:
            self._side_stream.wait_event(ready)
            with torch.cuda.stream(self._side_stream):
                ops.mark("ad:start")
                self.ad.loss_step(self, self.acts, self.plan, B, T, False, frozen=not self.finetune_action_decoder)
                ops.mark("ad:end")
            self._ad_join = self._side_stream
        return ready, ad_on_side

    def _defer_ad_update(self):
        return D.collectives_on(self.world_size) or getattr(self, "_force_graph_split", False)

    def _join_ad(self):
        if getattr(self, "_ad_join", None) is not None:
            torch.cuda.current_stream().wait_stream(self._ad_join)
            self._ad_join = None

    def get_pr_latent_plan(self, batch, noise=None, nchw=True):
        B, T, hw = self._stage_frames(batch, noise, nchw)
        xd = BF16 if self.img_dtype == torch.bfloat16 else F32
        for c in self.all_modalities:
            H, W = hw[c]
            call("tacorl_encoder_fwd", 1, ops.ptr_array([self.frames[c]]), ops.ptr_array([self.lmp_net.enc(c)]),
                 ops.ptr_array([self.f_out[c]]), ops.ptr_array([self.f_act[c]]), ops.int_array([B * T]), H, W, xd,
                 self.compute, ops.stream())
        for j, c in enumerate(self.plan_recognition_modalities):
            ops.copy_cols(self.f_out[c], 0, 32, self.pr_in, 32 * j, self.pr_in.shape[1], B * T, 32)
        head = self.pr.forward(self.pr_in, self.pr_in.shape[1], B, T, self.compute, inference=True)
        call("tacorl_pr_sample", ptr(head), ptr(self.eps_pr), ptr(self.plan), None, None, B, self.action_dim,
             float(self.pr.min_std), ops.stream())
        return self.plan

    def training_step(self, batch, batch_idx=0, noise=None):
        self._step(batch, noise, optimize=True, log_type="train")
        self._tick_optimizers()

    def validation_step(self, batch, *args, noise=None, **kwargs):
        self._step(batch, noise, optimize=False, log_type="validation")

    def _step(self, batch, noise, optimize, log_type, nchw=True):
        B, T, hw = self._stage_frames(batch, noise, nchw)
        with_ad = self._ad_due()
        key = ("tacorl", B, T, tuple(sorted(hw.items())), self.current_epoch < self.bc_epochs, optimize, with_ad)
        e, bc = self.engine, self.current_epoch < self.bc_epochs
        ad_update = with_ad and optimize and self.finetune_action_decoder and self._defer_ad_update()

        def tail():
            e.phase_c(optimize)
            self._join_ad()
            if ad_update:
                self.ad.update(self)
            ops.mark("step:end")

        segmented = self._segmented()
        ad_ft = optimize and self.finetune_action_decoder
        ad_side = with_ad and segmented and self._use_graph
        side = None
        if ad_side and ad_ft:
            side = (0, lambda: self.ad.loss_step(self, self.acts, self.plan, B, T, True, defer_update=True), 1)
        elif ad_side:
            side = (0, lambda: self.ad.loss_step(self, self.acts, self.plan, B, T, False, frozen=not self.finetune_action_decoder))
        def allreduce_grads():
            if ad_update:
                self._join_ad()
            e.allreduce_grads()

        self._run_segments(key, [lambda: self._device_front(B, T, hw, optimize, with_ad and not ad_side),
                                 lambda: e.phase_b(bc, optimize), tail],
                           [e.allreduce_alpha, allreduce_grads], side=side)
        self._publish_logs(log_type, extra=("action_loss",) if with_ad else ())

    def configure_optimizers(self):
        o = super().configure_optimizers()
        if self.finetune_action_decoder and self.ad is not None:
            blk = self.ad.blk
            o.append(self._make_adam("action_decoder", [(blk, self._pv["action_decoder"], blk.views_of(blk.m),
                                                         blk.views_of(blk.v))], self.action_decoder_lr))
        return o
```

Baseline: 1238 grad-steps/s.

## Read fp32 window frames directly in fused encoder, skipping bf16 pack pass

The fused encoder forward can now load fp32 CHW frames straight from the batch tensor through a pointer slot. It converts them to interleaved bf16 in LDS, with the global-to-LDS loads overlapped with the conv MFMAs. This drops the separate pack kernel that wrote a bf16 copy of all B*T window frames, saving one full read and write pass over the frames. The cost is more global traffic inside the encoder, since fp32 is twice the bytes of bf16, plus extra conversion work and single-buffer handling. Frames are materialised lazily only when something else needs them.

```diff
diff --git a/include/tacorl_hip.h b/include/tacorl_hip.h
--- a/include/tacorl_hip.h
+++ b/include/tacorl_hip.h
@@ -106,6 +106,10 @@
 int tacorl_encoder_fwd_fused_wg(int nprob, const void* const* img, const void* const* packed,
                                 const float* const* params, float* const* out, float* const* act,
                                 const int* n_img, int H, int W, int max_workgroups, tacorl_stream_t stream);
+int tacorl_encoder_fwd_fused_src(int nprob, const void* const* img, const int* src_kind, const long* src_pitch,
+                                 const void* const* packed, const float* const* params, float* const* out,
+                                 float* const* act, const int* n_img, int H, int W, int max_workgroups,
+                                 tacorl_stream_t stream);
 
 size_t tacorl_encoder_bwd_fused_ws_bytes(int nprob, const int* n_img, int H, int W);
 int tacorl_encoder_bwd_fused(int nprob, const void* const* img, const float* const* params,
@@ -176,6 +180,9 @@
                        int n, int C, int H, int W, tacorl_stream_t stream);
 int tacorl_pack_images_batch(int njobs, const float* const* src, const long* img_pitch, void* const* dst,
                              const int* n_img, int dst_dtype, int H, int W, tacorl_stream_t stream);
+int tacorl_pack_images_batch_slot(int njobs, const float* const* src, const long* img_pitch, void* const* dst,
+                                  const int* n_img, int dst_dtype, int H, int W, void* slot, const void* slot_value,
+                                  tacorl_stream_t stream);
 int tacorl_pack_images_window_batch(int njobs, const float* const* src, const long* img_pitch, void* const* dst,
                                     const int* n_img, void* const* dst_first, void* const* dst_last,
                                     const int* window, int dst_dtype, int H, int W, tacorl_stream_t stream);
diff --git a/tacorl_amd/_lib.py b/tacorl_amd/_lib.py
--- a/tacorl_amd/_lib.py
+++ b/tacorl_amd/_lib.py
@@ -104,6 +104,7 @@
     "tacorl_encoder_pack_weights": (_i, [_i, _p, _p, _p]),
     "tacorl_encoder_fwd_fused": (_i, [_i, _p, _p, _p, _p, _p, _p, _i, _i, _p]),
     "tacorl_encoder_fwd_fused_wg": (_i, [_i, _p, _p, _p, _p, _p, _p, _i, _i, _i, _p]),
+    "tacorl_encoder_fwd_fused_src": (_i, [_i, _p, _p, _p, _p, _p, _p, _p, _p, _i, _i, _i, _p]),
     "tacorl_encoder_bwd_fused_ws_bytes": (_sz, [_i, _p, _i, _i]),
     "tacorl_encoder_bwd_fused": (_i, [_i, _p, _p, _p, _p, _p, _p, _i, _i, _i, _p, _sz, _p]),
     "tacorl_encoder_bwd_fused_pack": (_i, [_i, _p, _p, _i, _i, _p, _sz, _p]),
@@ -118,6 +119,7 @@
     "tacorl_mlp_bwd": (_i, [_i, _p, _i, _p, _p, _p, _i, _p, _p, _i, _p, _i, _p, _p, _i, _i, _p, _sz, _p]),
     "tacorl_pack_images": (_i, [_p, _l, _i, _p, _i, _i, _i, _i, _i, _p]),
     "tacorl_pack_images_batch": (_i, [_i, _p, _p, _p, _p, _i, _i, _i, _p]),
+    "tacorl_pack_images_batch_slot": (_i, [_i, _p, _p, _p, _p, _i, _i, _i, _p, _p, _p]),
     "tacorl_pack_images_window_batch": (_i, [_i, _p, _p, _p, _p, _p, _p, _p, _i, _i, _i, _p]),
     "tacorl_pack_images_u8_batch": (_i, [_i, _p, _p, _p, _p, _i, _i, _i, _p]),
     "tacorl_pack_images_u8_gather_batch": (_i, [_i, _p, _p, _p, _p, _p, _p, _i, _i, _i, _p]),
diff --git a/tacorl_amd/csrc/encoder_fused.h b/tacorl_amd/csrc/encoder_fused.h
--- a/tacorl_amd/csrc/encoder_fused.h
+++ b/tacorl_amd/csrc/encoder_fused.h
@@ -23,6 +23,9 @@
   int n_img;
   int cost;
   long ustart;
+  int src_f32;
+  long src_pitch;
+  const float* const* src_slot;
 };
 struct EFArgs {
   EFProblem p[EF_MAXP];
diff --git a/tacorl_amd/csrc/encoder_fused.hip b/tacorl_amd/csrc/encoder_fused.hip
--- a/tacorl_amd/csrc/encoder_fused.hip
+++ b/tacorl_amd/csrc/encoder_fused.hip
@@ -10,6 +10,9 @@
 #define EF_DCHUNK 8
 #ifndef EF_SETUP_COST
 #define EF_SETUP_COST 128
+#endif
+#ifndef EF_F32_COST
+#define EF_F32_COST 94
 #endif
 #ifndef EF_ACT_COST
 #define EF_ACT_COST 72
@@ -360,9 +363,60 @@
   };
 #undef EF_LEAN_LD
 
+  constexpr int F32_HALF = G::S2 ? G::H * G::W / 2 : 4, F32_SEG = F32_HALF * 4;
+  constexpr int F32_KPS = (F32_SEG + 1023) / 1024;
+  constexpr int F32_LASTN = (F32_SEG - (F32_KPS - 1) * 1024) >> 4;
+  static_assert(!G::S2 || (3 * F32_SEG == G::LDS_IMG && F32_HALF % 4 == 0 && F32_SEG % 16 == 0), "fp32 halves fill one image buffer");
+  const bool f32 = G::S2 && P.src_f32;
+  const float* src32 = nullptr;
+  if (f32) src32 = P.src_slot ? *P.src_slot : reinterpret_cast<const float*>(P.img);
+  auto f32_piece = [&](long img, int h, int qb, int t) {
+    const int m = t / 3, seg = t - 3 * m, kk = 4 * m + 3 - wu;
+    if (kk >= F32_KPS) return;
+    const unsigned char* gsrc = reinterpret_cast<const unsigned char*>(src32 + img * P.src_pitch) +
+                                (long)seg * (G::H * G::W * 4) + h * F32_SEG + kk * 1024;
+    const unsigned dst = lds_base + qb * a.lds_img + seg * F32_SEG + kk * 1024;
+    asm volatile("s_mov_b32 m0, %0\n\ts_nop 0" :: "s"(__builtin_amdgcn_readfirstlane(dst)) : "memory");
+    if (kk < F32_KPS - 1 || l < F32_LASTN)
+      asm volatile("global_load_lds_dwordx4 %0, %1" :: "v"(dma_voff_l), "s"(gsrc) : "memory");
+  };
+  constexpr int F32_NT = 3 * ((F32_KPS + 3) / 4);
+  auto f32_two = [&](long img, int h, int qb, int p) {
+#pragma unroll
+    for (int j = 0; j < 2; j++)
+      if (2 * p + j < F32_NT) f32_piece(img, h, qb, 2 * p + j);
+  };
+  auto f32_convert = [&](int h, int qb, int pb) {
+    const unsigned char* s0 = lds + qb * a.lds_img;
+    unsigned char* d0 = lds + pb * a.lds_img + h * (F32_HALF * 6);
+#pragma unroll
+    for (int m = 0; m < (F32_KPS + 3) / 4; m++) {
+      const int kk = 4 * m + 3 - wu, q = kk * 64 + l;
+      if (kk < F32_KPS && q < F32_HALF / 4) {
+        const f32x4 r = *reinterpret_cast<const f32x4*>(s0 + q * 16);
+        const f32x4 g = *reinterpret_cast<const f32x4*>(s0 + F32_SEG + q * 16);
+        const f32x4 b = *reinterpret_cast<const f32x4*>(s0 + 2 * F32_SEG + q * 16);
+        u32x2* d = reinterpret_cast<u32x2*>(d0 + q * 24);
+        d[0] = pack4_bf16(r[0], g[0], b[0], r[1]);
+        d[1] = pack4_bf16(g[1], b[1], r[2], g[2]);
+        d[2] = pack4_bf16(b[2], r[3], g[3], b[3]);
+      }
+    }
+  };
+
   long cur = worker;
   int it = 0, buf = 0;
-  dma_load(cur, 0, 0);
+  if (f32) {
+#pragma unroll 1
+    for (int h = 0; h < 2; h++) {
+#pragma unroll 1
+      for (int t = 0; t < F32_NT; t++) f32_piece(cur, h, 1, t);
+      asm volatile("s_waitcnt vmcnt(0)" ::: "memory");
+      f32_convert(h, 1, 0);
+    }
+  } else {
+    dma_load(cur, 0, 0);
+  }
   __builtin_amdgcn_s_waitcnt(0x0F70);
   __syncthreads();
   STAMP(0);
@@ -457,7 +511,10 @@
 #if !(EF_X & 1)
         if (G::WHOLE) {
 #pragma unroll
-          for (int q = 0; q < DPT; q++) lean_piece(i * DPT + q);
+          for (int q = 0; q < DPT; q++) {
+            if (f32) f32_two(has_next ? nxt : cur, 0, buf ^ 1, i * DPT + q);
+            else lean_piece(i * DPT + q);
+          }
         }
 #endif
       };
@@ -470,7 +527,10 @@
         for (int s = 1; s < 6; s++) {
           MFMA_AW(A0[i], wc1a[s], bf[s]);
 #if !(EF_X & 1)
-          if (G::WHOLE && (s == 1 || s == 3) && (s >> 1) < DPT) lean_piece(i * DPT + (s >> 1));
+          if (G::WHOLE && (s == 1 || s == 3) && (s >> 1) < DPT) {
+            if (f32) f32_two(has_next ? nxt : cur, 0, buf ^ 1, i * DPT + (s >> 1));
+            else lean_piece(i * DPT + (s >> 1));
+          }
 #endif
           if (s == 4 && prev >= 0) {
             asm volatile("" : "+v"(A0[prev]), "+v"(A1[prev]));
@@ -522,6 +582,11 @@
     STAMP(2);
     asm volatile("s_waitcnt lgkmcnt(0)" ::: "memory");
     EF_IMG_BARRIER();
+    const bool f32n = f32 && has_next;
+    if (f32n) {
+      asm volatile("s_waitcnt vmcnt(0)" ::: "memory");
+      f32_convert(0, buf ^ 1, buf);
+    }
     STAMP(3);
 
     {
@@ -624,6 +689,7 @@
           for (int i = 1; i < 8; i++) {
             MFMA_AW(C1[t2], wc2b[i], fa[i]);
             fa[i - 1] = ld2one(bcur, i - 1);
+            if ((i == 2 || i == 5) && f32n) f32_two(nxt, 1, buf ^ 1, 4 * t2 + (i == 5));
             __builtin_amdgcn_sched_barrier(0);
           }
           MFMA_AW(C0[t2], wc2a[8], fb[0]);
@@ -636,6 +702,7 @@
           for (int i = 1; i < 8; i++) {
             MFMA_AW(C1[t2], wc2b[8 + i], fb[i]);
             fb[i - 1] = ld2one(bcur, 8 + i - 1);
+            if ((i == 2 || i == 5) && f32n) f32_two(nxt, 1, buf ^ 1, 4 * t2 + 2 + (i == 5));
             __builtin_amdgcn_sched_barrier(0);
           }
           fb[7] = ld2one(bcur, 15);
@@ -716,7 +783,7 @@
       }
     }
     STAMP(4);
-    const bool early_land = G::WHOLE && P.act == nullptr;
+    const bool early_land = G::WHOLE && P.act == nullptr && !f32;
 #if EF_X & 32
     if (early_land) asm volatile("s_waitcnt lgkmcnt(0)" ::: "memory");
 #else
@@ -1006,12 +1073,17 @@
       asm volatile("s_waitcnt vmcnt(0)" ::: "memory");
       break;
     }
+    if (f32n) {
+      asm volatile("s_waitcnt vmcnt(0)" ::: "memory");
+      f32_convert(1, buf ^ 1, buf);
+    }
     if (!early_land) {
       asm volatile("s_waitcnt vmcnt(0)" ::: "memory");
       __syncthreads();
     }
     STAMP(9);
-    cur = nxt; it++; buf ^= 1;
+    cur = nxt; it++;
+    if (!f32) buf ^= 1;
   }
 #if defined(EF_STAMPS) || defined(EF_BLKCLK)
   n_served += it + 1;
@@ -1059,6 +1131,12 @@
 extern "C" int tacorl_encoder_fwd_fused_wg(int nprob, const void* const* img, const void* const* packed,
                                            const float* const* params, float* const* out, float* const* act,
                                            const int* n_img, int H, int W, int max_workgroups, tacorl_stream_t stream) {
+  return tacorl_encoder_fwd_fused_src(nprob, img, nullptr, nullptr, packed, params, out, act, n_img, H, W, max_workgroups, stream);
+}
+extern "C" int tacorl_encoder_fwd_fused_src(int nprob, const void* const* img, const int* src_kind, const long* src_pitch,
+                                            const void* const* packed, const float* const* params, float* const* out,
+                                            float* const* act, const int* n_img, int H, int W, int max_workgroups,
+                                            tacorl_stream_t stream) {
   if (nprob < 1 || nprob > EF_MAXP || !tacorl_encoder_fused_supported(H, W)) return TACORL_EINVAL;
   if (max_workgroups < 0 || (max_workgroups > 0 && max_workgroups < nprob)) return TACORL_EINVAL;
   EFArgs a{};
@@ -1077,6 +1155,17 @@
     a.p[p].out = out[p]; a.p[p].n_img = n_img[p];
     a.p[p].act = act ? act[p] : nullptr;
     a.p[p].cost = a.p[p].act ? (ring ? (a.act_bf16 ? 84 : 96) : EF_ACT_COST) : 64;
+    const int kind = src_kind ? src_kind[p] : 0;
+    if (kind < 0 || kind > 2) return TACORL_EINVAL;
+    if (kind) {
+      if (!(H == 84 && W == 84) || a.p[p].act || !src_pitch || src_pitch[p] < 3L * H * W || src_pitch[p] % 4 ||
+          (kind == 1 && ((uintptr_t)img[p] & 15)) || (kind == 2 && (!img[p] || ((uintptr_t)img[p] & 7))))
+        return TACORL_EINVAL;
+      a.p[p].src_f32 = 1;
+      a.p[p].src_pitch = src_pitch[p];
+      a.p[p].src_slot = kind == 2 ? (const float* const*)img[p] : nullptr;
+      a.p[p].cost = EF_F32_COST;
+    }
     if (n_img[p] > 0 && !first) units += setup_cost;
     a.p[p].ustart = units;
     units += (long)a.p[p].cost * n_img[p];
diff --git a/tacorl_amd/csrc/rl_ops.hip b/tacorl_amd/csrc/rl_ops.hip
--- a/tacorl_amd/csrc/rl_ops.hip
+++ b/tacorl_amd/csrc/rl_ops.hip
@@ -51,9 +51,12 @@
   void* dupA[PACK_MAXJ];
   void* dupB[PACK_MAXJ];
   int dupT[PACK_MAXJ];
+  const void** slot;
+  const void* slot_value;
 };
 template <typename OutT>
 __global__ void pack_nchw3_batch_kernel(PackTbl t, int HW) {
+  if (t.slot && blockIdx.x == 0 && blockIdx.y == 0 && threadIdx.x == 0) *t.slot = t.slot_value;
   const int j = blockIdx.y, q4 = HW / 4;
   const long total = (long)t.n[j] * q4;
   const float* __restrict__ src = t.src[j];
@@ -94,11 +97,26 @@
                                         const int* n_img, int dst_dtype, int H, int W, tacorl_stream_t stream) {
   return tacorl_pack_images_window_batch(njobs, src, img_pitch, dst, n_img, nullptr, nullptr, nullptr, dst_dtype, H, W, stream);
 }
+static int pack_batch(int njobs, const float* const* src, const long* img_pitch, void* const* dst, const int* n_img,
+                      void* const* dst_first, void* const* dst_last, const int* window, int dst_dtype, int H, int W,
+                      void* slot, const void* slot_value, tacorl_stream_t stream);
+extern "C" int tacorl_pack_images_batch_slot(int njobs, const float* const* src, const long* img_pitch, void* const* dst,
+                                             const int* n_img, int dst_dtype, int H, int W, void* slot, const void* slot_value,
+                                             tacorl_stream_t stream) {
+  if (!slot || ((uintptr_t)slot & 7)) return TACORL_EINVAL;
+  return pack_batch(njobs, src, img_pitch, dst, n_img, nullptr, nullptr, nullptr, dst_dtype, H, W, slot, slot_value, stream);
+}
 extern "C" int tacorl_pack_images_window_batch(int njobs, const float* const* src, const long* img_pitch, void* const* dst,
                                                const int* n_img, void* const* dst_first, void* const* dst_last,
                                                const int* window, int dst_dtype, int H, int W, tacorl_stream_t stream) {
-  if (njobs < 1 || njobs > PACK_MAXJ || (H * W) % 4) return TACORL_EINVAL;
+  return pack_batch(njobs, src, img_pitch, dst, n_img, dst_first, dst_last, window, dst_dtype, H, W, nullptr, nullptr, stream);
+}
+static int pack_batch(int njobs, const float* const* src, const long* img_pitch, void* const* dst, const int* n_img,
+                      void* const* dst_first, void* const* dst_last, const int* window, int dst_dtype, int H, int W,
+                      void* slot, const void* slot_value, tacorl_stream_t stream) {
+  if (njobs < 0 || njobs > PACK_MAXJ || (njobs < 1 && !slot) || (H * W) % 4) return TACORL_EINVAL;
   PackTbl t{};
+  t.slot = (const void**)slot; t.slot_value = slot_value;
   long mx = 0;
   int m = 0;
   for (int j = 0; j < njobs; j++) {
@@ -114,12 +132,12 @@
     mx = tot > mx ? tot : mx;
     m++;
   }
-  if (m == 0) return TACORL_OK;
-  const int blocks = (int)((mx + 255) / 256 > 8192 ? 8192 : (mx + 255) / 256);
+  if (m == 0 && !slot) return TACORL_OK;
+  const int blocks = mx == 0 ? 1 : (int)((mx + 255) / 256 > 8192 ? 8192 : (mx + 255) / 256);
   if (dst_dtype == TACORL_BF16)
-    hipLaunchKernelGGL(pack_nchw3_batch_kernel<__bf16>, dim3(blocks, m), dim3(256), 0, (hipStream_t)stream, t, H * W);
+    hipLaunchKernelGGL(pack_nchw3_batch_kernel<__bf16>, dim3(blocks, m ? m : 1), dim3(256), 0, (hipStream_t)stream, t, H * W);
   else
-    hipLaunchKernelGGL(pack_nchw3_batch_kernel<float>, dim3(blocks, m), dim3(256), 0, (hipStream_t)stream, t, H * W);
+    hipLaunchKernelGGL(pack_nchw3_batch_kernel<float>, dim3(blocks, m ? m : 1), dim3(256), 0, (hipStream_t)stream, t, H * W);
   return LAUNCH_OK();
 }
 
diff --git a/tacorl_amd/engine.py b/tacorl_amd/engine.py
--- a/tacorl_amd/engine.py
+++ b/tacorl_amd/engine.py
@@ -1,4 +1,5 @@
 import contextlib
+import ctypes as C
 import os
 
 import torch
@@ -295,10 +296,11 @@
 
     def _all_problems(self, c, which="all"):
         pr = [] if which == "extra" else [
-            (self._img_ptr(c, r0), net, self.enc_out[(k, c)], self.enc_act[(k, c)], n, k in self.GRAD_PROBS, c)
+            (self._img_ptr(c, r0), net, self.enc_out[(k, c)], self.enc_act[(k, c)], n, k in self.GRAD_PROBS, c, (0, 0))
             for k, net, r0, n in self.enc_probs]
         if which != "own":
-            pr += [(x["img"], x["net"], x["out"], x["act"], x["n"], False, c) for x in self.extra_enc if x["cam"] == c]
+            pr += [(x["img"], x["net"], x["out"], x["act"], x["n"], False, c, x.get("src", (0, 0)))
+                   for x in self.extra_enc if x["cam"] == c]
         return pr
 
     def encode_split(self, between):
@@ -351,6 +353,13 @@
 
     def _launch_fused(self, c, pr, max_wg=0):
         H, W = self.hw[c]
+        if any(x[7][0] for x in pr):
+            call("tacorl_encoder_fwd_fused_src", len(pr), ops.ptr_array([x[0] for x in pr]), ops.int_array([x[7][0] for x in pr]),
+                 (C.c_long * len(pr))(*[x[7][1] for x in pr]), ops.ptr_array([self._packed(x[1], x[6]) for x in pr]),
+                 ops.ptr_array([x[1].enc(x[6]) for x in pr]), ops.ptr_array([x[2] for x in pr]),
+                 ops.ptr_array([x[3] if x[5] else None for x in pr]), ops.int_array([x[4] for x in pr]), H, W, int(max_wg),
+                 ops.stream())
+            return
         call("tacorl_encoder_fwd_fused_wg", len(pr), ops.ptr_array([x[0] for x in pr]),
              ops.ptr_array([self._packed(x[1], x[6]) for x in pr]), ops.ptr_array([x[1].enc(x[6]) for x in pr]),
              ops.ptr_array([x[2] for x in pr]), ops.ptr_array([x[3] if x[5] else None for x in pr]),
diff --git a/tacorl_amd/modules/tacorl/tacorl.py b/tacorl_amd/modules/tacorl/tacorl.py
--- a/tacorl_amd/modules/tacorl/tacorl.py
+++ b/tacorl_amd/modules/tacorl/tacorl.py
@@ -80,12 +80,16 @@
             out.update({f"action_decoder.{k}": v for k, v in self.ad.blk.grad_views.items()})
         return out
 
-    def _ensure_seq(self, B, T, hw):
+    def _ensure_seq(self, B, T, hw, direct=()):
+        self._direct = tuple(sorted(direct))
         if self._T == (B, T, tuple(sorted(hw.items()))):
+            self._point_extra(hw)
             return
         ops.note_alloc()
         dev = self.dev
-        self.frames = {c: torch.zeros(B * T, *hw[c], 3, device=dev, dtype=self.img_dtype) for c in self.all_modalities}
+        self._frames = {c: torch.zeros(B * T, *hw[c], 3, device=dev, dtype=self.img_dtype) for c in self.all_modalities}
+        self._frames_src = {}
+        self.src_slot = {c: torch.zeros(1, dtype=torch.int64, device=dev) for c in self.all_modalities}
         self.f_out = {c: torch.zeros(B * T, 32, device=dev) for c in self.all_modalities}
         self.f_act = {c: torch.zeros(ops.encoder_act_layout(B * T, *hw[c])[1], device=dev) for c in self.all_modalities}
         npr = len(self.plan_recognition_modalities)
@@ -93,9 +97,39 @@
         e = self.engine
         assert e.action.shape == (B, self.action_dim) and e.action.dtype == torch.float32
         self.plan, self.reward = e.action, e.reward
-        self.engine.extra_enc = [dict(cam=c, img=self.frames[c], net=self.lmp_net, out=self.f_out[c],
+        self.engine.extra_enc = [dict(cam=c, img=self._frames[c], net=self.lmp_net, out=self.f_out[c],
                                       act=self.f_act[c], n=B * T) for c in self.all_modalities]
         self._T = (B, T, tuple(sorted(hw.items())))
+        self._point_extra(hw)
+
+    @property
+    def frames(self):
+        fr = self.__dict__.get("_frames")
+        src = self.__dict__.get("_frames_src")
+        if src:
+            import ctypes as C
+            xd = BF16 if self.img_dtype == torch.bfloat16 else F32
+            for c, (v, simg, n, H, W) in src.items():
+                call("tacorl_pack_images_batch", 1, (C.c_void_p * 1)(v.data_ptr()), (C.c_long * 1)(simg),
+                     (C.c_void_p * 1)(fr[c].data_ptr()), ops.int_array([n]), xd, H, W, ops.stream())
+            src.clear()
+        return fr
+
+    def _point_extra(self, hw):
+        for x in self.engine.extra_enc:
+            c = x["cam"]
+            if c in self._direct:
+                x.update(img=self.src_slot[c].data_ptr(), src=(2, 3 * hw[c][0] * hw[c][1]))
+            else:
+                x.update(img=self._frames[c], src=(0, 0))
+
+    def _direct_cams(self, states, hw, nchw):
+        if os.environ.get("TACORL_EF_F32_WINDOW", "1") != "1" or not nchw or self.img_dtype != torch.bfloat16:
+            return ()
+        e = self.engine
+        return tuple(c for c in self.all_modalities
+                     if c in e.cams and tuple(hw[c]) == (84, 84) and e._fused_ok(c) and states[c].dtype == torch.float32
+                     and states[c].data_ptr() % 16 == 0)
 
     def _stage_small(self, batch, noise, B, T):
         e = self.engine
@@ -114,7 +148,7 @@
             e.done.copy_(self.reward)
         e.set_noise(noise)
 
-    def _stage_frames(self, batch, noise, nchw=True):
+    def _stage_frames(self, batch, noise, nchw=True, direct_ok=True):
         from ...data.replay import wait_ready
 
         wait_ready(batch)
@@ -139,7 +173,8 @@
         self.engine.extra_normal = {"eps_pr": (B, self.action_dim)}
         self.engine.ensure_batch(B, {c: hw[c] for c in self.engine.cams})
         self.eps_pr = self.engine.extra_noise["eps_pr"]
-        self._ensure_seq(B, T, hw)
+        direct = self._direct_cams(states, hw, nchw) if (direct_ok and rp is None and not u8) else ()
+        self._ensure_seq(B, T, hw, direct)
         xd = BF16 if self.img_dtype == torch.bfloat16 else F32
         e = self.engine
         if self.ad is not None and (getattr(self, "acts", None) is None or self.acts.shape[:2] != (B, T)):
@@ -154,6 +189,7 @@
             self._stage_small(batch, noise, B, T)
         for c in sorted(set(self.all_modalities) | set(e.cams)):
             H, W = hw[c]
+            self._frames_src.pop(c, None)
             v = states[c]
             sz = 1 if u8 else 4
             assert v.is_cuda and v.is_contiguous() and v.dtype == (torch.uint8 if u8 else torch.float32)
@@ -162,7 +198,7 @@
                 ids, fb = rp["ids"], 3 * Hs * Ws
                 assert ids.is_cuda and ids.dtype == torch.int64 and ids.is_contiguous() and ids.numel() == B * T + B
                 ip = ids.data_ptr()
-                jobs = [(v.data_ptr(), fb, self.frames[c].data_ptr(), B * T, ip, 1)] if c in self.all_modalities else []
+                jobs = [(v.data_ptr(), fb, self._frames[c].data_ptr(), B * T, ip, 1)] if c in self.all_modalities else []
                 if c in e.cams:
                     esz, x3, ob = e.X3[c].element_size(), e.X3[c].data_ptr(), 3 * H * W
                     jobs += [(v.data_ptr(), fb, x3, B, ip, T), (v.data_ptr(), fb, x3 + B * ob * esz, B, ip + 8 * B * T, 1),
@@ -184,7 +220,7 @@
                 continue
             Hs, Ws = src_hw[c]
             simg = 3 * Hs * Ws
-            jobs = [(v.data_ptr(), simg, self.frames[c].data_ptr(), B * T)] if c in self.all_modalities else []
+            jobs = [(v.data_ptr(), simg, self._frames[c].data_ptr(), B * T)] if c in self.all_modalities else []
             if c in e.cams:
                 g = batch["goal"][c]
                 assert g.is_cuda and g.is_contiguous() and g.dtype == v.dtype
@@ -209,6 +245,13 @@
                 ops.pack_images_u8_batch(jobs, xd, H, W)
             elif nchw and (H * W) % 4 == 0:
                 import ctypes as C
+                if c in direct:
+                    js = jobs[1:]
+                    self._frames_src[c] = (v, simg, B * T, H, W)
+                    call("tacorl_pack_images_batch_slot", len(js), (C.c_void_p * len(js))(*[j[0] for j in js]),
+                         (C.c_long * len(js))(*[j[1] for j in js]), (C.c_void_p * len(js))(*[j[2] for j in js]),
+                         ops.int_array([j[3] for j in js]), xd, H, W, self.src_slot[c].data_ptr(), v.data_ptr(), ops.stream())
+                    continue
                 if (c in self.all_modalities and c in e.cams and len(jobs) == 4 and T >= 2
                         and os.environ.get("TACORL_PACK_DEDUP", "1") == "1"):
                     win, _, goal, _ = jobs
@@ -315,7 +358,7 @@
             self._ad_join = None
 
     def get_pr_latent_plan(self, batch, noise=None, nchw=True):
-        B, T, hw = self._stage_frames(batch, noise, nchw)
+        B, T, hw = self._stage_frames(batch, noise, nchw, direct_ok=False)
         xd = BF16 if self.img_dtype == torch.bfloat16 else F32
         for c in self.all_modalities:
             H, W = hw[c]
@@ -339,7 +382,7 @@
     def _step(self, batch, noise, optimize, log_type, nchw=True):
         B, T, hw = self._stage_frames(batch, noise, nchw)
         with_ad = self._ad_due()
-        key = ("tacorl", B, T, tuple(sorted(hw.items())), self.current_epoch < self.bc_epochs, optimize, with_ad)
+        key = ("tacorl", B, T, tuple(sorted(hw.items())), self.current_epoch < self.bc_epochs, optimize, with_ad, self._direct)
         e, bc = self.engine, self.current_epoch < self.bc_epochs
         ad_update = with_ad and optimize and self.finetune_action_decoder and self._defer_ad_update()
 
```

New measurement: 1284 grad-steps/s, median of 6. 1.04x the previous value.
